# MIT-SPARK/Khronos

Hardware: AMD Instinct MI355X
Metric: active-window frames/sec (+ Mvoxel-updates/sec) at 1280x720 RGB-D+labels, 2 cm voxels (higher is better)
Workload: dtype f32

## Files before the change

### include/khronos_amd.h

```cpp
#ifndef KHRONOS_AMD_H_
#define KHRONOS_AMD_H_

#include <stddef.h>
#include <stdint.h>

#ifdef __cplusplus
extern "C" {
#endif

#define KHR_OK 0
#define KHR_EINVAL (-1)
#define KHR_ENOMEM (-2)
#define KHR_EDEVICE (-3)
#define KHR_ENOTFOUND (-4)
#define KHR_ESTATE (-5)

#define KHR_VOX_ACTIVE 1u
#define KHR_VOX_EVER_FREE 2u
#define KHR_VOX_TO_REMOVE 4u
#define KHR_VOX_SEM_VALID 8u
#define KHR_BLK_UPDATED 1u
#define KHR_BLK_MESH_UPDATED 2u
#define KHR_BLK_TRACKING_UPDATED 4u
#define KHR_BLK_HAS_ACTIVE_DATA 8u
// ... 8 lines not shown
  int32_t use_weight_dropoff;
  float weight_dropoff_epsilon;
  int32_t use_constant_weight;
  float max_weight;
  int32_t interpolation_method;
  float adaptive_max_range_difference;
  int32_t range_mode;
  int32_t semantic_mode;
  float label_confidence;
  float temporal_buffer;
  float tsdf_occupancy_threshold;
  int32_t neighbor_connectivity;
  float temporal_window;
  int32_t md_neighbor_connectivity;
  int32_t md_min_cluster_size;
  int32_t md_max_cluster_size;
  float md_min_separation_distance;
  float md_max_range;
  float md_min_z_coordinate;
  float mesh_min_weight;
  uint32_t max_blocks;
  uint32_t max_frame_pixels;
  uint32_t num_frame_slots;
  uint64_t max_mesh_vertices;
  uint32_t max_band_records;
  int32_t disable_culling;
  int32_t device;
  int32_t rank;
  int32_t world_size;
  int32_t relaxed_arithmetic;
  uint32_t max_snapshot_blocks;
  int32_t alloc_candidate;
  int32_t color_blend_weight;
  int32_t mesh_attr_source;
  float mesh_degenerate_eps;
  int32_t packed_likelihood_rows;
} khr_config;

typedef struct khr_sensor {
  int32_t width, height;
  float fx, fy, cx, cy;
  float min_range, max_range;
} khr_sensor;

typedef struct khr_frame {
  uint64_t timestamp_ns;
  double world_T_sensor[16];
  const float* depth;
  const uint8_t* color;
  const int32_t* label;
} khr_frame;

typedef struct khr_stats {
  uint64_t n_allocated_blocks;
  uint64_t n_visible_blocks;
  uint64_t n_new_blocks;
  uint64_t n_visited_voxels;
  uint64_t n_updated_voxels;
  uint64_t n_band_voxels;
  uint64_t n_tracking_updated_blocks;
  uint64_t n_seeds;
  uint64_t n_mesh_blocks;
  uint64_t n_mesh_vertices;
  uint64_t pool_exhausted;
  uint64_t cum_updated_voxels;
  uint64_t cum_band_voxels;
  uint64_t cum_visited_voxels;
  uint64_t cum_integrate_calls;
  uint64_t n_tsdf_blocks;
  uint64_t band_overflow;
  uint64_t n_tracking_processed_blocks;
  uint64_t n_fuse_items;
  uint64_t n_seed_waits;
  uint64_t n_seed_waits_late;
  uint64_t seed_wait_max_us;
  uint64_t seed_wait_hist[8];
  uint64_t seed_wait_late_us;
  uint64_t seed_wait_late_frame;
  uint64_t seed_wait_late_state;
  uint64_t n_md_device_merges;
  uint64_t n_md_host_walks;
  uint64_t n_md_prelaunched;
  uint64_t n_md_prelaunch_repeats;
} khr_stats;

typedef struct khr_cluster {
  int32_t id;
  uint64_t num_pixels_listed;
  uint32_t num_pixels_painted;
  float bbox_min[3], bbox_max[3];
  float centroid[3];
  int32_t semantic_id;
} khr_cluster;

typedef struct khr_object_detector_config {
  int32_t use_full_connectivity;
  int32_t min_cluster_size;
  int32_t max_cluster_size;
  int32_t use_3d;
  float grid_size;
  float max_range;
  const int32_t* object_labels;
  int32_t n_object_labels;
} khr_object_detector_config;

typedef struct khr_ctx khr_ctx;

int khr_create(const khr_config* cfg, khr_ctx** out);
void khr_destroy(khr_ctx* ctx);
const char* khr_last_error(void);

void khr_host_trace(const char* tag);
int khr_set_stream(khr_ctx* ctx, void* hip_stream);
int khr_sync(khr_ctx* ctx);
void khr_default_config(khr_config* cfg);
int khr_reset_map(khr_ctx* ctx, float voxel_size, float truncation_distance);
int khr_retain_slot(khr_ctx* ctx, int slot);
int khr_release_slot(khr_ctx* ctx, int slot);
int khr_depend_on(khr_ctx* ctx, khr_ctx* other);
int khr_get_config(khr_ctx* ctx, khr_config* out);

int khr_upload_frame(khr_ctx* ctx, const khr_sensor* sensor, const khr_frame* frame, int on_device);
int khr_set_frame_image(khr_ctx* ctx, int slot, int which, const int32_t* image, int on_device);
int khr_download_frame(khr_ctx* ctx, int slot, float* range, float* vertex_map, int32_t* dynamic_image);
int khr_download_frame_image(khr_ctx* ctx, int slot, int which, int32_t* image);
typedef struct khr_frame_copy khr_frame_copy;
int khr_frame_copy_create(khr_ctx* ctx, int slot, khr_frame_copy** out);
int khr_frame_copy_download(khr_frame_copy* fc, float* depth, float* range, uint8_t* color_rgb, int32_t* labels, float* vertex_map);
void khr_frame_copy_release(khr_frame_copy* fc);
int khr_copy_frame_image(khr_ctx* ctx, int slot, int which, void* device_dst);

int khr_integrate(khr_ctx* ctx, int slot, int allocate_blocks, int use_mask, int object_id);
int khr_integrate_shared(khr_ctx* ctx, khr_ctx* src, int src_slot, int allocate_blocks, int use_mask, int object_id);
int khr_integrate_shared_batch(khr_ctx* ctx, khr_ctx* src, const int* src_slots, const int* object_ids, int n_frames,
                               int allocate_blocks, int use_mask);
int khr_update_tracking(khr_ctx* ctx, uint64_t timestamp_ns);
int khr_update_tracking_phase(khr_ctx* ctx, uint64_t timestamp_ns, int phase);
#define KHR_HALO_RECORD_BYTES 528
int khr_export_halo(khr_ctx* ctx, void* records, int64_t cap_records, int on_device);
int khr_import_halo(khr_ctx* ctx, const void* records, int64_t n_records, int on_device);
int khr_detect_motion(khr_ctx* ctx, int slot);
int khr_motion_keys(khr_ctx* ctx, int slot, void* keys_out, int on_device, uint32_t* n_seed_pixels);
int khr_detect_motion_from_keys(khr_ctx* ctx, int slot, const void* keys, int on_device);
size_t khr_motion_bits_bytes(int64_t n_pixels);
int khr_motion_bits(khr_ctx* ctx, int slot, void* bits_device);
int khr_detect_motion_from_bits(khr_ctx* ctx, int slot, const void* bits_device);
int khr_dynamic_pack_bytes(khr_ctx* ctx, int slot, void* dst_device);
int khr_dynamic_unpack_bytes(khr_ctx* ctx, int slot, const void* src_device);
int khr_mirror_dynamic(khr_ctx* ctx, int src_slot, int dst_slot);
int khr_get_dynamic_clusters(khr_ctx* ctx, int slot, khr_cluster* out, int cap);
int khr_configure_object_detector(khr_ctx* ctx, const khr_object_detector_config* cfg);
int khr_detect_objects(khr_ctx* ctx, int slot);
int khr_detect_objects_launch(khr_ctx* ctx, int slot);
int khr_get_semantic_clusters(khr_ctx* ctx, int slot, khr_cluster* out, int cap);
int64_t khr_cluster_voxels(khr_ctx* ctx, int slot, int which, float voxel_size, int32_t* ids_out, int64_t* voxels_out,
                           int64_t cap);
int khr_cluster_voxels_launch(khr_ctx* ctx, int slot, int which, float voxel_size);
int64_t khr_cluster_voxels_fetch(khr_ctx* ctx, int which, int32_t* ids_out, int64_t* voxels_out, int64_t cap);
int khr_configure_object_voxel_sets(khr_ctx* ctx, float voxel_size);
typedef struct khr_pixel_ref {
  int32_t slot;
  int32_t which;
  int32_t id;
} khr_pixel_ref;
int khr_pixel_iou(khr_ctx* ctx, int slot, const khr_pixel_ref* refs, int n_refs, int max_id, uint32_t* n_points, uint32_t* inter);
int khr_forward_instances(khr_ctx* ctx, int slot, float max_range, const int32_t* background_ids, int n_background, int max_id,
// ... 228 lines not shown
```

### khronos_amd/capi.py

```python
import ctypes as C
import os

import numpy as np

_HERE = os.path.dirname(os.path.abspath(__file__))
LIB_PATH = os.path.join(_HERE, "lib", "libkhronos_amd.so")

KHR_OK, KHR_EINVAL, KHR_ENOMEM, KHR_EDEVICE, KHR_ENOTFOUND, KHR_ESTATE = 0, -1, -2, -3, -4, -5
VOX_ACTIVE, VOX_EVER_FREE, VOX_TO_REMOVE, VOX_SEM_VALID = 1, 2, 4, 8
BLK_UPDATED, BLK_MESH_UPDATED, BLK_TRACKING_UPDATED, BLK_HAS_ACTIVE_DATA = 1, 2, 4, 8


class KhrConfig(C.Structure):
    _fields_ = [
        ("voxel_size", C.c_float), ("voxels_per_side", C.c_int32), ("truncation_distance", C.c_float),
        ("with_semantics", C.c_int32), ("with_tracking", C.c_int32), ("num_labels", C.c_int32),
        ("use_weight_dropoff", C.c_int32), ("weight_dropoff_epsilon", C.c_float),
        ("use_constant_weight", C.c_int32), ("max_weight", C.c_float), ("interpolation_method", C.c_int32),
        ("adaptive_max_range_difference", C.c_float), ("range_mode", C.c_int32), ("semantic_mode", C.c_int32),
        ("label_confidence", C.c_float),
        ("temporal_buffer", C.c_float), ("tsdf_occupancy_threshold", C.c_float),
        ("neighbor_connectivity", C.c_int32), ("temporal_window", C.c_float),
        ("md_neighbor_connectivity", C.c_int32), ("md_min_cluster_size", C.c_int32),
        ("md_max_cluster_size", C.c_int32), ("md_min_separation_distance", C.c_float),
# ... 21 lines not shown


class KhrQueryStats(C.Structure):
    _fields_ = [(n, C.c_uint64) for n in ("n_value", "n_gradient", "n_voxel")]


KHR_QP_VALUE, KHR_QP_GRADIENT, KHR_QP_VOXEL = 1, 2, 4


class KhrDfRequest(C.Structure):
    _fields_ = [("origin", C.c_int32 * 3), ("dims", C.c_int32 * 3), ("ratio", C.c_int32), ("min_weight", C.c_float),
                ("max_distance", C.c_float), ("surface_distance", C.c_float), ("unknown_is_obstacle", C.c_int32),
                ("positive_only", C.c_int32)]


class KhrDfStats(C.Structure):
    _fields_ = [(n, C.c_uint64) for n in ("n_observed", "n_obstacle", "n_free", "n_in_range")]


KHR_DF_OBSERVED, KHR_DF_OBSTACLE, KHR_DF_IN_RANGE = 1, 2, 4
KHR_DF_MAX_DIM, KHR_DF_FAR = 512, 1 << 30


class KhrAlignRequest(C.Structure):
    _fields_ = [("n", C.c_int64), ("points", C.c_void_p), ("depth", C.c_void_p), ("sensor", KhrSensor), ("stride", C.c_int32),
                ("weights", C.c_void_p), ("world_T_source", C.c_double * 16), ("min_weight", C.c_float), ("gate", C.c_float),
                ("huber_delta", C.c_float)]


class KhrAlignOptions(C.Structure):
    _fields_ = [("max_iterations", C.c_int32), ("min_inliers", C.c_int32), ("lambda_", C.c_double), ("eps_rot", C.c_double),
                ("eps_trans", C.c_double)]


class KhrAlignResult(C.Structure):
    _fields_ = [("iterations", C.c_int32), ("converged", C.c_int32), ("n_inlier_first", C.c_uint64), ("n_inlier_last", C.c_uint64),
                ("rmse_first", C.c_double), ("rmse_last", C.c_double), ("H", C.c_double * 21), ("b", C.c_double * 6)]


KHR_ALIGN_WORDS, KHR_ALIGN_MAX_SOURCES = 32, 1 << 20


class KhrFrame(C.Structure):
    _fields_ = [("timestamp_ns", C.c_uint64), ("world_T_sensor", C.c_double * 16), ("depth", C.c_void_p),
                ("color", C.c_void_p), ("label", C.c_void_p)]


class KhrConvertedFrame(C.Structure):
    _fields_ = [("timestamp_ns", C.c_uint64), ("world_T_sensor", C.c_double * 16), ("range", C.c_void_p), ("depth", C.c_void_p),
                ("rgba", C.c_void_p), ("label", C.c_void_p), ("tile_max", C.c_void_p)]


class KhrCluster(C.Structure):
    _fields_ = [("id", C.c_int32), ("num_pixels_listed", C.c_uint64), ("num_pixels_painted", C.c_uint32),
                ("bbox_min", C.c_float * 3), ("bbox_max", C.c_float * 3), ("centroid", C.c_float * 3),
                ("semantic_id", C.c_int32)]


class KhrObjectDetectorConfig(C.Structure):
    _fields_ = [("use_full_connectivity", C.c_int32), ("min_cluster_size", C.c_int32), ("max_cluster_size", C.c_int32),
                ("use_3d", C.c_int32), ("grid_size", C.c_float), ("max_range", C.c_float),
                ("object_labels", C.POINTER(C.c_int32)), ("n_object_labels", C.c_int32)]


CKPT_SECTIONS = ("indices", "distance", "weight", "color", "last_observed", "last_occupied", "flags", "sem_label", "block_flags",
                 "likelihoods")


class KhrCheckpointHeader(C.Structure):
    _fields_ = [("magic", C.c_uint32), ("version", C.c_uint32), ("voxel_size", C.c_float), ("voxels_per_side", C.c_int32),
                ("truncation_distance", C.c_float), ("with_semantics", C.c_int32), ("with_tracking", C.c_int32),
                ("num_labels", C.c_int32), ("semantic_mode", C.c_int32), ("header_bytes", C.c_uint32),
                ("num_blocks", C.c_uint64), ("total_bytes", C.c_uint64), ("offset", C.c_uint64 * len(CKPT_SECTIONS))]


class KhrStats(C.Structure):
    _fields_ = [(n, C.c_uint64) for n in (
        "n_allocated_blocks", "n_visible_blocks", "n_new_blocks", "n_visited_voxels", "n_updated_voxels",
        "n_band_voxels", "n_tracking_updated_blocks", "n_seeds", "n_mesh_blocks", "n_mesh_vertices",
        "pool_exhausted", "cum_updated_voxels", "cum_band_voxels", "cum_visited_voxels", "cum_integrate_calls", "n_tsdf_blocks", "band_overflow",
        "n_tracking_processed_blocks", "n_fuse_items", "n_seed_waits", "n_seed_waits_late", "seed_wait_max_us")] + [
        ("seed_wait_hist", C.c_uint64 * 8)] + [(n, C.c_uint64) for n in (
        "seed_wait_late_us", "seed_wait_late_frame", "seed_wait_late_state", "n_md_device_merges", "n_md_host_walks",
        "n_md_prelaunched", "n_md_prelaunch_repeats")]


EXPORTS = [
    "khr_create", "khr_destroy", "khr_last_error", "khr_host_trace", "khr_set_stream", "khr_sync", "khr_default_config",
    "khr_upload_frame", "khr_set_frame_image", "khr_download_frame", "khr_frame_copy_create", "khr_frame_copy_download", "khr_frame_copy_release", "khr_integrate", "khr_update_tracking",
    "khr_detect_motion", "khr_generate_mesh", "khr_reset_inactive", "khr_mark_all_inactive", "khr_clear_updated",
    "khr_allocate_blocks", "khr_object_prune", "khr_get_stats", "khr_num_blocks", "khr_block_indices",
    "khr_download_block", "khr_mesh_num_vertices", "khr_download_mesh", "khr_fetch_mesh", "khr_fetch_mesh_into", "khr_timing_enable", "khr_timing_reset",
    "khr_timing_get", "khr_debug_read", "khr_tick_ingest", "khr_tick_integrate", "khr_tick_live_bound", "khr_tick_seed_counts", "khr_converted_bytes", "khr_export_converted",
    "khr_converted_views", "khr_tick_adopt", "khr_copy_frame_image", "khr_rv_detect_changes", "khr_last_removed", "khr_process_frame", "khr_ingest_ahead", "khr_ingest_ahead_host", "khr_ingest_cancel", "khr_integrate_shared", "khr_integrate_shared_batch", "khr_pixel_iou", "khr_forward_instances", "khr_update_tracking_phase",
    "khr_export_halo", "khr_import_halo", "khr_get_dynamic_clusters", "khr_motion_keys", "khr_motion_bits_bytes", "khr_motion_bits", "khr_detect_motion_from_bits",
    "khr_dynamic_pack_bytes", "khr_dynamic_unpack_bytes",
    "khr_detect_motion_from_keys", "khr_download_updated", "khr_mesh_halo_requests", "khr_mesh_halo_export",
    "khr_mesh_halo_requests_sorted", "khr_mesh_halo_plan", "khr_mesh_halo_answer", "khr_mesh_halo_adopt",
    "khr_mesh_halo_import", "khr_configure_object_detector", "khr_detect_objects", "khr_get_semantic_clusters",
    "khr_cluster_voxels", "khr_download_frame_image", "khr_detect_objects_launch", "khr_pool_exhausted", "khr_map_digest",
    "khr_rv_create", "khr_rv_destroy", "khr_rv_clear", "khr_rv_add_rays", "khr_rv_num_rays", "khr_rv_num_pairs", "khr_rv_check",
    "khr_snapshot_updated", "khr_take_snapshot", "khr_snapshot_num_blocks", "khr_snapshot_download", "khr_snapshot_download_extra", "khr_snapshot_download_begin", "khr_snapshot_download_end", "khr_snapshot_poll", "khr_fetch_mesh_launch", "khr_reserve_mesh_staging", "khr_reserve_snapshots", "khr_mirror_dynamic", "khr_snapshot_release",
    "khr_rv_check_stamps", "khr_get_config", "khr_cluster_voxels_launch", "khr_cluster_voxels_fetch", "khr_reset_map", "khr_depend_on", "khr_retain_slot", "khr_release_slot",
    "khr_map_slice", "khr_slice_voxel_z", "khr_render_view", "khr_query_points",
    "khr_align_linearize", "khr_align_frame", "khr_distance_field",
    "khr_checkpoint_size", "khr_checkpoint_save", "khr_checkpoint_load", "khr_checkpoint_inspect",
    "khr_debug_live_resources", "khr_configure_object_voxel_sets",
]

_lib = None


class KhronosAmdError(RuntimeError):
    pass


def load_library():
    global _lib
    if _lib is not None:
        return _lib
    if not os.path.exists(LIB_PATH):
        raise KhronosAmdError(
            "HIP extension %s is missing: run `python -c 'import __graft_entry__ as g; g.build()'`. "
            "The khronos_amd fusion path has no CPU fallback." % LIB_PATH)
    lib = C.CDLL(LIB_PATH)
    vp, i32, i64, u64 = C.c_void_p, C.c_int, C.c_int64, C.c_uint64
    lib.khr_create.argtypes = [C.POINTER(KhrConfig), C.POINTER(vp)]
    lib.khr_create.restype = i32
    lib.khr_destroy.argtypes = [vp]
    lib.khr_destroy.restype = None
    lib.khr_last_error.restype = C.c_char_p
    lib.khr_host_trace.argtypes = [C.c_char_p]
    lib.khr_host_trace.restype = None
    lib.khr_set_stream.argtypes = [vp, vp]
    lib.khr_sync.argtypes = [vp]
    lib.khr_default_config.argtypes = [C.POINTER(KhrConfig)]
    lib.khr_default_config.restype = None
    lib.khr_upload_frame.argtypes = [vp, C.POINTER(KhrSensor), C.POINTER(KhrFrame), i32]
    lib.khr_set_frame_image.argtypes = [vp, i32, i32, vp, i32]
    lib.khr_download_frame.argtypes = [vp, i32, vp, vp, vp]
    lib.khr_integrate.argtypes = [vp, i32, i32, i32, i32]
    lib.khr_integrate_shared.argtypes = [vp, vp, i32, i32, i32, i32]
    lib.khr_integrate_shared_batch.argtypes = [vp, vp, vp, vp, i32, i32, i32]
    lib.khr_update_tracking.argtypes = [vp, u64]
    lib.khr_update_tracking_phase.argtypes = [vp, u64, i32]
    lib.khr_export_halo.argtypes = [vp, vp, i64, i32]
    lib.khr_import_halo.argtypes = [vp, vp, i64, i32]
    lib.khr_detect_motion.argtypes = [vp, i32]
    lib.khr_motion_keys.argtypes = [vp, i32, vp, i32, C.POINTER(C.c_uint32)]
    lib.khr_detect_motion_from_keys.argtypes = [vp, i32, vp, i32]
    lib.khr_get_dynamic_clusters.argtypes = [vp, i32, C.POINTER(KhrCluster), i32]
    lib.khr_configure_object_detector.argtypes = [vp, C.POINTER(KhrObjectDetectorConfig)]
    lib.khr_detect_objects.argtypes = [vp, i32]
    lib.khr_pixel_iou.argtypes = [vp, i32, vp, i32, i32, vp, vp]
    lib.khr_forward_instances.argtypes = [vp, i32, C.c_float, vp, i32, i32, C.POINTER(KhrCluster)]
    lib.khr_download_frame_image.argtypes = [vp, i32, i32, vp]
    lib.khr_rv_create.argtypes = [C.c_float, C.c_float, C.c_float, i32, C.POINTER(vp)]
    lib.khr_rv_destroy.argtypes = [vp]
    lib.khr_rv_destroy.restype = None
    lib.khr_rv_clear.argtypes = [vp]
    lib.khr_rv_add_rays.argtypes = [vp, C.c_int64, vp, vp, vp]
    lib.khr_rv_num_rays.argtypes = [vp]
    lib.khr_rv_num_rays.restype = C.c_int64
    lib.khr_rv_num_pairs.argtypes = [vp]
    lib.khr_rv_num_pairs.restype = C.c_int64
    lib.khr_rv_check.argtypes = [vp, C.c_int64, vp, vp, vp, vp, vp, C.POINTER(C.c_uint64), C.POINTER(C.c_uint64)]
    lib.khr_rv_check_stamps.argtypes = [vp, vp, vp]
# ... 1045 lines not shown
```

### khronos_amd/csrc/khr_device.h

```cpp
#pragma once
#include <hip/hip_runtime.h>
#include <stdint.h>

namespace khr {

constexpr uint64_t kEmptyKey = ~0ull;
constexpr uint32_t kInvalidSlot = 0xffffffffu;

constexpr uint32_t BLK_UPDATED = 1u, BLK_MESH_UPDATED = 2u, BLK_TRACKING_UPDATED = 4u, BLK_HAS_ACTIVE = 8u,
                   BLK_LIVE = 16u,
                   BLK_TRACK_DIRTY = 32u,
                   BLK_ANY_KEEP = 64u,
                   BLK_HAS_NEG = 128u;
constexpr uint8_t VOX_ACTIVE = 1, VOX_EVER_FREE = 2, VOX_TO_REMOVE = 4, VOX_SEM_VALID = 8;
constexpr uint8_t VOX_OCC = 16;
constexpr uint8_t VOX_PUBLIC_MASK = 0x0f;

enum Counter : int {
  C_FREE_HEAD = 0,
  C_N_FREE,
  C_MAX_SLOT,
  C_N_VISIBLE,
  C_N_NEW,
  C_N_EF,
  C_N_LIVE,
  C_POOL_EXHAUSTED,
  C_N_UPD_LO,
  C_N_REMOVED,
  C_N_SEEDS,
  C_N_MESH,
  C_N_BAND,
  C_N_TSDF,
  C_BAND_OVERFLOW,
  C_TSDF_CURSOR,
  C_MESH_OVERFLOW,
  C_N_PROC,
  C_N_EF_A,
  C_N_PROC2,
  C_N_EF2,
  C_MP_DONE,
  C_N_ITEMS0,
  C_N_ITEMS1,
  C_N_ITEMS2,
  C_N_ITEMS3,
  C_COUNT = 32
};
enum Stat64 : int { S_UPD = 0 , S_BAND , S_MESH_VERTS, S_PRUNED, S_CUM_UPD, S_CUM_BAND, S_CUM_VISITED, S_CUM_CALLS, S_COUNT = 8 };

struct MeshDesc {
  uint32_t offset;
  uint32_t count;
};

struct DevMap {
  uint64_t* ht_keys;
  uint32_t* ht_vals;
  uint32_t ht_mask;
  uint32_t capacity;
  int4* blk_index;
  uint32_t* blk_flags;
  float* dist;
  float* weight;
  uint32_t* color;
  uint64_t* last_obs;
  ulonglong2* obs;
  uint64_t* last_occ;
  uint64_t* trk_lim;
  uint8_t* vflags;
  uint32_t* sem_label;
  float* lik;
  uint64_t* freebits;
  uint16_t* blk_band;
  uint32_t* free_slots;
  uint32_t* counters;
  unsigned long long* stats;
  MeshDesc* mesh_desc;
};

constexpr int kBandSlots = 32;
constexpr uint16_t kItemTouched = 0x8000u, kItemNeg = 0x4000u, kItemBandMask = 0x3fffu;
struct FuseList {
  uint4* a;
  uint4* b;
  uint32_t cap;
  uint32_t* counts;
};
__device__ inline uint32_t fuseClass(uint32_t band) { return band > 128u ? 0u : (band > 64u ? 1u : (band > 0u ? 2u : 3u)); }
__device__ inline uint4* fuseDescPtr(const FuseList& l, uint32_t cls, uint32_t pos) {
  uint4* const arr = cls < 2u ? l.a : l.b;
  return arr + ((cls & 1u) ? l.cap - 1u - pos : pos);
}

__host__ __device__ inline int likStride(int K) { return K <= 4 ? K : ((K + 31) & ~31); }

struct DevParams {
  float vs, vs_inv, bs, bs_inv, trunc;
  int vps, nvox, K;
  int KS;
  int with_semantics, with_tracking;
  int use_dropoff, const_weight, interp, range_mode, sem_mode;
  float dropoff_eps, max_weight, adaptive_diff, log_match, log_nomatch;
  float occ_thr;
  double temporal_buffer, temporal_window;
  int nn;
  float mesh_min_weight;
  float mesh_eps;
  int mesh_attr_source;
  int alloc_candidate;
  int rank, world;
  int dbg;
};

struct DevFrame {
  const float* depth;
  const float* range;
  const uint32_t* rgba;
  const int32_t* label;
  int32_t* dyn;
  const int32_t* obj;
  int W, H;
  float fx, fy, cx, cy, min_range, max_range;
  float R[9], t[3];
  float Rw[9], tw[3];
  uint64_t stamp;
  int has_color, has_label;
};

struct DevFrustum {
  float n[4][3];
  float infl;
  int3 bc;
  int n_steps;
  int max_steps;
  float tw[3];
};

__host__ __device__ inline uint32_t mix32(uint32_t h) {
  h ^= h >> 16;
  h *= 0x85ebca6bu;
  h ^= h >> 13;
  h *= 0xc2b2ae35u;
  h ^= h >> 16;
  return h;
}

__host__ __device__ inline int ownerOf(int x, int y, int z, int world) {
  if (world <= 1) return 0;
  const uint32_t h = mix32(static_cast<uint32_t>(x) * 73856093u ^
                           mix32(static_cast<uint32_t>(y) * 19349663u ^ mix32(static_cast<uint32_t>(z) * 83492791u)));
  return static_cast<int>((static_cast<uint64_t>(h) * static_cast<uint64_t>(world)) >> 32);
}

__host__ __device__ inline uint64_t packKey(int x, int y, int z) {
  return (static_cast<uint64_t>(static_cast<uint32_t>(x + (1 << 20)) & 0x1fffffu)) |
         (static_cast<uint64_t>(static_cast<uint32_t>(y + (1 << 20)) & 0x1fffffu) << 21) |
         (static_cast<uint64_t>(static_cast<uint32_t>(z + (1 << 20)) & 0x1fffffu) << 42);
}
__host__ __device__ inline void unpackKey(uint64_t k, int* x, int* y, int* z) {
  *x = static_cast<int>(k & 0x1fffffu) - (1 << 20);
  *y = static_cast<int>((k >> 21) & 0x1fffffu) - (1 << 20);
  *z = static_cast<int>((k >> 42) & 0x1fffffu) - (1 << 20);
}
__host__ __device__ inline uint32_t hashKey(uint64_t k) {
  return mix32(static_cast<uint32_t>(k) ^ mix32(static_cast<uint32_t>(k >> 32) + 0x9e3779b9u));
}

__device__ inline uint32_t htLookup(const DevMap& m, uint64_t key) {
  uint32_t h = hashKey(key) & m.ht_mask;
// ... 88 lines not shown
  if (!(vx >= 0 && vy >= 0 && vz >= 0 && vx < p.vps && vy < p.vps && vz < p.vps)) return ~0ull;
  *lin_out = vx + p.vps * (vy + p.vps * vz);
  return packKey(bx * p.vps + vx, by * p.vps + vy, bz * p.vps + vz);
}
__device__ inline uint64_t motionPixelKey(const DevMap& m, const DevParams& p, float r, float d, int u, int v, float fx,
                                          float fy, float cx, float cy, const float* Rw, const float* tw,
                                          float md_max_range, float min_z_world, int ignore_epoch = 0) {
  uint64_t bkey = 0ull;
  int lin = 0;
  uint64_t key = motionPixelVoxel(p, r, d, u, v, fx, fy, cx, cy, Rw, tw, md_max_range, min_z_world, &bkey, &lin);
  if (key == ~0ull) return key;
  uint32_t slot = htLookup(m, bkey);
  if (slot != kInvalidSlot && ignore_epoch != 0 && m.blk_index[slot].w == ignore_epoch) slot = kInvalidSlot;
  if (slot == kInvalidSlot) return ~0ull;
  if (m.vflags[static_cast<size_t>(slot) * p.nvox + lin] & VOX_EVER_FREE) key |= kSeedFlag;
  return key;
}

__device__ inline uint64_t lastObserved(const DevMap& m, size_t slot, uint32_t lin, int nvox) {
  const ulonglong2 w = m.obs[slot * static_cast<size_t>(nvox >> 6) + (lin >> 6)];
  return ((w.x >> (lin & 63u)) & 1ull) ? w.y : m.last_obs[slot * static_cast<size_t>(nvox) + lin];
}

__device__ inline double toSeconds(uint64_t ns) { return static_cast<double>(ns) / 1e9; }

__device__ inline uint32_t laneId() { return __lane_id(); }

__device__ inline uint32_t waveAggInc(uint32_t* counter, bool pred) {
  const unsigned long long mask = __ballot(pred);
  if (mask == 0) return 0;
  const uint32_t lane = laneId();
  const uint32_t rank = __popcll(mask & ((1ull << lane) - 1ull));
  const int leader = __ffsll(static_cast<long long>(mask)) - 1;
  uint32_t base = 0;
  if (lane == static_cast<uint32_t>(leader)) base = atomicAdd(counter, static_cast<uint32_t>(__popcll(mask)));
  base = __shfl(base, leader);
  return base + rank;
}

__device__ inline uint8_t toU8(float f) {
  float r = floorf(f + 0.5f);
  r = fminf(255.f, fmaxf(0.f, r));
  return static_cast<uint8_t>(r);
}

__device__ inline void publishSeedCount(const DevMap& m, volatile uint32_t* host_seed, uint32_t ticket) {
  host_seed[0] = atomicAdd(&m.counters[C_N_SEEDS], 0u);
  __threadfence_system();
  host_seed[1] = ticket;
  __threadfence_system();
}

constexpr int kUpdateStatSlots = 2048;

__device__ inline void beginIntegrate(DevMap m, int nvox, uint32_t* wg_stats) {
  unsigned long long u = 0, b = 0;
  uint2* __restrict__ st = reinterpret_cast<uint2*>(wg_stats);
#pragma unroll 4
  for (int i = threadIdx.x; i < kUpdateStatSlots; i += blockDim.x) {
    const uint2 v = st[i];
    u += v.x;
    b += v.y;
    if (v.x | v.y) st[i] = make_uint2(0u, 0u);
  }
#pragma unroll
  for (int o = 32; o > 0; o >>= 1) {
    u += __shfl_down(u, o);
    b += __shfl_down(b, o);
  }
  if ((threadIdx.x & 63) == 0 && (u | b)) {
    atomicAdd(&m.stats[S_CUM_UPD], u);
    atomicAdd(&m.stats[S_CUM_BAND], b);
  }
  if (threadIdx.x == 0) {
    m.stats[S_CUM_VISITED] += static_cast<unsigned long long>(m.counters[C_N_VISIBLE]) * nvox;
    m.stats[S_CUM_CALLS] += 1ull;
    m.counters[C_N_VISIBLE] = 0u;
    m.counters[C_N_NEW] = 0u;
    m.counters[C_N_TSDF] = 0u;
    m.counters[C_N_ITEMS0] = 0u;
    m.counters[C_N_ITEMS1] = 0u;
    m.counters[C_N_ITEMS2] = 0u;
    m.counters[C_N_ITEMS3] = 0u;
  }
}

__device__ inline uint32_t ufLoad(const uint32_t* parent, uint32_t x) { return __atomic_load_n(parent + x, __ATOMIC_RELAXED); }
__device__ inline uint32_t ufFind(uint32_t* parent, uint32_t x) {
  uint32_t p = ufLoad(parent, x);
  while (p != x) {
    const uint32_t gp = ufLoad(parent, p);
    if (gp != p) atomicMin(parent + x, gp);
    x = p;
    p = gp;
  }
  return x;
}
__device__ inline uint32_t ufFind(const uint32_t* parent, uint32_t x) {
  while (true) {
    const uint32_t p = ufLoad(parent, x);
    if (p == x) return x;
    x = p;
  }
}
__device__ inline void ufUnion(uint32_t* parent, uint32_t a, uint32_t b) {
  a = ufFind(parent, a);
  b = ufFind(parent, b);
  while (a != b) {
    if (a < b) { const uint32_t t = a; a = b; b = t; }
    const uint32_t old = atomicCAS(parent + a, a, b);
    if (old == a) return;
    a = ufFind(parent, old);
  }
}

}
```

### khronos_amd/csrc/khr_kernels_fuse.h

```cpp
#pragma once
#include "khr_device.h"
#include "khr_fuse_math.h"

namespace khr {

typedef float f2u __attribute__((ext_vector_type(2), aligned(4)));

struct FuseFrame {
  const float* range;
  const int32_t* dyn;
  const uint32_t* rgba;
  const int32_t* label;
  const int32_t* obj;
  int W, H;
  float fx, fy, cx, cy, min_range, max_range;
  float R[9], t[3];
  uint64_t stamp;
  int use_mask, do_sem, has_color, object_id;
  const float* tile_max;
  int tw, th;
};

struct FuseArgs : FuseFrame {
  const int4* blk_index;
  uint32_t* blk_flags;
  float* dist;
  float* weight;
  uint64_t* last_obs;
  ulonglong2* obs;
  uint32_t* color;
  uint8_t* vflags;
  uint32_t* sem_label;
  float* lik;
  uint32_t* wg_stats;
  uint16_t* blk_band;
  float vs, bs, trunc, dropoff_eps, max_weight, adaptive_diff, log_match, log_nomatch;
  int interp, range_mode, use_dropoff, const_weight, with_tracking;
  int K, sem_mode;
  int KS;
  int band_mode;
  int blend_pre;
  const uint32_t* gate;
  void* sink;
  const FuseFrame* frames;
  int n_frames;
  uint8_t* item_mask;
  const uint32_t* frame_bits;
  int frame_words;
  int frame_bit0;
};

constexpr int kRecCap = 256;

typedef uint32_t u4v __attribute__((ext_vector_type(4)));
typedef const u4v __attribute__((address_space(4))) * DescK;

__device__ __forceinline__ uint32_t firstListPos() { return (blockIdx.x & 7u) * (gridDim.x >> 3) + (blockIdx.x >> 3); }
__device__ __forceinline__ uint32_t pullListPos(uint32_t* s_q, int lane, uint32_t first) {
  uint32_t j = 0u;
  if (lane == 0) j = atomicAdd(s_q, 1u);
  j = static_cast<uint32_t>(__builtin_amdgcn_readfirstlane(static_cast<int>(j)));
  return first + gridDim.x * j;
}
__device__ __forceinline__ uint4 descOf(const FuseList& list, uint32_t nc0, uint32_t nc1, uint32_t nc2, uint32_t i) {
  const DescK la = (DescK)list.a, lb = (DescK)list.b;
  u4v d;
  if (i < nc0) d = la[i];
  else if (i < nc1) d = la[list.cap - 1u - (i - nc0)];
  else if (i < nc2) d = lb[i - nc1];
  else d = lb[list.cap - 1u - (i - nc2)];
  return make_uint4(d.x, d.y, d.z, d.w);
}
__device__ __forceinline__ FuseFrame loadFuseFrame(const FuseFrame* p) {
  FuseFrame F;
  const uint32_t __attribute__((address_space(4)))* const w = (const uint32_t __attribute__((address_space(4)))*)p;
  uint32_t* const d = reinterpret_cast<uint32_t*>(&F);
#pragma unroll
  for (int i = 0; i < static_cast<int>(sizeof(FuseFrame) / 4); ++i) d[i] = w[i];
  return F;
}
__device__ __forceinline__ bool frameMayTouch(const FuseArgs& a, size_t item, int fi, uint32_t& fbits) {
  if (a.frame_bits == nullptr) return true;
  const int gf = fi + a.frame_bit0;
  if ((gf & 31) == 0 || fi == 0)
    fbits = *(const uint32_t __attribute__((address_space(4)))*)(a.frame_bits + item * static_cast<size_t>(a.frame_words) + static_cast<size_t>(gf >> 5));
  return ((fbits >> (gf & 31)) & 1u) != 0u;
}
__device__ __forceinline__ void multiItemEpilogue(const FuseArgs& a, size_t slot, int sbi, int lane, bool touched, bool wrote_neg, uint32_t cnt) {
  if (lane == 0) {
    if (touched) atomicOr(&a.blk_flags[slot], BLK_UPDATED | BLK_MESH_UPDATED | BLK_TRACKING_UPDATED | (wrote_neg ? BLK_HAS_NEG : 0u));
    a.blk_band[slot * kBandSlots + (sbi & (kBandSlots - 1))] = static_cast<uint16_t>(min(cnt, 65535u));
  }
}
template <int WPW>
__device__ __forceinline__ void statsEpilogue(uint32_t (&s_stat)[WPW][2], int wave, int lane, uint32_t n_upd, uint32_t n_band, uint32_t* wg_stats) {
  if (lane == 0) {
    s_stat[wave][0] = n_upd;
    s_stat[wave][1] = n_band;
  }
  __syncthreads();
  if (threadIdx.x == 0) {
    uint32_t su = 0u, sb = 0u;
#pragma unroll
    for (int w = 0; w < WPW; ++w) {
      su += s_stat[w][0];
      sb += s_stat[w][1];
    }
    if (su | sb) {
      wg_stats[2 * blockIdx.x] += su;
      wg_stats[2 * blockIdx.x + 1] += sb;
    }
  }
}


typedef const FuseArgs __attribute__((address_space(4))) * FuseArgsK;
typedef const FuseFrame __attribute__((address_space(4))) * FuseFrameK;
constexpr int kLikVec = 5;
template <int VPS>
__device__ inline void fuseBandRecord(FuseArgsK ka, FuseFrameK kf, size_t slot, uint32_t lin_mode, float w, float w_new, float u, float v) {
  constexpr int NV = VPS * VPS * VPS;
  const FuseArgs __attribute__((address_space(4)))& a = *ka;
  const FuseFrame __attribute__((address_space(4)))& f = *kf;
  const uint32_t lin = lin_mode & 0xffffu;
  const bool use_nearest = (lin_mode & 0x10000u) != 0;
  const int K = a.K;
  const bool has_color = f.has_color != 0, do_sem = f.do_sem != 0, vec = (K & 3) == 0;
  char* const color_b = reinterpret_cast<char*>(a.color + slot * NV);
  char* const vfl_b = reinterpret_cast<char*>(a.vflags + slot * NV);
  char* const lab_b = reinterpret_cast<char*>(a.sem_label + slot * NV);
  char* const lik_b = reinterpret_cast<char*>(a.lik + slot * NV * static_cast<size_t>(a.KS));
  const uint32_t lik_o = lin * static_cast<uint32_t>(a.KS) * 4u;
  int px4[4];
  float du, dv, w4[4];
  interpPixels(u, v, f.W, f.H, px4, &du, &dv);
  const int best = interpWeights(du, dv, use_nearest, w4);
  const uint32_t best_o = static_cast<uint32_t>(px4[best]) * 4u;
  uint32_t c4[4] = {0u, 0u, 0u, 0u}, co = 0u;
  if (has_color) {
    const char* const rgba_b = reinterpret_cast<const char*>(f.rgba);
#pragma unroll
    for (int k = 0; k < 4; ++k) c4[k] = *reinterpret_cast<const uint32_t*>(rgba_b + static_cast<uint32_t>(px4[k]) * 4u);
    co = *reinterpret_cast<const uint32_t*>(color_b + lin * 4u);
  }
  int label = -1;
// ... 129 lines not shown
      if (p0 > 0) {
#pragma unroll
        for (int p = 0; p < kRowPasses; ++p) {
          const uint32_t rl = min((p0 + static_cast<uint32_t>(p)) * rpp + rl0, n_here - 1u);
          l4[p] = *reinterpret_cast<const float4*>(lik_b + ((rec[base + rl] & 0xffffu) * row_bytes + j16));
        }
      }
#pragma unroll
      for (int p = 0; p < kRowPasses; ++p) {
        const uint32_t rl_own = (p0 + static_cast<uint32_t>(p)) * rpp + rl0;
        const uint32_t rl = min(rl_own, n_here - 1u);
        const uint32_t pk = rec[CAP + base + rl];
        const uint32_t off = (rec[base + rl] & 0xffffu) * row_bytes + j16;
        const bool on = (pk & 0x80000000u) != 0u;
        const int lab = static_cast<int>(pk & 0xffffu);
        const bool emp = (pk & 0x40000000u) != 0u;
        float l[4] = {l4[p].x, l4[p].y, l4[p].z, l4[p].w};
        float bv = -__builtin_inff();
        uint32_t bk = 0xffffu;
#pragma unroll
        for (int q = 0; q < 4; ++q) {
          const int k = 4 * static_cast<int>(j) + q;
          if (k < K) {
            if (emp) l[q] = 0.f;
            l[q] += (k == lab) ? add_hit : add_miss;
            if (k == 0 || l[q] > bv) {
              bv = l[q];
              bk = static_cast<uint32_t>(k);
            }
          } else {
            l[q] = 0.f;
          }
        }
        *reinterpret_cast<float4*>(lik_b + off) = on ? make_float4(l[0], l[1], l[2], l[3]) : l4[p];
        auto take = [&](float ov, uint32_t ok, uint32_t sh) {
          if (j + sh < lpr && ov > bv) {
            bv = ov;
            bk = ok;
          }
        };
        take(__uint_as_float(rowDown<1>(__float_as_uint(bv))), rowDown<1>(bk), 1u);
        take(__uint_as_float(rowDown<2>(__float_as_uint(bv))), rowDown<2>(bk), 2u);
        take(__uint_as_float(rowDown<4>(__float_as_uint(bv))), rowDown<4>(bk), 4u);
        if (lpr > 8u) take(__uint_as_float(rowDown<8>(__float_as_uint(bv))), rowDown<8>(bk), 8u);
        for (uint32_t sh = 16u; sh < lpr; sh <<= 1) {
          const float ov = __shfl_down(bv, sh);
          const uint32_t ok = static_cast<uint32_t>(__shfl_down(static_cast<int>(bk), sh));
          take(ov, ok, sh);
        }
        if (on && j == 0u && rl_own < n_here) rec[2 * CAP + base + rl] = bk;
      }
    }
    __builtin_amdgcn_fence(__ATOMIC_RELEASE, "wavefront");
    __builtin_amdgcn_wave_barrier();
    __builtin_amdgcn_fence(__ATOMIC_ACQUIRE, "wavefront");
    if (valid && upd) {
      *reinterpret_cast<uint32_t*>(lab_b + lin * 4u) = rec[2 * CAP + r];
      if (empty) *reinterpret_cast<uint8_t*>(vfl_b + lin) = fl | VOX_SEM_VALID;
    }
  }
}

template <int VPS, int ZR>
struct FuseItem {
  size_t slot;
  int z0, sbi;
  float oz, pxy2;
  int lin_xy;
  float u[ZR], v[ZR], z[ZR], yz[ZR], d[ZR], w[ZR];
  f2u ra[ZR], rb[ZR];
};

template <int VPS, int ZSPLIT, bool DEFCFG, bool EXACT, int WPW>
__global__ __launch_bounds__(64 * WPW) void k_fuse(FuseArgs a, FuseList list) {
  constexpr int NV = VPS * VPS * VPS;
  constexpr int SL = VPS * VPS;
  constexpr int PATCHES = SL / 64;
  constexpr int ZR = VPS / ZSPLIT;
  static_assert(SL % 64 == 0 && VPS % ZSPLIT == 0 && (ZR == 2 || ZR == 4), "bad block shape");
  static_assert(64 * ZR <= kRecCap, "record list must hold one item");
  __shared__ uint32_t s_rec[WPW][5][kRecCap];
  __shared__ uint32_t s_stat[WPW][2];
  __shared__ uint32_t s_q;
  const int wave = __builtin_amdgcn_readfirstlane(static_cast<int>(threadIdx.x >> 6));
  const int lane = static_cast<int>(threadIdx.x & 63);
  const int range_mode = DEFCFG ? 0 : a.range_mode;
  const int interp = DEFCFG ? 2 : a.interp;
  const bool use_dropoff = DEFCFG ? true : (a.use_dropoff != 0);
  const bool const_weight = DEFCFG ? false : (a.const_weight != 0);
  const float Wm1 = static_cast<float>(a.W - 1), Hm1 = static_cast<float>(a.H - 1);
  const float fxfy = a.fx * a.fy;
  const float den = a.trunc - a.dropoff_eps;
  const float yden = rcpRefined(den);
  const char* const range_b = reinterpret_cast<const char*>(a.range);
  const uint32_t W4 = static_cast<uint32_t>(a.W) * 4u;
  const uint32_t n_items = list.counts[0] + list.counts[1] + list.counts[2] + list.counts[3];
  uint32_t n_upd = 0, n_band = 0;
  if (a.gate != nullptr && *a.gate != 0u) return;
  if (threadIdx.x == 0) s_q = 0u;
  __syncthreads();
  char* const sink_b = reinterpret_cast<char*>(a.sink) + (static_cast<size_t>(blockIdx.x) * WPW + static_cast<size_t>(wave)) * 256u;
  const bool trk = a.with_tracking != 0;
  const uint32_t first = firstListPos();
  auto pull = [&]() -> uint32_t { return pullListPos(&s_q, lane, first); };
  auto descOf = [&](uint32_t i) -> uint4 {
    typedef const FuseList __attribute__((address_space(4))) * FuseListK;
    const char __attribute__((address_space(4)))* kb = (const char __attribute__((address_space(4)))*)__builtin_amdgcn_kernarg_segment_ptr();
    asm volatile("" : "+s"(kb));
    const FuseListK kl = (FuseListK)(kb + ((sizeof(FuseArgs) + 7u) & ~static_cast<size_t>(7)));
    const uint32_t __attribute__((address_space(4)))* const kc = (const uint32_t __attribute__((address_space(4)))*)kl->counts;
    const uint32_t c0 = kc[0], c1 = c0 + kc[1], c2 = c1 + kc[2];
    const DescK la = (DescK)kl->a, lb = (DescK)kl->b;
    const uint32_t cap = kl->cap;
    u4v d;
    if (i < c0) d = la[i];
    else if (i < c1) d = la[cap - 1u - (i - c0)];
    else if (i < c2) d = lb[i - c1];
    else d = lb[cap - 1u - (i - c2)];
    return make_uint4(d.x, d.y, d.z, d.w);
  };

  auto phase1 = [&](FuseItem<VPS, ZR>& it, const uint4 desc) {
    const uint32_t dx = static_cast<uint32_t>(__builtin_amdgcn_readfirstlane(static_cast<int>(desc.x)));
    it.slot = dx & 0xffffffu;
    it.sbi = static_cast<int>(dx >> 24);
    const int bx = __builtin_amdgcn_readfirstlane(static_cast<int>(desc.y));
    const int by = __builtin_amdgcn_readfirstlane(static_cast<int>(desc.z));
    const int bz = __builtin_amdgcn_readfirstlane(static_cast<int>(desc.w));
    const int patch = it.sbi % PATCHES;
    it.z0 = (it.sbi / PATCHES) * ZR;
    const float ox = static_cast<float>(bx) * a.bs, oy = static_cast<float>(by) * a.bs;
    it.oz = static_cast<float>(bz) * a.bs;
    it.lin_xy = patch * 64 + lane;
    const int ix = it.lin_xy % VPS, iy = it.lin_xy / VPS;
    const float px = ox + (static_cast<float>(ix) + 0.5f) * a.vs;
    const float py = oy + (static_cast<float>(iy) + 0.5f) * a.vs;
    float pxy[3];
#pragma unroll
    for (int c = 0; c < 3; ++c) pxy[c] = a.R[3 * c] * px + a.R[3 * c + 1] * py;
    it.pxy2 = pxy[2];
    const char* const dist_b = reinterpret_cast<const char*>(a.dist + it.slot * NV);
    const char* const wgt_b = reinterpret_cast<const char*>(a.weight + it.slot * NV);
#pragma unroll
    for (int k = 0; k < ZR; ++k) {
      const int iz = it.z0 + k;
      const uint32_t lin = static_cast<uint32_t>(it.lin_xy + iz * SL);
      const float pz = it.oz + (static_cast<float>(iz) + 0.5f) * a.vs;
      const VoxelProj p = projectVoxel(a, pxy, pz, Wm1, Hm1, range_mode);
      const PairOffsets o = pairOffsets<true>(p.uc, p.vc, a.H, W4);
      it.ra[k] = *reinterpret_cast<const f2u*>(range_b + o.o0);
      it.rb[k] = *reinterpret_cast<const f2u*>(range_b + o.o1);
      it.d[k] = *reinterpret_cast<const float*>(dist_b + lin * 4u);
      it.w[k] = *reinterpret_cast<const float*>(wgt_b + lin * 4u);
      it.u[k] = p.uc;
      it.v[k] = p.vc;
      it.z[k] = p.ok ? p.range : -1.f;
      it.yz[k] = p.yz;
    }
  };

  auto phase2 = [&](FuseItem<VPS, ZR>& cur) {
    const size_t slot = cur.slot;
    char* const dist_b = reinterpret_cast<char*>(a.dist + slot * NV);
    char* const wgt_b = reinterpret_cast<char*>(a.weight + slot * NV);
    char* const lobs_b = reinterpret_cast<char*>(a.last_obs + slot * NV);
    uint32_t cnt = 0;
    bool touched = false;
    bool wrote_neg = false;
    const size_t w0 = slot * static_cast<size_t>(NV / 64) + static_cast<size_t>(cur.z0 * PATCHES + cur.sbi % PATCHES);
    u4v ow_next = trk ? ((DescK)(a.obs + w0))[0] : u4v{0u, 0u, 0u, 0u};
#pragma unroll
    for (int k = 0; k < ZR; ++k) {
      const u4v ow_k = ow_next;
      if (k + 1 < ZR && trk) ow_next = ((DescK)(a.obs + w0))[(k + 1) * PATCHES];
      bool ok = cur.z[k] >= 0.f;
      const int iz = cur.z0 + k;
      const uint32_t lin = static_cast<uint32_t>(cur.lin_xy + iz * SL);
      const float d_old = cur.d[k], w_old = cur.w[k];
      float d_out = d_old, w_out = w_old;
      if (__builtin_amdgcn_ballot_w64(ok) != 0ull) {
      const float uc = cur.u[k], vc = cur.v[k], voxel_range = cur.z[k], yz = cur.yz[k];
      float depth = voxel_range;
      if (range_mode != 0) {
        const float pz = cur.oz + (static_cast<float>(iz) + 0.5f) * a.vs;
        depth = (cur.pxy2 + a.R[8] * pz) + a.t[2];
      }
      const SurfaceSample s = sampleSurface(ok, cur.ra[k].x, cur.ra[k].y, cur.rb[k].x, cur.rb[k].y, uc, vc, a.W, interp, a.adaptive_diff, voxel_range,
                                            a.min_range, a.max_range, a.trunc);
      const float sdf = s.sdf;
      const bool use_nearest = s.use_nearest;
      ok = s.ok;
      bool in_band = s.in_band;
      if (__builtin_expect(a.use_mask && __builtin_amdgcn_ballot_w64(in_band) != 0ull, 0)) {
        const PairOffsets o = pairOffsets<false>(uc, vc, a.H, W4);
        if (in_band && *reinterpret_cast<const int32_t*>(reinterpret_cast<const char*>(a.dyn) + maskPixelOffset(s, o.o0, o.o1)) != 0) {
          ok = false;
          in_band = false;
        }
      }
      if (__builtin_amdgcn_ballot_w64(ok) != 0ull) {
      const float w = measurementWeight<EXACT>(a.vs, fxfy, depth, yz, sdf, a.trunc, a.dropoff_eps, den, yden, use_dropoff, const_weight);
      ok = ok && (w > 0.f);
      in_band = in_band && ok;
      const VoxelAverage avg = runningAverage<EXACT>(d_old, w_old, sdf, w, a.trunc, a.max_weight);
      const float d_new = avg.d_new, w_new = avg.w_new;
      if (ok) {
        d_out = d_new;
        w_out = w_new;
      }
      const unsigned long long m_band = __builtin_amdgcn_ballot_w64(in_band);
      wrote_neg = wrote_neg || (__builtin_amdgcn_ballot_w64(ok && d_new < 0.f) != 0ull);
      if (m_band) {
        n_band += static_cast<uint32_t>(__popcll(m_band));
        if (in_band) {
          const uint32_t pos = cnt + __builtin_amdgcn_mbcnt_hi(static_cast<uint32_t>(m_band >> 32),
                                                              __builtin_amdgcn_mbcnt_lo(static_cast<uint32_t>(m_band), 0u));
          uint32_t* const rec = &s_rec[wave][0][pos];
          rec[0] = lin | (use_nearest ? 0x10000u : 0u);
          rec[kRecCap] = __float_as_uint(w);
          rec[2 * kRecCap] = __float_as_uint(a.blend_pre ? w_old : w_new);
          rec[3 * kRecCap] = __float_as_uint(uc);
          rec[4 * kRecCap] = __float_as_uint(vc);
        }
        cnt += static_cast<uint32_t>(__popcll(m_band));
      }
      } else {
        ok = false;
      }
      }
      const unsigned long long m_ok = __builtin_amdgcn_ballot_w64(ok);
      n_upd += static_cast<uint32_t>(__popcll(m_ok));
      touched = touched || (m_ok != 0ull);
      {
        char* const d_b = m_ok != 0ull ? dist_b : sink_b;
        char* const w_b = m_ok != 0ull ? wgt_b : sink_b;
        const uint32_t vo = (m_ok != 0ull ? lin : static_cast<uint32_t>(lane)) * 4u;
        *reinterpret_cast<float*>(d_b + vo) = d_out;
        *reinterpret_cast<float*>(w_b + vo) = w_out;
      }
      {
        const uint64_t bits0 = static_cast<uint64_t>(ow_k.x) | (static_cast<uint64_t>(ow_k.y) << 32);
        const uint64_t stamp0 = static_cast<uint64_t>(ow_k.z) | (static_cast<uint64_t>(ow_k.w) << 32);
        const bool same = stamp0 == a.stamp;
        const uint64_t mat = (m_ok != 0ull && !same) ? (bits0 & ~m_ok) : 0ull;
        const uint64_t nb = m_ok == 0ull ? bits0 : (same ? (bits0 | m_ok) : m_ok);
        const uint64_t ns = m_ok == 0ull ? stamp0 : a.stamp;
        const bool real = trk && mat != 0ull;
        char* const st_b = real ? lobs_b : sink_b;
        const uint32_t first_lin = lin - static_cast<uint32_t>(lane) + static_cast<uint32_t>(__builtin_ctzll(mat | (1ull << 63)));
        const bool mine = ((mat >> static_cast<uint32_t>(lane)) & 1ull) != 0ull;
        const uint32_t so = real ? (mine ? lin : first_lin) * 8u : 0u;
        *reinterpret_cast<uint64_t*>(st_b + so) = stamp0;
        ulonglong2* const wp = trk ? (a.obs + w0 + k * PATCHES) : reinterpret_cast<ulonglong2*>(sink_b + 16);
        *wp = make_ulonglong2(nb, ns);
      }
    }
    const uint32_t item_band = cnt;
    if (__builtin_expect(cnt > 0u, 0)) {
      __builtin_amdgcn_fence(__ATOMIC_RELEASE, "wavefront");
      __builtin_amdgcn_wave_barrier();
      FuseArgsK ka = (FuseArgsK)__builtin_amdgcn_kernarg_segment_ptr();
      asm volatile("" : "+s"(ka));
      const FuseFrameK kf = (FuseFrameK)ka;
      if (ka->band_mode != 0 && fuseBandRowsOk(ka->KS, ka->sem_mode, ka->do_sem, ka->has_color)) {
        fuseBandRows<VPS>(ka, kf, slot, &s_rec[wave][0][0], cnt, lane);
      } else {
        for (uint32_t r = static_cast<uint32_t>(lane); r < cnt; r += 64u) {
          const uint32_t* const rec = &s_rec[wave][0][r];
          fuseBandRecord<VPS>(ka, kf, slot, rec[0], __uint_as_float(rec[kRecCap]), __uint_as_float(rec[2 * kRecCap]),
                              __uint_as_float(rec[3 * kRecCap]), __uint_as_float(rec[4 * kRecCap]));
        }
      }
      __builtin_amdgcn_fence(__ATOMIC_ACQUIRE, "wavefront");
      __builtin_amdgcn_wave_barrier();
      __builtin_amdgcn_s_waitcnt(0x0f70);
    }
    {
      const uint32_t recw = min(item_band, static_cast<uint32_t>(kItemBandMask)) | (touched ? kItemTouched : 0u) | (wrote_neg ? kItemNeg : 0u);
      a.blk_band[slot * kBandSlots + (cur.sbi & (kBandSlots - 1))] = static_cast<uint16_t>(recw);
    }
  };

  uint32_t item = pull();
  if (item < n_items) {
    FuseItem<VPS, ZR> sa, sb;
    uint4 d_cur = descOf(item);
    phase1(sa, d_cur);
    uint32_t item_next = pull();
    uint4 d_next = item_next < n_items ? descOf(item_next) : d_cur;
    while (true) {
      {
        phase1(sb, d_next);
        const uint32_t item_nn = item_next < n_items ? pull() : 0xffffffffu;
        const uint4 d_nn = item_nn < n_items ? descOf(item_nn) : d_next;
        phase2(sa);
        if (item_next >= n_items) break;
        item_next = item_nn;
        d_next = d_nn;
      }
      {
        phase1(sa, d_next);
        const uint32_t item_nn = item_next < n_items ? pull() : 0xffffffffu;
        const uint4 d_nn = item_nn < n_items ? descOf(item_nn) : d_next;
        phase2(sb);
        if (item_next >= n_items) break;
        item_next = item_nn;
        d_next = d_nn;
      }
    }
  }
  statsEpilogue<WPW>(s_stat, wave, lane, n_upd, n_band, a.wg_stats);
}

__global__ __launch_bounds__(256) void k_fuse_fold(uint32_t* __restrict__ blk_flags, uint16_t* __restrict__ blk_band,
                                                  const uint32_t* __restrict__ max_slot, const uint32_t* gate) {
  if (gate != nullptr && *gate != 0u) return;
  const uint32_t s = blockIdx.x * blockDim.x + threadIdx.x;
  if (s >= *max_slot) return;
  foldItemRecords(blk_flags, blk_band, s);
}

template <int VPS, int ZSPLIT, bool EXACT, int WPW, int MINW>
__global__ __launch_bounds__(64 * WPW, MINW) void k_fuse2(FuseArgs a, FuseList list) {
  constexpr int NV = VPS * VPS * VPS;
  constexpr int SL = VPS * VPS;
  constexpr int PATCHES = SL / 64;
  constexpr int ZR = VPS / ZSPLIT;
  constexpr int CAP = 64 * ZR;
  static_assert(SL % 64 == 0 && VPS % ZSPLIT == 0 && (ZR == 2 || ZR == 4), "bad block shape");
  __shared__ uint32_t s_rec[WPW][5][CAP];
  __shared__ uint32_t s_stat[WPW][2];
  __shared__ uint32_t s_q;
  const int wave = __builtin_amdgcn_readfirstlane(static_cast<int>(threadIdx.x >> 6));
  const int lane = static_cast<int>(threadIdx.x & 63);
  const float den = a.trunc - a.dropoff_eps;
  const float yden = rcpRefined(den);
  const uint32_t nc0 = list.counts[0], nc1 = nc0 + list.counts[1], nc2 = nc1 + list.counts[2], n_items = nc2 + list.counts[3];
  uint32_t n_upd = 0, n_band = 0;
  if (a.gate != nullptr && *a.gate != 0u) return;
  if (threadIdx.x == 0) s_q = 0u;
  __syncthreads();
  const uint32_t first = firstListPos();
  uint32_t item = pullListPos(&s_q, lane, first);
  uint4 desc = make_uint4(0u, 0u, 0u, 0u);
  if (item < n_items) desc = descOf(list, nc0, nc1, nc2, item);
  while (item < n_items) {
    const uint32_t item_next = pullListPos(&s_q, lane, first);
    uint4 d_next = make_uint4(0u, 0u, 0u, 0u);
    if (item_next < n_items) d_next = descOf(list, nc0, nc1, nc2, item_next);
    const size_t slot = desc.x & 0xffffffu;
    const int sbi = static_cast<int>(desc.x >> 24);
    const int bx = static_cast<int>(desc.y), by = static_cast<int>(desc.z), bz = static_cast<int>(desc.w);
    const int patch = sbi % PATCHES;
    const int z0 = (sbi / PATCHES) * ZR;
    const float ox = static_cast<float>(bx) * a.bs, oy = static_cast<float>(by) * a.bs, oz = static_cast<float>(bz) * a.bs;
    const int lin_xy = patch * 64 + lane;
    const int ix = lin_xy % VPS, iy = lin_xy / VPS;
    const float px = ox + (static_cast<float>(ix) + 0.5f) * a.vs;
    const float py = oy + (static_cast<float>(iy) + 0.5f) * a.vs;
    char* const dist_b = reinterpret_cast<char*>(a.dist + slot * NV);
    char* const wgt_b = reinterpret_cast<char*>(a.weight + slot * NV);
    char* const lobs_b = reinterpret_cast<char*>(a.last_obs + slot * NV);
    const size_t mi = slot * static_cast<size_t>(PATCHES * ZSPLIT) + static_cast<size_t>(sbi);
    bool touched = false, wrote_neg = false;
    uint32_t cnt = 0;
    const int n_frames = a.n_frames;
    float dreg[ZR], wreg[ZR];
    int lidx[ZR];
#pragma unroll
    for (int k = 0; k < ZR; ++k) {
      const uint32_t lin = static_cast<uint32_t>(lin_xy + (z0 + k) * SL);
      dreg[k] = *reinterpret_cast<const float*>(dist_b + lin * 4u);
      wreg[k] = *reinterpret_cast<const float*>(wgt_b + lin * 4u);
      lidx[k] = -1;
    }
    uint32_t frame_mask = ~0u;
    if (a.item_mask != nullptr) {
      const uint32_t word = *(const uint32_t __attribute__((address_space(4)))*)(a.item_mask + (mi & ~static_cast<size_t>(3)));
      frame_mask = (word >> (8u * static_cast<uint32_t>(mi & 3))) & 0xffu;
      asm volatile("" : "+s"(frame_mask) : : "memory");
      if (lane == 0) a.item_mask[mi] = 0;
    }
    uint32_t fbits = ~0u;
    for (int fi = 0; fi < n_frames; ++fi) {
    if (((frame_mask >> fi) & 1u) == 0u) continue;
    if (!frameMayTouch(a, mi, fi, fbits)) {
      cnt = 0;
      continue;
    }
    const FuseFrame F = loadFuseFrame(a.frames + fi);
// ... 409 lines not shown
```

### khronos_amd/csrc/khr_kernels_fusion.h

```cpp
#pragma once
#include "khr_device.h"

namespace khr {


constexpr int kTile = 16;
constexpr int kMaxTick = 8;

__device__ inline void ingestTile(const float* __restrict__ depth_in, const uint8_t* __restrict__ rgb_in,
                                  const int32_t* __restrict__ label_in, float* __restrict__ depth, float* __restrict__ range,
                                  uint32_t* __restrict__ rgba, int32_t* __restrict__ label, int32_t* __restrict__ dyn,
                                  float* __restrict__ tile_max, int tile, int tw, int W, int H, float fx, float fy, float cx,
                                  float cy, int range_mode, float* d_out, float* r_out) {
  const int tx = tile % tw, ty = tile / tw;
  const int u = tx * kTile + (threadIdx.x & 15), v = ty * kTile + (threadIdx.x >> 4);
  float r = 0.f, d = 0.f;
  if (u < W && v < H) {
    const int i = v * W + u;
    d = depth_in[i];
    if (d > 0.f && isfinite(d)) {
      if (range_mode == 0) {
        r = d;
      } else {
        const float x = (static_cast<float>(u) - cx) / fx, y = (static_cast<float>(v) - cy) / fy;
        r = d * sqrtf((x * x + y * y) + 1.f);
      }
    }
    depth[i] = d;
    range[i] = r;
    dyn[i] = 0;
    if (rgb_in)
      rgba[i] = static_cast<uint32_t>(rgb_in[3 * i]) | (static_cast<uint32_t>(rgb_in[3 * i + 1]) << 8) |
                (static_cast<uint32_t>(rgb_in[3 * i + 2]) << 16) | 0xff000000u;
    if (label_in) label[i] = label_in[i];
  }
  *d_out = d;
  *r_out = r;
  float rm = r;
#pragma unroll
  for (int o = 32; o > 0; o >>= 1) rm = fmaxf(rm, __shfl_down(rm, o));
  __shared__ float s[4];
  if ((threadIdx.x & 63) == 0) s[threadIdx.x >> 6] = rm;
  __syncthreads();
  if (threadIdx.x == 0) tile_max[tile] = fmaxf(fmaxf(s[0], s[1]), fmaxf(s[2], s[3]));
}

__global__ __launch_bounds__(256) void k_frame_ingest(const float* __restrict__ depth_in,
                                                     const uint8_t* __restrict__ rgb_in,
                                                     const int32_t* __restrict__ label_in, float* __restrict__ depth,
                                                     float* __restrict__ range, uint32_t* __restrict__ rgba,
                                                     int32_t* __restrict__ label, int32_t* __restrict__ dyn,
                                                     float* __restrict__ tile_max, int tw, int W, int H, float fx,
                                                     float fy, float cx, float cy, int range_mode, DevMap m, int nvox,
                                                     uint32_t* __restrict__ wg_stats, int do_begin) {
  if (blockIdx.x == 0 && threadIdx.x == 0) m.counters[C_N_SEEDS] = 0u;
  if (do_begin && blockIdx.x == 0) beginIntegrate(m, nvox, wg_stats);
  float d, r;
  ingestTile(depth_in, rgb_in, label_in, depth, range, rgba, label, dyn, tile_max, blockIdx.x, tw, W, H, fx, fy, cx, cy,
             range_mode, &d, &r);
}

struct TickIngest {
  const float* depth_in[kMaxTick];
  const uint8_t* rgb_in[kMaxTick];
  const int32_t* label_in[kMaxTick];
  float* depth[kMaxTick];
  float* range[kMaxTick];
  uint32_t* rgba[kMaxTick];
  int32_t* label[kMaxTick];
  int32_t* dyn[kMaxTick];
  float* tile_max[kMaxTick];
  float Rw[kMaxTick][9], tw[kMaxTick][3], min_z_world[kMaxTick];
};
__global__ __launch_bounds__(256) void k_tick_ingest(TickIngest t, int tw, int W, int H, float fx, float fy, float cx, float cy,
                                                    int range_mode, DevMap m, DevParams p, float md_max_range, int count_seeds,
                                                    uint32_t* __restrict__ seed_counts) {
  const int cam = blockIdx.y;
  if (blockIdx.x == 0 && cam == 0 && threadIdx.x == 0) m.counters[C_N_SEEDS] = 0u;
  float d, r;
  ingestTile(t.depth_in[cam], t.rgb_in[cam], t.label_in[cam], t.depth[cam], t.range[cam], t.rgba[cam], t.label[cam], t.dyn[cam],
             t.tile_max[cam], blockIdx.x, tw, W, H, fx, fy, cx, cy, range_mode, &d, &r);
  if (!count_seeds) return;
  const int u = (blockIdx.x % tw) * kTile + (threadIdx.x & 15), v = (blockIdx.x / tw) * kTile + (threadIdx.x >> 4);
  bool seed = false;
  if (u < W && v < H) {
    const uint64_t key = motionPixelKey(m, p, r, d, u, v, fx, fy, cx, cy, t.Rw[cam], t.tw[cam], md_max_range, t.min_z_world[cam]);
    seed = key != ~0ull && (key & kSeedFlag);
  }
  const unsigned long long b = __ballot(seed);
  if (b && laneId() == static_cast<uint32_t>(__ffsll(static_cast<long long>(b)) - 1))
    atomicAdd(&seed_counts[cam], static_cast<uint32_t>(__popcll(b)));
}

struct TickAdopt {
  const float* range[kMaxTick];
  const float* depth[kMaxTick];
  int32_t* dyn[kMaxTick];
  float Rw[kMaxTick][9], tw[kMaxTick][3], min_z_world[kMaxTick];
};
__global__ __launch_bounds__(256) void k_tick_adopt(TickAdopt t, int W, int H, float fx, float fy, float cx, float cy, DevMap m,
                                                   DevParams p, float md_max_range, int count_seeds,
                                                   uint32_t* __restrict__ seed_counts) {
  const int cam = blockIdx.y;
  if (blockIdx.x == 0 && cam == 0 && threadIdx.x == 0) m.counters[C_N_SEEDS] = 0u;
  const int i = blockIdx.x * blockDim.x + threadIdx.x;
  bool seed = false;
  if (i < W * H) {
    t.dyn[cam][i] = 0;
    if (count_seeds) {
      const float r = t.range[cam][i];
      const float d = t.depth[cam] ? t.depth[cam][i] : r;
      const uint64_t key = motionPixelKey(m, p, r, d, i % W, i / W, fx, fy, cx, cy, t.Rw[cam], t.tw[cam], md_max_range, t.min_z_world[cam]);
      seed = key != ~0ull && (key & kSeedFlag);
    }
  }
  const unsigned long long b = __ballot(seed);
  if (b && laneId() == static_cast<uint32_t>(__ffsll(static_cast<long long>(b)) - 1))
    atomicAdd(&seed_counts[cam], static_cast<uint32_t>(__popcll(b)));
}

__global__ __launch_bounds__(256) void k_pack_converted(const float* __restrict__ range, const uint32_t* __restrict__ rgba,
                                                       const int32_t* __restrict__ label, const float* __restrict__ tile_max,
                                                       const float* __restrict__ depth, uint32_t n, uint32_t n_tiles,
                                                       uint32_t tiles_padded, uint32_t* __restrict__ out) {
  const uint32_t stride = gridDim.x * blockDim.x;
  for (uint32_t i = blockIdx.x * blockDim.x + threadIdx.x; i < n; i += stride) {
    out[i] = __float_as_uint(range[i]);
    out[n + i] = rgba ? rgba[i] : 0u;
    out[2 * n + i] = label ? static_cast<uint32_t>(label[i]) : 0u;
    if (depth) out[3 * n + tiles_padded + i] = __float_as_uint(depth[i]);
  }
  for (uint32_t i = blockIdx.x * blockDim.x + threadIdx.x; i < tiles_padded; i += stride)
    out[3 * n + i] = i < n_tiles ? __float_as_uint(tile_max[i]) : 0u;
}

__global__ void k_tick_publish(uint32_t* __restrict__ counts, int n, volatile uint32_t* __restrict__ host_counts,
                               volatile uint32_t* __restrict__ host_ticket, uint32_t ticket, long long* __restrict__ dev_counts) {
  if (threadIdx.x < static_cast<uint32_t>(n)) {
    const uint32_t v = atomicAdd(&counts[threadIdx.x], 0u);
    host_counts[threadIdx.x] = v;
    if (dev_counts) dev_counts[threadIdx.x] = static_cast<long long>(v);
    counts[threadIdx.x] = 0u;
// ... 90 lines not shown
struct TickFrusta {
  float R[kMaxTick][9], t[kMaxTick][3], max_range[kMaxTick];
  DevFrustum fr[kMaxTick];
};
constexpr int kTickAllocThreads = 1024;
__global__ __launch_bounds__(kTickAllocThreads) void k_tick_alloc(DevMap m, DevParams p, TickFrusta tf, int ncam, int3 lo, int3 dim,
                                                   uint32_t* __restrict__ work, uint32_t list_stride,
                                                   uint32_t* __restrict__ new_list, uint32_t* __restrict__ tick_counts, int epoch) {
  const int total = dim.x * dim.y * dim.z;
  const int i = blockIdx.x * blockDim.x + threadIdx.x;
  uint32_t seen = 0u;
  int bx = 0, by = 0, bz = 0;
  if (i < total) {
    bx = lo.x + i % dim.x;
    by = lo.y + (i / dim.x) % dim.y;
    bz = lo.z + i / (dim.x * dim.y);
    if (ownerOf(bx, by, bz, p.world) == p.rank) {
      for (int k = 0; k < ncam; ++k) {
        const DevFrustum& fr = tf.fr[k];
        if (abs(bx - fr.bc.x) > fr.n_steps || abs(by - fr.bc.y) > fr.n_steps || abs(bz - fr.bc.z) > fr.n_steps) continue;
        const bool in = blockIsCandidate(p, fr, tf.R[k], tf.t[k], tf.max_range[k], bx, by, bz);
        if (in) seen |= 1u << k;
      }
    }
  }
  const bool visible = seen != 0u;
  uint32_t slot = kInvalidSlot;
  const uint64_t key = packKey(bx, by, bz);
  if (visible) slot = htLookup(m, key);
  const bool need = visible && slot == kInvalidSlot;
  const uint32_t fidx = waveAggInc(&m.counters[C_FREE_HEAD], need);
  bool got = false;
  if (need) {
    if (fidx < m.counters[C_N_FREE]) {
      slot = m.free_slots[fidx];
      got = true;
      m.blk_index[slot] = make_int4(bx, by, bz, epoch);
      m.blk_flags[slot] = BLK_LIVE | BLK_TRACK_DIRTY | BLK_ANY_KEEP;
      m.mesh_desc[slot] = MeshDesc{0u, 0u};
      htInsertUnique(m, key, slot);
      atomicMax(&m.counters[C_MAX_SLOT], slot + 1);
    } else {
      atomicAdd(&m.counters[C_POOL_EXHAUSTED], 1u);
      slot = kInvalidSlot;
    }
  }
  const uint32_t nidx = waveAggInc(&m.counters[C_N_NEW], got);
  if (got) new_list[nidx] = slot;
  if (slot == kInvalidSlot) seen = 0u;
  __shared__ uint32_t s_cnt[kMaxTick], s_base[kMaxTick];
  if (threadIdx.x < kMaxTick) s_cnt[threadIdx.x] = 0u;
  __syncthreads();
  uint32_t loff[kMaxTick];
#pragma unroll
  for (int k = 0; k < kMaxTick; ++k) {
    loff[k] = 0u;
    if (k < ncam) loff[k] = waveAggInc(&s_cnt[k], ((seen >> k) & 1u) != 0u);
  }
  __syncthreads();
  if (threadIdx.x < static_cast<uint32_t>(ncam)) {
    const uint32_t n = s_cnt[threadIdx.x];
    s_base[threadIdx.x] = n ? atomicAdd(&tick_counts[2 * threadIdx.x], n) : 0u;
  }
  if (threadIdx.x == 64) {
    uint32_t tot = 0u;
    for (int k = 0; k < ncam; ++k) tot += s_cnt[k];
    if (tot) atomicAdd(&m.counters[C_N_VISIBLE], tot);
  }
  __syncthreads();
#pragma unroll
  for (int k = 0; k < kMaxTick; ++k)
    if (k < ncam && ((seen >> k) & 1u)) work[static_cast<size_t>(k) * list_stride + s_base[k] + loff[k]] = slot;
}

__global__ void k_begin_integrate(DevMap m, int nvox, uint32_t* wg_stats) {
  if (blockIdx.x == 0) beginIntegrate(m, nvox, wg_stats);
}
__global__ void k_tick_begin(DevMap m, int nvox, uint32_t* wg_stats, uint32_t* tick_counts, uint32_t extra_calls) {
  beginIntegrate(m, nvox, wg_stats);
  if (threadIdx.x < 6 * kMaxTick) tick_counts[threadIdx.x] = 0u;
  if (threadIdx.x == 0) m.stats[S_CUM_CALLS] += extra_calls;
}

__device__ inline void cullBlocks(const DevMap& m, const DevParams& p, const DevFrame& f, const uint32_t* __restrict__ work,
                                  const uint32_t* __restrict__ n_work, FuseList out, uint32_t wpb,
                                  uint32_t* __restrict__ n_tsdf, const float* __restrict__ tile_max, int tw, int th,
                                  uint32_t bid, uint32_t nblk, uint32_t* __restrict__ item_mask = nullptr, uint32_t cam = 0u) {
  constexpr int kPerWg = 8;
  __shared__ uint4 s_blk[kPerWg];
  __shared__ uint16_t s_item[4][kPerWg * kBandSlots];
  __shared__ uint32_t s_nkeep, s_ccnt[4], s_off[4];
  const uint32_t n = *n_work;
  const uint32_t lane = threadIdx.x & 63;
  for (uint32_t base = bid * kPerWg; base < n; base += nblk * kPerWg) {
  if (threadIdx.x == 0) s_nkeep = 0;
  if (threadIdx.x < 4) s_ccnt[threadIdx.x] = 0;
  __syncthreads();
  for (uint32_t wi = base + (threadIdx.x >> 6); wi < min(n, base + kPerWg); wi += 4) {
    const uint32_t slot = work[wi];
    const int4 bi = m.blk_index[slot];
    bool keep = true;
    if (tile_max) {
      const float margin = 1e-3f;
      const float lo[3] = {static_cast<float>(bi.x) * p.bs + 0.5f * p.vs, static_cast<float>(bi.y) * p.bs + 0.5f * p.vs,
                           static_cast<float>(bi.z) * p.bs + 0.5f * p.vs};
      const float ext = p.bs - p.vs;
      float zmin = 1e30f, zmax = -1e30f, umin = 1e30f, umax = -1e30f, vmin = 1e30f, vmax = -1e30f;
      float pcs[8][3];
#pragma unroll
      for (int k = 0; k < 8; ++k) {
        xform(f.R, f.t, lo[0] + ((k & 1) ? ext : 0.f), lo[1] + ((k & 2) ? ext : 0.f), lo[2] + ((k & 4) ? ext : 0.f), pcs[k]);
        zmin = fminf(zmin, pcs[k][2]);
        zmax = fmaxf(zmax, pcs[k][2]);
      }
      if (zmax <= -margin) keep = false;
      if (zmin > f.max_range + margin) keep = false;
      if (p.range_mode == 0 && zmax < f.min_range - margin) keep = false;
      if (keep && zmin > 0.05f) {
#pragma unroll
        for (int k = 0; k < 8; ++k) {
          const float u = (pcs[k][0] * f.fx) / pcs[k][2] + f.cx, v = (pcs[k][1] * f.fy) / pcs[k][2] + f.cy;
          umin = fminf(umin, u); umax = fmaxf(umax, u);
          vmin = fminf(vmin, v); vmax = fmaxf(vmax, v);
        }
        if (umax < -1.f || vmax < -1.f || umin > static_cast<float>(f.W) || vmin > static_cast<float>(f.H)) {
          keep = false;
        } else {
          const int tx0 = max(0, (static_cast<int>(floorf(umin)) - 1) / kTile);
          const int ty0 = max(0, (static_cast<int>(floorf(vmin)) - 1) / kTile);
          const int tx1 = min(tw - 1, (static_cast<int>(ceilf(umax)) + 2) / kTile);
          const int ty1 = min(th - 1, (static_cast<int>(ceilf(vmax)) + 2) / kTile);
          if (tx1 >= tx0 && ty1 >= ty0) {
            const int nx = tx1 - tx0 + 1, nt = nx * (ty1 - ty0 + 1);
            float mr = 0.f;
            for (int t = lane; t < nt; t += 64) mr = fmaxf(mr, tile_max[(ty0 + t / nx) * tw + tx0 + t % nx]);
#pragma unroll
            for (int o = 32; o > 0; o >>= 1) mr = fmaxf(mr, __shfl_xor(mr, o));
            if (mr < zmin - p.trunc - margin) keep = false;
          }
        }
      }
    }
    if (keep) {
      uint32_t kslot = 0;
      if (lane == 0) {
        kslot = atomicAdd(&s_nkeep, 1u);
        s_blk[kslot] = make_uint4(slot, static_cast<uint32_t>(bi.x), static_cast<uint32_t>(bi.y), static_cast<uint32_t>(bi.z));
      }
      kslot = __shfl(kslot, 0);
      const uint32_t lpi = 64u / wpb, item = lane / lpi, sub = lane % lpi;
      bool ikeep = true;
      if (tile_max && (p.dbg & 256) == 0) {
        const float margin = 1e-3f;
        const int patches = (p.vps * p.vps) >> 6, rows = 64 / p.vps, zr = p.vps / (static_cast<int>(wpb) / patches);
        const int y0 = (static_cast<int>(item) % patches) * rows, z0 = (static_cast<int>(item) / patches) * zr;
        const float lo[3] = {static_cast<float>(bi.x) * p.bs + 0.5f * p.vs, static_cast<float>(bi.y) * p.bs + (static_cast<float>(y0) + 0.5f) * p.vs,
                             static_cast<float>(bi.z) * p.bs + (static_cast<float>(z0) + 0.5f) * p.vs};
        const float ex[3] = {p.bs - p.vs, static_cast<float>(rows - 1) * p.vs, static_cast<float>(zr - 1) * p.vs};
        float zmin = 1e30f, zmax = -1e30f, umin = 1e30f, umax = -1e30f, vmin = 1e30f, vmax = -1e30f;
        float pcs[8][3];
#pragma unroll
        for (int k = 0; k < 8; ++k) {
          xform(f.R, f.t, lo[0] + ((k & 1) ? ex[0] : 0.f), lo[1] + ((k & 2) ? ex[1] : 0.f), lo[2] + ((k & 4) ? ex[2] : 0.f), pcs[k]);
          zmin = fminf(zmin, pcs[k][2]);
          zmax = fmaxf(zmax, pcs[k][2]);
        }
        if (zmax <= -margin) ikeep = false;
        if (zmin > f.max_range + margin) ikeep = false;
        if (p.range_mode == 0 && zmax < f.min_range - margin) ikeep = false;
        if (ikeep && zmin > 0.05f) {
#pragma unroll
          for (int k = 0; k < 8; ++k) {
            const float iz = __builtin_amdgcn_rcpf(pcs[k][2]);
            const float u = (pcs[k][0] * f.fx) * iz + f.cx, v = (pcs[k][1] * f.fy) * iz + f.cy;
            umin = fminf(umin, u); umax = fmaxf(umax, u);
            vmin = fminf(vmin, v); vmax = fmaxf(vmax, v);
          }
          if (umax < -2.f || vmax < -2.f || umin > static_cast<float>(f.W) + 1.f || vmin > static_cast<float>(f.H) + 1.f) {
            ikeep = false;
          } else {
            const int tx0 = max(0, (static_cast<int>(floorf(umin)) - 2) / kTile);
            const int ty0 = max(0, (static_cast<int>(floorf(vmin)) - 2) / kTile);
            const int tx1 = min(tw - 1, (static_cast<int>(ceilf(umax)) + 3) / kTile);
            const int ty1 = min(th - 1, (static_cast<int>(ceilf(vmax)) + 3) / kTile);
            const int nx = tx1 - tx0 + 1, nt = nx * (ty1 - ty0 + 1);
            if (tx1 >= tx0 && ty1 >= ty0 && nt <= 16 * static_cast<int>(lpi)) {
              float m0 = 0.f, m1 = 0.f;
              int t = static_cast<int>(sub);
              for (; t + static_cast<int>(lpi) < nt; t += 2 * static_cast<int>(lpi)) {
                const int t2 = t + static_cast<int>(lpi);
                const float a = tile_max[(ty0 + t / nx) * tw + tx0 + t % nx];
                const float b = tile_max[(ty0 + t2 / nx) * tw + tx0 + t2 % nx];
                m0 = fmaxf(m0, a);
                m1 = fmaxf(m1, b);
              }
              if (t < nt) m0 = fmaxf(m0, tile_max[(ty0 + t / nx) * tw + tx0 + t % nx]);
              float mr = fmaxf(m0, m1);
              for (uint32_t o = 1; o < lpi; o <<= 1) mr = fmaxf(mr, __shfl_xor(mr, static_cast<int>(o)));
              if (mr < zmin - p.trunc - margin) ikeep = false;
            }
          }
        }
      }
      if (ikeep && sub == 0 && item_mask) {
        const size_t mi = static_cast<size_t>(slot) * wpb + item;
        const uint32_t sh = 8u * static_cast<uint32_t>(mi & 3);
        const uint32_t old = atomicOr(&item_mask[mi >> 2], (1u << cam) << sh);
        if ((old >> sh) & 0xffu) ikeep = false;
      }
      if (ikeep && sub == 0) {
        const uint32_t cls = fuseClass(m.blk_band[static_cast<size_t>(slot) * kBandSlots + item] & kItemBandMask);
        s_item[cls][atomicAdd(&s_ccnt[cls], 1u)] = static_cast<uint16_t>((kslot << 8) | item);
      }
    }
  }
  __syncthreads();
  if (threadIdx.x < 4) s_off[threadIdx.x] = s_ccnt[threadIdx.x] ? atomicAdd(&out.counts[threadIdx.x], s_ccnt[threadIdx.x]) : 0u;
  if (threadIdx.x == 0 && s_nkeep) atomicAdd(n_tsdf, s_nkeep);
  __syncthreads();
#pragma unroll
  for (uint32_t cls = 0; cls < 4; ++cls) {
    for (uint32_t i = threadIdx.x; i < s_ccnt[cls]; i += blockDim.x) {
      const uint32_t it = s_item[cls][i];
      uint4 d = s_blk[it >> 8];
      d.x |= (it & 0xffu) << 24;
      *fuseDescPtr(out, cls, s_off[cls] + i) = d;
    }
  }
  __syncthreads();
  }
}

__global__ __launch_bounds__(256) void k_cull_blocks(DevMap m, DevParams p, DevFrame f,
                                                    const uint32_t* __restrict__ work, FuseList out, uint32_t wpb,
                                                    const float* __restrict__ tile_max, int tw, int th) {
  cullBlocks(m, p, f, work, &m.counters[C_N_VISIBLE], out, wpb, &m.counters[C_N_TSDF], tile_max, tw, th, blockIdx.x, gridDim.x);
}

struct TickFrames {
  DevFrame f[kMaxTick];
  const float* tile_max[kMaxTick];
};
__global__ __launch_bounds__(256) void k_tick_cull(DevMap m, DevParams p, TickFrames t, const uint32_t* __restrict__ work,
                                                  uint32_t list_stride, uint4* __restrict__ desc, uint32_t desc_stride, uint32_t wpb,
                                                  uint32_t* __restrict__ tick_counts, int use_tiles, int tw, int th,
                                                  uint32_t* __restrict__ item_mask) {
  const int cam = blockIdx.y;
  const int lc = item_mask ? 0 : cam;
  FuseList out{desc + static_cast<size_t>(2 * lc) * desc_stride, desc + static_cast<size_t>(2 * lc + 1) * desc_stride, desc_stride,
               &tick_counts[2 * kMaxTick + 4 * lc]};
  cullBlocks(m, p, t.f[cam], work + static_cast<size_t>(cam) * list_stride, &tick_counts[2 * cam], out, wpb, &tick_counts[2 * cam + 1],
             use_tiles ? t.tile_max[cam] : nullptr, tw, th, blockIdx.x, gridDim.x, item_mask, static_cast<uint32_t>(cam));
}

__global__ __launch_bounds__(256) void k_alloc_list(DevMap m, const int* __restrict__ idx, int n,
                                                   uint32_t* __restrict__ new_list) {
  const int i = blockIdx.x * blockDim.x + threadIdx.x;
  bool need = false;
  int bx = 0, by = 0, bz = 0;
  if (i < n) {
    bx = idx[3 * i];
    by = idx[3 * i + 1];
    bz = idx[3 * i + 2];
    need = htLookup(m, packKey(bx, by, bz)) == kInvalidSlot;
  }
  const uint32_t fidx = waveAggInc(&m.counters[C_FREE_HEAD], need);
  bool got = false;
  uint32_t slot = kInvalidSlot;
  if (need) {
    if (fidx < m.counters[C_N_FREE]) {
      slot = m.free_slots[fidx];
      got = true;
      m.blk_index[slot] = make_int4(bx, by, bz, 0);
      m.blk_flags[slot] = BLK_LIVE | BLK_TRACK_DIRTY | BLK_ANY_KEEP;
      m.mesh_desc[slot] = MeshDesc{0u, 0u};
      htInsertUnique(m, packKey(bx, by, bz), slot);
      atomicMax(&m.counters[C_MAX_SLOT], slot + 1);
    } else {
      atomicAdd(&m.counters[C_POOL_EXHAUSTED], 1u);
    }
  }
  const uint32_t nidx = waveAggInc(&m.counters[C_N_NEW], got);
  if (got) new_list[nidx] = slot;
}

__global__ __launch_bounds__(256) void k_list_live(DevMap m, uint32_t* __restrict__ work, uint32_t* counter,
                                                  uint32_t require_flags, FuseList out = FuseList{nullptr, nullptr, 0u, nullptr},
                                                  uint32_t wpb = 0u) {
  const uint32_t s = blockIdx.x * blockDim.x + threadIdx.x;
  bool live = false;
  if (s < m.counters[C_MAX_SLOT]) {
    const uint32_t fl = m.blk_flags[s];
    live = (fl & BLK_LIVE) && ((fl & require_flags) == require_flags);
  }
  const uint32_t idx = waveAggInc(counter, live);
  if (live) work[idx] = s;
  if (out.a) {
    const unsigned long long mask = __ballot(live);
    if (mask) {
      const uint32_t lane = laneId();
      const int leader = __ffsll(static_cast<long long>(mask)) - 1;
      uint32_t base = 0;
      if (lane == static_cast<uint32_t>(leader)) base = atomicAdd(&out.counts[3], static_cast<uint32_t>(__popcll(mask)) * wpb);
      base = __shfl(base, leader) + static_cast<uint32_t>(__popcll(mask & ((1ull << lane) - 1ull))) * wpb;
      if (live) {
        const int4 bi = m.blk_index[s];
        for (uint32_t it = 0; it < wpb; ++it)
          *fuseDescPtr(out, 3u, base + it) =
              make_uint4(s | (it << 24), static_cast<uint32_t>(bi.x), static_cast<uint32_t>(bi.y), static_cast<uint32_t>(bi.z));
      }
    }
  }
}

__device__ inline void initBlocks(const DevMap& m, const DevParams& p, const uint32_t* __restrict__ new_list, uint32_t bid,
                                  uint32_t nblk) {
  const uint32_t n = m.counters[C_N_NEW];
  const int nv = p.nvox;
  for (uint32_t b = bid; b < n; b += nblk) {
    const size_t slot = new_list[b];
    const uint4 z = make_uint4(0, 0, 0, 0);
    uint4* d4 = reinterpret_cast<uint4*>(m.dist + slot * nv);
    uint4* w4 = reinterpret_cast<uint4*>(m.weight + slot * nv);
    uint4* c4 = reinterpret_cast<uint4*>(m.color + slot * nv);
    uint4* l4 = reinterpret_cast<uint4*>(m.sem_label + slot * nv);
    for (int i = threadIdx.x; i < nv / 4; i += blockDim.x) {
      d4[i] = z;
      w4[i] = z;
      c4[i] = z;
      if (p.with_semantics) l4[i] = z;
    }
    uint4* f4 = reinterpret_cast<uint4*>(m.vflags + slot * nv);
    for (int i = threadIdx.x; i < nv / 16; i += blockDim.x) f4[i] = z;
    if (threadIdx.x < kBandSlots) m.blk_band[slot * kBandSlots + threadIdx.x] = 0;
    if (p.with_tracking) {
      uint4* o4 = reinterpret_cast<uint4*>(m.last_obs + slot * nv);
      uint4* q4 = reinterpret_cast<uint4*>(m.last_occ + slot * nv);
      for (int i = threadIdx.x; i < nv / 2; i += blockDim.x) {
        o4[i] = z;
        q4[i] = z;
      }
      uint64_t* fb = m.freebits + slot * (nv / 64);
      for (int i = threadIdx.x; i < nv / 64; i += blockDim.x) {
        fb[i] = 0ull;
        m.obs[slot * (nv / 64) + i] = make_ulonglong2(0ull, 0ull);
      }
    }
  }
}

__global__ __launch_bounds__(256) void k_init_blocks(DevMap m, DevParams p, const uint32_t* __restrict__ new_list) {
  initBlocks(m, p, new_list, blockIdx.x, gridDim.x);
}

__global__ __launch_bounds__(256) void k_init_cull(DevMap m, DevParams p, DevFrame f, const uint32_t* __restrict__ new_list,
                                                  const uint32_t* __restrict__ work, FuseList out, uint32_t wpb,
                                                  const float* __restrict__ tile_max, int tw, int th, uint32_t n_cull) {
  if (blockIdx.x < n_cull)
    cullBlocks(m, p, f, work, &m.counters[C_N_VISIBLE], out, wpb, &m.counters[C_N_TSDF], tile_max, tw, th, blockIdx.x, n_cull);
  else
    initBlocks(m, p, new_list, blockIdx.x - n_cull, gridDim.x - n_cull);
}

__device__ inline uint32_t foldItemRecords(uint32_t* __restrict__ blk_flags, uint16_t* __restrict__ blk_band, uint32_t s) {
  static_assert(kBandSlots == 32, "record row = 4 x 16 bytes");
  uint4* const row = reinterpret_cast<uint4*>(blk_band + static_cast<size_t>(s) * kBandSlots);
  uint32_t any = 0u;
  uint4 r[4];
#pragma unroll
  for (int i = 0; i < 4; ++i) {
    r[i] = row[i];
    any |= r[i].x | r[i].y | r[i].z | r[i].w;
  }
  const uint32_t tm = static_cast<uint32_t>(kItemTouched) * 0x00010001u, nm = static_cast<uint32_t>(kItemNeg) * 0x00010001u;
  uint32_t fl = blk_flags[s];
  if ((any & tm) == 0u) return fl;
  fl |= BLK_UPDATED | BLK_MESH_UPDATED | BLK_TRACKING_UPDATED | ((any & nm) ? BLK_HAS_NEG : 0u);
  blk_flags[s] = fl;
  const uint32_t keep = static_cast<uint32_t>(kItemBandMask) * 0x00010001u;
#pragma unroll
  for (int i = 0; i < 4; ++i) row[i] = make_uint4(r[i].x & keep, r[i].y & keep, r[i].z & keep, r[i].w & keep);
  return fl;
}
__global__ __launch_bounds__(256) void k_tracking_select(DevMap m, uint64_t lim_active, uint64_t lim_free, int force_full,
                                                        uint32_t* __restrict__ proc, uint32_t* __restrict__ ef_list,
                                                        uint32_t* __restrict__ cnt ,
                                                        uint32_t* __restrict__ cnt_next, uint16_t* __restrict__ fold_band) {
  const uint32_t s = blockIdx.x * blockDim.x + threadIdx.x;
  if (s == 0) { cnt_next[0] = 0u; cnt_next[1] = 0u; }
  bool need = false, touched = false, reload = false;
  if (s < m.counters[C_MAX_SLOT]) {
    const uint32_t fl = fold_band ? foldItemRecords(m.blk_flags, fold_band, s) : m.blk_flags[s];
    if (fl & BLK_LIVE) {
      touched = fl & BLK_TRACKING_UPDATED;
      need = force_full || (fl & (BLK_TRACKING_UPDATED | BLK_TRACK_DIRTY));
      reload = need;
      if (!need) {
        const ulonglong2 lim = reinterpret_cast<const ulonglong2*>(m.trk_lim)[s];
        need = !(lim_active <= lim.x && lim_free <= lim.y);
      }
    }
  }
  const uint32_t ip = waveAggInc(&cnt[0], need);
  if (need) {
    proc[ip] = s | (reload ? 0x80000000u : 0u);
    reinterpret_cast<ulonglong2*>(m.trk_lim)[s] = make_ulonglong2(~0ull, ~0ull);
    m.blk_flags[s] = m.blk_flags[s] & ~(BLK_TRACKING_UPDATED | BLK_HAS_ACTIVE | BLK_TRACK_DIRTY | BLK_ANY_KEEP);
  }
  const uint32_t ie = waveAggInc(&cnt[1], touched);
  if (touched) ef_list[ie] = s;
}

template <int VPS, int CH>
__global__ __launch_bounds__(256) void k_tracking_update(DevMap m, DevParams p, uint64_t stamp, uint64_t prev_stamp,
                                                        uint64_t lim_active, uint64_t lim_free,
                                                        const uint32_t* __restrict__ proc, const uint32_t* __restrict__ n_proc) {
  constexpr int NV = VPS * VPS * VPS;
  __shared__ uint64_t s_min[2][4];
  __shared__ uint32_t s_bits;
  const uint32_t n = *n_proc * CH;
  for (uint32_t wi = blockIdx.x; wi < n; wi += gridDim.x) {
    const uint32_t pe = proc[wi / CH];
    const uint32_t s = pe & 0x7fffffffu;
    const bool reload = (pe >> 31) != 0u;
    const int g0 = static_cast<int>(wi % CH) * (NV / 4 / CH);
    const size_t slot = s;
    const float4* __restrict__ dist4 = reinterpret_cast<const float4*>(m.dist + slot * NV);
    const ulonglong2* __restrict__ lobs2 = reinterpret_cast<const ulonglong2*>(m.last_obs + slot * NV);
    uint64_t* __restrict__ locc = m.last_occ + slot * NV;
    uint32_t* __restrict__ vfl4 = reinterpret_cast<uint32_t*>(m.vflags + slot * NV);
    uint64_t* __restrict__ fb = m.freebits + slot * (NV / 64);
    bool any_active = false, any_keep = false;
    uint64_t a_min = ~0ull, f_min = ~0ull;
    if (threadIdx.x == 0) s_bits = 0u;
    constexpr int G = NV / 4 / CH / 256 > 0 ? NV / 4 / CH / 256 : 1;
    constexpr int GEND = NV / 4 / CH;
    float4 d_[G];
    ulonglong2 oa_[G], ob_[G], ca_[G], cb_[G], ow_[G];
    uint32_t v4_[G];
    uint32_t need_[G];
#pragma unroll
    for (int q = 0; q < G; ++q) {
// ... 270 lines not shown
```

### khronos_amd/csrc/khronos_amd.hip

```cpp
#include <hip/hip_runtime.h>
#include <hip/hip_ext.h>
#include <hipcub/hipcub.hpp>

#include <algorithm>
#include <array>
#include <atomic>
#include <chrono>
#include <memory>
#include <mutex>
#include <cmath>
#include <cstdarg>
#include <cstdio>
#include <climits>
#include <cstring>
#include <cstdlib>
#include <functional>
#include <map>
#include <string>
#include <thread>
#include <tuple>
#include <unordered_map>
#include <vector>

#include "../../include/khronos_amd.h"
#include "khr_device.h"
#include "khr_owned.h"
#include "khr_kernels_aux.h"
#include "khr_kernels_fusion.h"
#include "khr_kernels_fuse.h"
#include "khr_kernels_objects.h"
#include "khr_kernels_slice.h"
#include "khr_kernels_render.h"
#include "khr_kernels_query.h"
#include "khr_kernels_distance.h"
#include "khr_kernels_align.h"
#include "khr_kernels_checkpoint.h"

using namespace khr;

namespace {

thread_local std::string g_last_error;

int fail(int code, const char* fmt, ...) {
  char buf[512];
  va_list ap;
  va_start(ap, fmt);
  vsnprintf(buf, sizeof(buf), fmt, ap);
  va_end(ap);
  g_last_error = buf;
  return code;
}

#define HIP_TRY(expr)                                                                              \
  do {                                                                                             \
    hipError_t _e = (expr);                                                                        \
    if (_e != hipSuccess)                                                                          \
      return fail(KHR_EDEVICE, "%s failed: %s (%s:%d)", #expr, hipGetErrorString(_e), __FILE__, __LINE__); \
  } while (0)
#define KHR_TRY(expr)                  \
  do {                                 \
    if (int _rc = (expr)) return _rc;  \
  } while (0)

#define KHR_CHAIN(...)                       \
  do {                                       \
    if (rc == KHR_OK) rc = (__VA_ARGS__);    \
  } while (0)

struct FrameSlot {
  float* depth = nullptr;
  float* range = nullptr;
  uint32_t* rgba = nullptr;
  int32_t* label = nullptr;
  int32_t* dyn = nullptr;
  uint8_t* dynw = nullptr;
  int32_t* obj = nullptr;
  uint8_t* rgb_staging = nullptr;
  float* tile_max = nullptr;
  const float* x_depth = nullptr;
  const float* x_range = nullptr;
  const uint32_t* x_rgba = nullptr;
  const int32_t* x_label = nullptr;
  const float* x_tile_max = nullptr;
  const float* vDepth() const { return x_depth ? x_depth : depth; }
  const float* vRange() const { return x_range ? x_range : range; }
  const uint32_t* vRgba() const { return x_rgba ? x_rgba : rgba; }
  const int32_t* vLabel() const { return x_label ? x_label : label; }
  const float* vTileMax() const { return x_tile_max ? x_tile_max : tile_max; }
  int tw = 0, th = 0;
  khr_sensor sensor{};
  khr_frame meta{};
  bool valid = false, has_color = false, has_label = false, has_obj = false, objects_done = false;
  bool dyn_clean = false;
  bool dynw_valid = false;
  uint64_t aux_seq = 0;
  std::vector<khr_cluster> sem_clusters;
  std::vector<khr_cluster> clusters;
};

struct TimingRec {
  int which;
  Event a, b;
};

constexpr int kNumTimers = 13;
constexpr uint32_t kObjHead = 512;
constexpr uint32_t kCvHead = 8192;
constexpr int kGvReleaseGrid = 64;
constexpr uint32_t kCompCap = 1024, kCompHead = 64;

}

struct khr_ctx {
  khr_config cfg{};
  DevParams p{};
  DevMap m{};
  int device = 0;
  Stream stream;
  Stream aux_stream;
  Stream copy_stream;
  Stream snap_stream;
  Stream mc_stream;
  Stream h2d_stream;
  Event ev_aux, ev_aux_done;
  uint64_t aux_seq_issued = 0, aux_seq_done = 0, obj_seq = 0, cv_seq[3] = {0, 0, 0};
  std::vector<DevBuf<uint8_t>> allocs;
  std::vector<FrameSlot> slots;
  int next_slot = 0;
  std::unique_ptr<std::atomic<int>[]> slot_leases;
  uint32_t* d_work = nullptr;
  uint32_t* d_new = nullptr;
  uint32_t* d_ef = nullptr;
  uint32_t* d_trk_proc = nullptr;
  uint32_t* d_tick_work = nullptr;
  uint32_t* d_tick_counts = nullptr;
  uint32_t* d_tick_seeds = nullptr;
  PinnedBuf<uint32_t> h_tick;
  uint32_t tick_ticket = 0;
  std::vector<uint32_t> tick_seed_host;
  int tick_seed_n = 0, tick_seed_collected = 0;
  int tick_epoch = 0, motion_ignore_epoch = 0;
  unsigned long long* d_dbg = nullptr;
  unsigned long long* d_digest = nullptr;
  uint32_t* d_wg_stats = nullptr;
  bool fold_pending = false;
  int stream_priority = 0;
  unsigned char* d_fuse_sink = nullptr;
  DevBuf<uint32_t> d_pix_scratch;
  DevBuf<uint8_t> d_inst;
  uint4* d_work4 = nullptr;
  uint4* d_tick_work4 = nullptr;
  FuseFrame* d_tick_frames = nullptr;
  uint32_t* d_tick_mask = nullptr;
  bool tick_mask_dirty = false;
  uint32_t item_cap = 0;
  struct SnapArena {
    DevBuf<uint8_t> buf;
    PinnedBuf<uint32_t> count;
    volatile uint32_t* h_count() const { return count.get(); }
    int alloc(size_t bytes) {
      if (buf.alloc(bytes)) return fail(KHR_ENOMEM, "snapshot arena of %zu bytes", bytes);
      if (count.alloc(16)) {
        buf.reset();
        return fail(KHR_ENOMEM, "snapshot pinned words");
      }
      count[0] = count[1] = 0;
      return KHR_OK;
    }
  };
  struct SnapPool {
    std::mutex mu;
    std::vector<SnapArena> free;
    bool dead = false;
  };
  std::shared_ptr<SnapPool> snap_pool = std::make_shared<SnapPool>();
// ... 491 lines not shown
static std::vector<khr_ctx*> g_live_ctx;
static int createStream(khr_ctx* c, Stream& out) {
  int lo = 0, hi = 0;
  if (hipDeviceGetStreamPriorityRange(&lo, &hi) != hipSuccess || lo == hi || c->stream_priority == 0)
    return out.create(hipStreamNonBlocking);
  const int prio = c->stream_priority > 0 ? hi : lo;
  return out.create(hipStreamNonBlocking, &prio);
}

static bool ctxIsLive(khr_ctx* c) {
  std::lock_guard<std::mutex> lock(g_live_mu);
  return std::find(g_live_ctx.begin(), g_live_ctx.end(), c) != g_live_ctx.end();
}

int khr_release_slot(khr_ctx* c, int slot) {
  if (!c) return fail(KHR_EINVAL, "bad slot");
  std::lock_guard<std::mutex> live_lock(g_live_mu);
  if (std::find(g_live_ctx.begin(), g_live_ctx.end(), c) == g_live_ctx.end())
    return KHR_OK;
  if (slot < 0 || slot >= static_cast<int>(c->slots.size())) return fail(KHR_EINVAL, "bad slot");
  int cur = c->slot_leases[slot].load(std::memory_order_acquire);
  while (cur > 0)
    if (c->slot_leases[slot].compare_exchange_weak(cur, cur - 1, std::memory_order_acq_rel, std::memory_order_acquire)) return KHR_OK;
  return fail(KHR_ESTATE, "slot %d was not retained", slot);
}

int khr_depend_on(khr_ctx* c, khr_ctx* other) {
  if (!c || !other) return fail(KHR_EINVAL, "null ctx");
  if (c->device != other->device) return fail(KHR_EINVAL, "contexts live on different devices");
  HIP_TRY(hipSetDevice(c->device));
  KHR_TRY(c->ev_dep_aux.ensure());
  if (c->stream == other->stream) {
    HIP_TRY(hipEventRecord(c->ev_dep_aux, other->aux_stream));
    HIP_TRY(hipStreamWaitEvent(c->stream, c->ev_dep_aux, 0));
    c->dep_src = other;
    return KHR_OK;
  }
  KHR_TRY(c->ev_dep.ensure());
  HIP_TRY(hipEventRecord(c->ev_dep, other->stream));
  HIP_TRY(hipStreamWaitEvent(c->stream, c->ev_dep, 0));
  HIP_TRY(hipEventRecord(c->ev_dep_aux, other->aux_stream));
  HIP_TRY(hipStreamWaitEvent(c->stream, c->ev_dep_aux, 0));
  c->dep_src = other;
  return KHR_OK;
}

int khr_reset_map(khr_ctx* c, float voxel_size, float truncation_distance) {
  if (!c) return fail(KHR_EINVAL, "null ctx");
  if (!(voxel_size > 0.f) || !(truncation_distance > 0.f)) return fail(KHR_EINVAL, "voxel_size / truncation_distance must be > 0");
  HIP_TRY(hipSetDevice(c->device));
  c->cfg.voxel_size = voxel_size;
  c->cfg.truncation_distance = truncation_distance;
  deriveMetricParams(c->cfg, c->p);
  const size_t n = std::max<size_t>(static_cast<size_t>(c->m.ht_mask) + 1, c->m.capacity);
  hipLaunchKernelGGL(k_reset_map, dim3(gridFor(n)), dim3(256), 0, c->stream, c->m);
  HIP_TRY(hipGetLastError());
  c->mesh_cur = 0;
  c->mesh_total = 0;
  c->mesh_stale = false;
  c->host_index_valid = false, ++c->map_gen;
  c->explicit_blocks = 0;
  c->last_removed = 0;
  c->removed_pending = false;
  c->last_track_stamp = 0;
  c->dep_src = nullptr;
  c->halo_n = 0;
  c->mh_n = 0;
  c->stats = khr_stats{};
  for (auto& s : c->slots) {
    s.valid = false;
    s.clusters.clear();
    s.sem_clusters.clear();
  }
  for (size_t i = 0; i < c->slots.size(); ++i) c->slot_leases[i].store(0);
  return KHR_OK;
}

int khr_get_config(khr_ctx* c, khr_config* out) {
  if (!c || !out) return fail(KHR_EINVAL, "null argument");
  *out = c->cfg;
  return KHR_OK;
}

int khr_create(const khr_config* cfg, khr_ctx** out) {
  if (!cfg || !out) return fail(KHR_EINVAL, "null argument");
  *out = nullptr;
  if (!(cfg->voxel_size > 0.f) || !(cfg->truncation_distance > 0.f)) return fail(KHR_EINVAL, "voxel_size / truncation_distance must be > 0");
  if (cfg->voxels_per_side != 16 && cfg->voxels_per_side != 8) return fail(KHR_EINVAL, "voxels_per_side must be 8 or 16");
  auto conn_ok = [](int c) { return c == 6 || c == 18 || c == 26; };
  if (!conn_ok(cfg->neighbor_connectivity) || !conn_ok(cfg->md_neighbor_connectivity)) return fail(KHR_EINVAL, "neighbor_connectivity must be one of {6, 18, 26}");
  if (!(cfg->temporal_buffer > 0.f) || !(cfg->temporal_window > 0.f)) return fail(KHR_EINVAL, "temporal_buffer / temporal_window must be > 0");
  if (cfg->tsdf_occupancy_threshold == 0.f) return fail(KHR_EINVAL, "tsdf_occupancy_threshold must be != 0");
  if (cfg->md_max_cluster_size < cfg->md_min_cluster_size) return fail(KHR_EINVAL, "param 'max_cluster_size' must be >= 'min_cluster_size'");
  if (!(cfg->md_max_range > 0.f)) return fail(KHR_EINVAL, "md_max_range must be > 0");
  if (cfg->with_semantics && cfg->num_labels < 1) return fail(KHR_EINVAL, "num_labels must be >= 1 with semantics");
  if (cfg->semantic_mode == 1 && cfg->with_semantics && cfg->num_labels != 2) return fail(KHR_EINVAL, "binary semantic integrator needs num_labels == 2");
  if (cfg->max_blocks < 1 || cfg->max_frame_pixels < 1 || cfg->num_frame_slots < 1) return fail(KHR_EINVAL, "capacities must be >= 1");
  if (cfg->world_size < 1 || cfg->rank < 0 || cfg->rank >= cfg->world_size) return fail(KHR_EINVAL, "bad rank / world_size");

  int ndev = 0;
  if (hipGetDeviceCount(&ndev) != hipSuccess || ndev == 0)
    return fail(KHR_EDEVICE, "no HIP device available: the khronos_amd fusion path has no CPU fallback");
  if (cfg->device < 0 || cfg->device >= ndev) return fail(KHR_EINVAL, "device %d out of range (%d devices)", cfg->device, ndev);
  HIP_TRY(hipSetDevice(cfg->device));

  std::unique_ptr<khr_ctx, void (*)(khr_ctx*)> owner(new khr_ctx(), khr_destroy);
  khr_ctx* c = owner.get();
  c->cfg = *cfg;
  c->device = cfg->device;
  {
    static const bool prio_off = std::getenv("KHR_STREAM_PRIORITY") && std::atoi(std::getenv("KHR_STREAM_PRIORITY")) == 0;
    static const int prio_window = std::getenv("KHR_WINDOW_PRIORITY") ? std::atoi(std::getenv("KHR_WINDOW_PRIORITY")) : 0;
    c->stream_priority = prio_off ? 0 : (cfg->voxels_per_side == 8 ? -1 : prio_window);
  }
  if (createStream(c, c->stream)) return fail(KHR_EDEVICE, "hipStreamCreate failed");
  if (createStream(c, c->aux_stream) || c->ev_aux.ensure() || c->ev_aux_done.ensure())
    return fail(KHR_EDEVICE, "auxiliary stream / event creation failed");
  if (c->h_pinned.alloc(16) || c->ev_seed.ensure()) return fail(KHR_EDEVICE, "pinned scratch / event creation failed");
  std::memset(c->h_pinned, 0, 64);
  if (ensureStage(c, 1u << 20) != KHR_OK ||
      c->h_up.alloc(std::max<size_t>(1u << 16, cfg->voxels_per_side == 8 ? sizeof(int32_t) * 3 * static_cast<size_t>(cfg->max_blocks) : 0)))
    return fail(KHR_ENOMEM, "pinned staging buffers");

  DevParams& p = c->p;
  deriveMetricParams(*cfg, p);
  p.vps = cfg->voxels_per_side;
  p.nvox = p.vps * p.vps * p.vps;
  p.K = cfg->with_semantics ? cfg->num_labels : 1;
  p.KS = cfg->packed_likelihood_rows ? p.K : likStride(p.K);
  p.with_semantics = cfg->with_semantics;
  p.with_tracking = cfg->with_tracking;
  p.use_dropoff = cfg->use_weight_dropoff;
  p.const_weight = cfg->use_constant_weight;
  p.interp = cfg->interpolation_method;
  p.range_mode = cfg->range_mode;
  p.sem_mode = cfg->semantic_mode;
  p.max_weight = cfg->max_weight;
  p.adaptive_diff = cfg->adaptive_max_range_difference;
  p.log_match = std::log(cfg->label_confidence);
  p.log_nomatch = cfg->num_labels > 1 ? std::log((1.f - cfg->label_confidence) / static_cast<float>(cfg->num_labels - 1)) : 0.f;
  p.temporal_buffer = static_cast<double>(cfg->temporal_buffer);
  p.temporal_window = static_cast<double>(cfg->temporal_window);
  p.nn = cfg->neighbor_connectivity;
  p.mesh_min_weight = cfg->mesh_min_weight;
  p.mesh_eps = cfg->mesh_degenerate_eps > 0.f ? cfg->mesh_degenerate_eps : 1e-6f;
  p.mesh_attr_source = cfg->mesh_attr_source;
  p.alloc_candidate = cfg->alloc_candidate;
  p.rank = cfg->rank;
  p.world = cfg->world_size;
  p.dbg = std::getenv("KHR_DEBUG") ? std::atoi(std::getenv("KHR_DEBUG")) : 0;

  DevMap& m = c->m;
  const size_t cap = cfg->max_blocks, nv = p.nvox;
  uint32_t ht = 1;
  while (ht < cap * 4) ht <<= 1;
  m.ht_mask = ht - 1;
  m.capacity = static_cast<uint32_t>(cap);
  int rc = KHR_OK;
  KHR_CHAIN(devAlloc(c, &m.ht_keys, ht, false));
  KHR_CHAIN(devAlloc(c, &m.ht_vals, ht));
  KHR_CHAIN(devAlloc(c, &m.blk_index, cap));
  KHR_CHAIN(devAlloc(c, &m.blk_flags, cap));
  KHR_CHAIN(devAlloc(c, &m.dist, cap * nv, false));
  KHR_CHAIN(devAlloc(c, &m.weight, cap * nv, false));
  KHR_CHAIN(devAlloc(c, &m.color, cap * nv, false));
  KHR_CHAIN(devAlloc(c, &m.vflags, cap * nv, false));
  KHR_CHAIN(devAlloc(c, &m.sem_label, cfg->with_semantics ? cap * nv : 1, false));
  if (rc == KHR_OK && devAlloc(c, &m.lik, cfg->with_semantics ? cap * nv * p.KS : 1, false) != KHR_OK) {
    fail(KHR_ENOMEM, "the label-likelihood layer of %zu blocks needs %.2f GB (%d floats per voxel%s); khr_config.packed_likelihood_rows = 1 "
                     "stores %d per voxel, a smaller max_blocks less of everything", static_cast<size_t>(cap),
         1e-9 * static_cast<double>(cap) * nv * p.KS * 4, p.KS, p.KS != p.K ? ": rows padded to 128-byte lines" : "", p.K);
    KHR_CHAIN(KHR_ENOMEM);
  }
  KHR_CHAIN(devAlloc(c, &m.last_obs, cfg->with_tracking ? cap * nv : 1, false));
  KHR_CHAIN(devAlloc(c, &m.last_occ, cfg->with_tracking ? cap * nv : 1, false));
  KHR_CHAIN(devAlloc(c, &m.trk_lim, cfg->with_tracking ? cap * 2 : 2));
  KHR_CHAIN(devAlloc(c, &m.freebits, cfg->with_tracking ? cap * (nv / 64) : 1, false));
  KHR_CHAIN(devAlloc(c, &m.obs, cfg->with_tracking ? cap * (nv / 64) : 1, false));
  KHR_CHAIN(devAlloc(c, &m.free_slots, cap, false));
  KHR_CHAIN(devAlloc(c, &m.counters, C_COUNT));
  KHR_CHAIN(devAlloc(c, &m.stats, S_COUNT));
  KHR_CHAIN(devAlloc(c, &m.mesh_desc, cap));
  KHR_CHAIN(devAlloc(c, &c->d_work, cap));
  KHR_CHAIN(devAlloc(c, &c->d_new, cap));
  KHR_CHAIN(devAlloc(c, &c->d_ef, cap));
  KHR_CHAIN(devAlloc(c, &c->d_trk_proc, cap));
  KHR_CHAIN(devAlloc(c, &c->d_dbg, 4096 * 4 * 12));
  KHR_CHAIN(devAlloc(c, &c->d_digest, kDigestWords));
  KHR_CHAIN(devAlloc(c, &c->d_wg_stats, 2 * kUpdateStatSlots));
  KHR_CHAIN(devAlloc(c, &c->d_fuse_sink, static_cast<size_t>(kUpdateStatSlots) * 16 * 256, false));
  KHR_CHAIN(devAlloc(c, &c->d_fetch_done, 4));
  {
    const int zs = (cfg->voxels_per_side != 8 && (cfg->world_size >= 4 || cfg->max_frame_pixels <= 640u * 480u)) ? 8 : 4;
    c->fuse_zsplit = zs;
    c->wpb = static_cast<uint32_t>((cfg->voxels_per_side * cfg->voxels_per_side / 64) * zs);
    c->item_cap = static_cast<uint32_t>(cap) * c->wpb;
  }
  KHR_CHAIN(devAlloc(c, &c->d_work4, 2 * static_cast<size_t>(c->item_cap), false));
  if (cfg->voxels_per_side == 8 && rc == KHR_OK) {
    const size_t bits_words = static_cast<size_t>(c->item_cap) * 4;
    if (c->h_frames.alloc(kMaxMultiFrames) || c->d_frames.alloc(kMaxMultiFrames) || c->ev_frames.ensure() ||
        hipEventRecord(c->ev_frames, c->stream) != hipSuccess || c->d_frame_bits.alloc(bits_words) ||
        c->d_multi_list.alloc(2 * static_cast<size_t>(c->item_cap) + 1))
      rc = fail(KHR_ENOMEM, "buffers of the multi-frame update");
    if (rc == KHR_OK && (c->h_totals.alloc(C_COUNT + 2) || c->ev_up.ensure() || hipEventRecord(c->ev_up, c->stream) != hipSuccess ||
                         c->ev_dep.ensure() || c->ev_dep_aux.ensure()))
      rc = fail(KHR_ENOMEM, "page-locked words / events of an object mini-map");
  }
  KHR_CHAIN(devAlloc(c, &m.blk_band, cap * kBandSlots));
  KHR_CHAIN(devAlloc(c, &c->d_removed, cap));
  KHR_CHAIN(devAlloc(c, &c->d_mesh_count, cap + 1));
  KHR_CHAIN(devAlloc(c, &c->d_mesh_offset, cap + 1));
  KHR_CHAIN(devAlloc(c, &c->d_regen, cap));
  KHR_CHAIN(devAlloc(c, &c->d_mesh_old_off, cap + 1));
  KHR_CHAIN(devAlloc(c, &c->d_mh_flag, cap));
  KHR_CHAIN(devAlloc(c, &c->d_mesh_nwork, 8));
  const size_t npx = cfg->max_frame_pixels;
  KHR_CHAIN(devAlloc(c, &c->d_keys, npx, false));
  KHR_CHAIN(devAlloc(c, &c->d_pix, npx, false));
  {
    uint32_t ts = 1;
    while (ts < 2 * npx) ts <<= 1;
    c->md_mask = ts - 1;
    c->md_list_cap = static_cast<uint32_t>(std::min<size_t>(npx, 1u << 20));
    KHR_CHAIN(devAlloc(c, &c->d_md_keys, 3 * static_cast<size_t>(ts), false));
    KHR_CHAIN(devAlloc(c, &c->d_md_counts, 3 * static_cast<size_t>(ts), false));
    KHR_CHAIN(devAlloc(c, &c->d_md_ids, 3 * static_cast<size_t>(ts), false));
    {
      uint8_t* head = nullptr;
      KHR_CHAIN(devAlloc(c, &head, 16 + sizeof(CompAcc) * kCompCap));
      c->d_md_n = reinterpret_cast<uint32_t*>(head);
    }
    KHR_CHAIN(devAlloc(c, &c->d_md_parent, c->md_list_cap, false));
    KHR_CHAIN(devAlloc(c, &c->d_md_rootidx, c->md_list_cap, false));
    KHR_CHAIN(devAlloc(c, &c->d_md_edges, c->md_list_cap, false));
    KHR_CHAIN(devAlloc(c, &c->d_md_comp_acc, c->md_list_cap, false));
    KHR_CHAIN(devAlloc(c, &c->d_md_comp_final, kCompCap));
    KHR_CHAIN(c->h_md_head.alloc(16 + sizeof(CompAcc) * kCompCap));
    KHR_CHAIN(devAlloc(c, &c->d_md_scratch4, 16));
    c->md_host_walk = std::getenv("KHR_MD_HOST_WALK") != nullptr;
    if (const char* e = std::getenv("KHR_MD_LDS_MAX")) c->md_lds_max = std::min<uint32_t>(kCompLds, static_cast<uint32_t>(std::atoi(e)));
    KHR_CHAIN(devAlloc(c, &c->d_md_seed_keys, c->md_list_cap, false));
    KHR_CHAIN(devAlloc(c, &c->d_md_bnd_keys, c->md_list_cap, false));
    KHR_CHAIN(devAlloc(c, &c->d_md_seed_counts, c->md_list_cap, false));
    KHR_CHAIN(devAlloc(c, &c->d_md_bnd_counts, c->md_list_cap, false));
    KHR_CHAIN(devAlloc(c, &c->d_md_seed_final, c->md_list_cap, false));
    KHR_CHAIN(devAlloc(c, &c->d_md_bnd_final, c->md_list_cap, false));
    KHR_CHAIN(devAlloc(c, &c->d_md_bnd_deg, c->md_list_cap, false));
    KHR_CHAIN(devAlloc(c, &c->d_md_bnd_mask, c->md_list_cap, false));
    KHR_CHAIN(devAlloc(c, &c->d_md_adj, static_cast<size_t>(c->md_list_cap) * 26, false));
    KHR_CHAIN(c->h_md_walk.alloc(std::min<size_t>(c->md_list_cap, 16384) * (3 + 26 + 3 + 3) + 16));
    KHR_CHAIN(devAlloc(c, &c->d_md_acc, 256, false));
    KHR_CHAIN(c->h_md_acc_pinned.alloc(256));
    {
      std::vector<ClusterAcc> init(256);
      for (auto& a : init) clusterAccReset(a);
      KHR_CHAIN(hipMemcpy(c->d_md_acc, init.data(), sizeof(ClusterAcc) * 256, hipMemcpyHostToDevice) != hipSuccess ? KHR_EDEVICE : KHR_OK);
    }
  }
  if (rc == KHR_OK) {
    size_t t3 = 0;
    hipcub::DeviceScan::ExclusiveSum(nullptr, t3, c->d_mesh_count, c->d_mesh_offset, static_cast<int>(cap + 1), c->stream);
    c->cub_temp_bytes = t3 + 256;
    uint8_t* tmp = nullptr;
    KHR_CHAIN(devAlloc(c, &tmp, c->cub_temp_bytes, false));
    c->d_cub_temp = tmp;
  }
  for (int b = 0; b < 2 && rc == KHR_OK; ++b) {
    KHR_CHAIN(devAlloc(c, &c->mesh[b].points, cfg->max_mesh_vertices * 3, false));
    KHR_CHAIN(devAlloc(c, &c->mesh[b].colors, cfg->max_mesh_vertices, false));
    KHR_CHAIN(devAlloc(c, &c->mesh[b].labels, cfg->max_mesh_vertices, false));
    KHR_CHAIN(devAlloc(c, &c->mesh[b].stamps, cfg->max_mesh_vertices, false));
  }
  c->slots.resize(cfg->num_frame_slots);
  c->slot_leases.reset(new std::atomic<int>[cfg->num_frame_slots]);
  for (uint32_t i = 0; i < cfg->num_frame_slots; ++i) c->slot_leases[i].store(0);
  for (auto& s : c->slots) {
    if (rc != KHR_OK) break;
    KHR_CHAIN(devAlloc(c, &s.depth, npx, false));
    KHR_CHAIN(devAlloc(c, &s.range, npx + 4, false));
    KHR_CHAIN(devAlloc(c, &s.rgba, npx + 4, false));
    KHR_CHAIN(devAlloc(c, &s.label, npx, false));
    KHR_CHAIN(devAlloc(c, &s.dyn, npx));
    KHR_CHAIN(devAlloc(c, &s.dynw, npx, false));
    KHR_CHAIN(devAlloc(c, &s.obj, npx));
    KHR_CHAIN(devAlloc(c, &s.rgb_staging, npx * 3, false));
    KHR_CHAIN(devAlloc(c, &s.tile_max, npx / 16 + 64, false));
  }
  if (rc != KHR_OK) return rc;
  hipError_t e = hipMemsetAsync(m.ht_keys, 0xff, sizeof(uint64_t) * ht, c->stream);
  if (e == hipSuccess) {
    std::vector<uint32_t> ident(cap);
    for (size_t i = 0; i < cap; ++i) ident[i] = static_cast<uint32_t>(i);
    e = hipMemcpyAsync(m.free_slots, ident.data(), sizeof(uint32_t) * cap, hipMemcpyHostToDevice, c->stream);
    uint32_t ctr[C_COUNT] = {0};
    ctr[C_N_FREE] = static_cast<uint32_t>(cap);
    if (e == hipSuccess) e = hipMemcpyAsync(m.counters, ctr, sizeof(ctr), hipMemcpyHostToDevice, c->stream);
    if (e == hipSuccess) e = hipMemcpyToSymbol(HIP_SYMBOL(g_mc_tri), kMcTriTable, sizeof(kMcTriTable));
    if (e == hipSuccess) e = hipMemcpyToSymbol(HIP_SYMBOL(g_mc_ntri), kMcNumTris, sizeof(kMcNumTris));
    if (e == hipSuccess) e = hipStreamSynchronize(c->stream);
  }
  if (e != hipSuccess) return fail(KHR_EDEVICE, "context initialisation failed: %s", hipGetErrorString(e));
  {
    std::lock_guard<std::mutex> lock(g_live_mu);
    g_live_ctx.push_back(c);
  }
  *out = owner.release();
  return KHR_OK;
}

void khr_destroy(khr_ctx* c) {
  if (!c) return;
  {
    std::lock_guard<std::mutex> lock(g_live_mu);
    g_live_ctx.erase(std::remove(g_live_ctx.begin(), g_live_ctx.end(), c), g_live_ctx.end());
  }
  hipSetDevice(c->device);
  for (Stream* st : {&c->stream, &c->aux_stream, &c->h2d_stream, &c->snap_stream, &c->mc_stream, &c->copy_stream})
    if (*st) hipStreamSynchronize(*st);
  resolveTimers(c);
  if (c->pending_snapshot) khr_snapshot_release(c->pending_snapshot);
  {
    std::lock_guard<std::mutex> lock(c->snap_pool->mu);
    c->snap_pool->dead = true;
    c->snap_pool->free.clear();
  }
  {
    std::lock_guard<std::mutex> lock(c->frame_pool->mu);
    c->frame_pool->dead = true;
    c->frame_pool->free.clear();
  }
  delete c;
}

int khr_set_stream(khr_ctx* c, void* hip_stream) {
  if (!c) return fail(KHR_EINVAL, "null ctx");
  HIP_TRY(hipStreamSynchronize(c->stream));
  HIP_TRY(hipStreamSynchronize(c->aux_stream));
  if (hip_stream) {
    c->stream.refer(static_cast<hipStream_t>(hip_stream));
    return KHR_OK;
  }
  return createStream(c, c->stream);
}

int khr_sync(khr_ctx* c) {
  if (!c) return fail(KHR_EINVAL, "null ctx");
  HIP_TRY(hipStreamSynchronize(c->stream));
  HIP_TRY(hipStreamSynchronize(c->aux_stream));
  return KHR_OK;
}

static int auxAfterMain(khr_ctx* c) {
  HIP_TRY(hipEventRecord(c->ev_aux, c->stream));
  HIP_TRY(hipStreamWaitEvent(c->aux_stream, c->ev_aux, 0));
  return KHR_OK;
}

static int peekSlot(const khr_ctx* c) {
  const int n_slots = static_cast<int>(c->slots.size());
  for (int k = 0; k < n_slots; ++k) {
    const int cand = (c->next_slot + k) % n_slots;
    if (c->slot_leases[cand].load(std::memory_order_acquire) == 0) return cand;
  }
  return -1;
}

static int acquireSlot(khr_ctx* c) {
  const int n_slots = static_cast<int>(c->slots.size());
  int slot = -1;
  for (int k = 0; k < n_slots && slot < 0; ++k) {
    const int cand = (c->next_slot + k) % n_slots;
    if (c->slot_leases[cand].load(std::memory_order_acquire) == 0) slot = cand;
  }
  if (slot < 0) return fail(KHR_ENOMEM, "all %d frame slots are retained (raise num_frame_slots)", n_slots);
  c->next_slot = (slot + 1) % n_slots;
  if (c->slots[slot].aux_seq > c->aux_seq_done) {
    const uint64_t upto = c->aux_seq_issued;
    if (hipStreamQuery(c->aux_stream) != hipSuccess) HIP_TRY(hipStreamSynchronize(c->aux_stream));
    c->aux_seq_done = upto;
  }
  c->slots[slot].aux_seq = 0;
  FrameSlot& fs = c->slots[slot];
  fs.x_depth = fs.x_range = nullptr, fs.x_rgba = nullptr, fs.x_label = nullptr, fs.x_tile_max = nullptr;
  return slot;
}

static bool validSlot(const khr_ctx* c, int slot) {
  return slot >= 0 && slot < static_cast<int>(c->slots.size()) && c->slots[slot].valid;
}

static int checkSensor(const khr_ctx* c, const khr_sensor* sensor) {
  const size_t n = static_cast<size_t>(sensor->width) * sensor->height;
  if (sensor->width < 2 || sensor->height < 2 || n > c->cfg.max_frame_pixels)
    return fail(KHR_EINVAL, "frame %dx%d exceeds max_frame_pixels=%u", sensor->width, sensor->height, c->cfg.max_frame_pixels);
  if (!(sensor->fx > 0.f) || !(sensor->fy > 0.f) || !(sensor->max_range > sensor->min_range))
    return fail(KHR_EINVAL, "bad intrinsics / range");
  return KHR_OK;
}

static FrameSlot& newFrameSlot(khr_ctx* c, int slot, const khr_sensor& sensor, const khr_frame& meta, bool has_color, bool has_label,
                               bool valid) {
  FrameSlot& s = c->slots[slot];
  s.valid = valid;
  s.sensor = sensor;
  s.meta = meta;
  s.meta.depth = nullptr;
  s.meta.color = nullptr;
  s.meta.label = nullptr;
  s.has_color = has_color;
  s.has_label = has_label;
  s.has_obj = false;
  if (c->obj_cv_slot == slot) c->obj_cv_slot = -1;
  s.objects_done = false;
  s.clusters.clear();
  s.sem_clusters.clear();
  s.tw = (sensor.width + kTile - 1) / kTile;
  s.th = (sensor.height + kTile - 1) / kTile;
  s.dyn_clean = true, s.dynw_valid = false;
  return s;
}

struct IngestOpts {
  hipStream_t stream = nullptr;
  bool pinned = false;
  Event* h2d_event = nullptr;
  bool begin = false;
};

static int uploadFrame(khr_ctx* c, const khr_sensor* sensor, const khr_frame* frame, int on_device, const IngestOpts& opts) {
  if (!c || !sensor || !frame || !frame->depth) return fail(KHR_EINVAL, "null argument");
  KHR_TRY(checkSensor(c, sensor));
  const size_t n = static_cast<size_t>(sensor->width) * sensor->height;
  HIP_TRY(hipSetDevice(c->device));
  const int slot = acquireSlot(c);
  if (slot < 0) return slot;
  const hipMemcpyKind kind = on_device ? hipMemcpyDeviceToDevice : hipMemcpyHostToDevice;
  FrameSlot& s = newFrameSlot(c, slot, *sensor, *frame, frame->color != nullptr, frame->label != nullptr, false);
  const bool pinned = !on_device && opts.pinned;
  hipStream_t ist = ((on_device || pinned) && opts.stream) ? opts.stream : static_cast<hipStream_t>(c->stream);
  Event& evh = opts.h2d_event ? *opts.h2d_event : c->ev_h2d;
  ScopedTimer tm(c, ist == c->stream ? 6 : -1);
  const float* depth_src = frame->depth;
  const uint8_t* rgb_src = frame->color;
  const int32_t* label_src = frame->label;
  if (!on_device) {
    hipStream_t cs = c->stream;
    if (pinned) {
      if (!c->h2d_stream) KHR_TRY(createStream(c, c->h2d_stream));
      KHR_TRY(evh.ensure());
      cs = c->h2d_stream;
      if (ist == c->stream) {
        KHR_TRY(c->ev_ingest.ensure());
        HIP_TRY(hipEventRecord(c->ev_ingest, c->stream));
        HIP_TRY(hipStreamWaitEvent(cs, c->ev_ingest, 0));
      }
    }
    HIP_TRY(hipMemcpyAsync(s.depth, frame->depth, n * sizeof(float), kind, cs));
    depth_src = s.depth;
    if (frame->color) {
      HIP_TRY(hipMemcpyAsync(s.rgb_staging, frame->color, n * 3, kind, cs));
      rgb_src = s.rgb_staging;
    }
    if (frame->label) {
      HIP_TRY(hipMemcpyAsync(s.label, frame->label, n * sizeof(int32_t), kind, cs));
      label_src = s.label;
    }
    if (pinned) {
      HIP_TRY(hipEventRecord(evh, cs));
      HIP_TRY(hipStreamWaitEvent(ist, evh, 0));
      if (!opts.h2d_event) c->h2d_pending = true;
      c->h2d_bytes += n * (4u + (frame->color ? 3u : 0u) + (frame->label ? 4u : 0u));
    }
  }
  hipLaunchKernelGGL(k_frame_ingest, dim3(s.tw * s.th), dim3(256), 0, ist, depth_src, rgb_src, label_src, s.depth,
                     s.range, s.rgba, s.label, s.dyn, s.tile_max, s.tw, sensor->width, sensor->height, sensor->fx, sensor->fy,
                     sensor->cx, sensor->cy, c->p.range_mode, c->m, c->p.nvox, c->d_wg_stats, opts.begin ? 1 : 0);
  HIP_TRY(hipGetLastError());
  c->begun = opts.begin;
  if (!on_device && !pinned) HIP_TRY(hipStreamSynchronize(c->stream));
  s.valid = true;
  return slot;
}

int khr_upload_frame(khr_ctx* c, const khr_sensor* sensor, const khr_frame* frame, int on_device) {
  return uploadFrame(c, sensor, frame, on_device, IngestOpts{});
}

int khr_set_frame_image(khr_ctx* c, int slot, int which, const int32_t* image, int on_device) {
  if (!c || !validSlot(c, slot)) return fail(KHR_EINVAL, "bad slot");
  FrameSlot& s = c->slots[slot];
  const size_t n = static_cast<size_t>(s.sensor.width) * s.sensor.height;
  int32_t* dst = which == 0 ? s.dyn : s.obj;
  if (image) {
    HIP_TRY(hipMemcpyAsync(dst, image, n * sizeof(int32_t), on_device ? hipMemcpyDeviceToDevice : hipMemcpyHostToDevice, c->stream));
    if (!on_device) HIP_TRY(hipStreamSynchronize(c->stream));
  } else {
    HIP_TRY(hipMemsetAsync(dst, 0, n * sizeof(int32_t), c->stream));
  }
  if (which == 1) s.has_obj = image != nullptr;
  if (which == 1 && c->obj_cv_slot == slot) c->obj_cv_slot = -1;
  if (which == 0) s.dyn_clean = image == nullptr;
  if (which == 0) s.dynw_valid = false;
  if (which == 1) {
    const int rca = auxAfterMain(c);
    if (rca) return rca;
  }
  return KHR_OK;
}

int khr_download_frame(khr_ctx* c, int slot, float* range, float* vertex_map, int32_t* dynamic_image) {
  if (!c || !validSlot(c, slot)) return fail(KHR_EINVAL, "bad slot");
  FrameSlot& s = c->slots[slot];
  const size_t n = static_cast<size_t>(s.sensor.width) * s.sensor.height;
  if (range) HIP_TRY(hipMemcpyAsync(range, s.vRange(), n * sizeof(float), hipMemcpyDeviceToHost, c->stream));
  if (dynamic_image) HIP_TRY(hipMemcpyAsync(dynamic_image, s.dyn, n * sizeof(int32_t), hipMemcpyDeviceToHost, c->stream));
  if (vertex_map) {
    DevTemp tmpv;
    KHR_TRY(tmpv.alloc(n * 3 * sizeof(float)));
    float* d_v = tmpv.as<float>();
    hipLaunchKernelGGL(k_vertex_map, dim3(gridFor(n)), dim3(256), 0, c->stream, makeDevFrame(c, s), d_v);
    HIP_TRY(hipMemcpyAsync(vertex_map, d_v, n * 3 * sizeof(float), hipMemcpyDeviceToHost, c->stream));
    HIP_TRY(hipStreamSynchronize(c->stream));
  }
  HIP_TRY(hipStreamSynchronize(c->stream));
  return KHR_OK;
}

struct khr_frame_copy {
  std::shared_ptr<khr_ctx::FramePool> pool;
  DevBuf<uint8_t> block;
  int device = 0;
  Event ready;
  DevFrame f{};
  size_t n = 0, n_pad = 0;
};

int khr_frame_copy_create(khr_ctx* c, int slot, khr_frame_copy** out) {
  if (!c || !out || !validSlot(c, slot)) return fail(KHR_EINVAL, "bad argument");
  HIP_TRY(hipSetDevice(c->device));
  FrameSlot& s = c->slots[slot];
  const size_t n = static_cast<size_t>(s.sensor.width) * s.sensor.height, n_pad = (n + 3) / 4 * 4;
  if (n_pad > c->cfg.max_frame_pixels) return fail(KHR_EINVAL, "frame larger than max_frame_pixels");
  auto fc = std::make_unique<khr_frame_copy>();
  fc->pool = c->frame_pool;
  fc->device = c->device;
  const size_t bytes = 16 * n_pad;
  {
    std::lock_guard<std::mutex> lock(c->frame_pool->mu);
    auto& fr = c->frame_pool->free;
    for (size_t i = 0; i < fr.size(); ++i)
      if (fr[i].count() >= bytes) {
        fc->block = std::move(fr[i]);
        fr.erase(fr.begin() + static_cast<long>(i));
        break;
      }
  }
  if (!fc->block && fc->block.alloc(bytes)) return fail(KHR_ENOMEM, "frame copy (%zu bytes)", bytes);
  if (fc->ready.ensure()) return fail(KHR_EDEVICE, "event");
  if (s.aux_seq) HIP_TRY(hipStreamWaitEvent(c->stream, c->ev_aux_done, 0));
  hipLaunchKernelGGL(k_frame_copy, dim3(512), dim3(256), 0, c->stream, reinterpret_cast<const uint4*>(s.vDepth()),
                     reinterpret_cast<const uint4*>(s.vRange()), s.has_color ? reinterpret_cast<const uint4*>(s.vRgba()) : nullptr,
                     s.has_label ? reinterpret_cast<const uint4*>(s.vLabel()) : nullptr, reinterpret_cast<uint4*>(fc->block.get()),
                     static_cast<uint32_t>(n_pad / 4));
  HIP_TRY(hipGetLastError());
  HIP_TRY(hipEventRecord(fc->ready, c->stream));
  fc->f = makeDevFrame(c, s);
  fc->f.depth = reinterpret_cast<const float*>(fc->block.get());
  fc->f.range = reinterpret_cast<const float*>(fc->block + 4 * n_pad);
  fc->f.rgba = reinterpret_cast<const uint32_t*>(fc->block + 8 * n_pad);
  fc->f.label = reinterpret_cast<const int32_t*>(fc->block + 12 * n_pad);
  fc->f.dyn = nullptr;
  fc->f.obj = nullptr;
  fc->n = n;
  fc->n_pad = n_pad;
  *out = fc.release();
  return KHR_OK;
}

int khr_frame_copy_download(khr_frame_copy* fc, float* depth, float* range, uint8_t* color_rgb, int32_t* labels, float* vertex_map) {
  if (!fc) return fail(KHR_EINVAL, "null frame copy");
  HIP_TRY(hipSetDevice(fc->device));
  HIP_TRY(hipEventSynchronize(fc->ready));
  const size_t n = fc->n;
  if (depth) HIP_TRY(hipMemcpy(depth, fc->f.depth, n * 4, hipMemcpyDeviceToHost));
  if (range) HIP_TRY(hipMemcpy(range, fc->f.range, n * 4, hipMemcpyDeviceToHost));
  if (labels) HIP_TRY(hipMemcpy(labels, fc->f.label, n * 4, hipMemcpyDeviceToHost));
  if (color_rgb || vertex_map) {
    DevTemp tmp;
    KHR_TRY(tmp.alloc(n * 12));
    if (color_rgb) {
      hipLaunchKernelGGL(k_rgba_to_rgb, dim3(static_cast<unsigned>((n + 255) / 256)), dim3(256), 0, nullptr, fc->f.rgba, tmp.as<uint8_t>(), static_cast<uint32_t>(n));
      HIP_TRY(hipMemcpy(color_rgb, tmp.get(), n * 3, hipMemcpyDeviceToHost));
    }
    if (vertex_map) {
      hipLaunchKernelGGL(k_vertex_map, dim3(static_cast<unsigned>((n + 255) / 256)), dim3(256), 0, nullptr, fc->f, tmp.as<float>());
      HIP_TRY(hipMemcpy(vertex_map, tmp.get(), n * 12, hipMemcpyDeviceToHost));
    }
  }
  return KHR_OK;
}

void khr_frame_copy_release(khr_frame_copy* fc) {
  if (!fc) return;
  hipSetDevice(fc->device);
  if (fc->ready) hipEventSynchronize(fc->ready);
  {
    std::lock_guard<std::mutex> lock(fc->pool->mu);
    if (!fc->pool->dead && fc->pool->free.size() < 8) fc->pool->free.push_back(std::move(fc->block));
  }
  delete fc;
}

int khr_copy_frame_image(khr_ctx* c, int slot, int which, void* device_dst) {
  if (!c || !device_dst || !validSlot(c, slot)) return fail(KHR_EINVAL, "bad argument");
  if (which != 0 && which != 1) return fail(KHR_EINVAL, "which must be 0 (dynamic) or 1 (object)");
  HIP_TRY(hipSetDevice(c->device));
  FrameSlot& s = c->slots[slot];
  const size_t n = static_cast<size_t>(s.sensor.width) * s.sensor.height;
  if (which == 1 && !s.has_obj) {
    HIP_TRY(hipMemsetAsync(device_dst, 0, n * sizeof(int32_t), c->stream));
    return KHR_OK;
  }
  if (which == 1) {
    HIP_TRY(hipEventRecord(c->ev_aux_done, c->aux_stream));
    HIP_TRY(hipStreamWaitEvent(c->stream, c->ev_aux_done, 0));
  }
  HIP_TRY(hipMemcpyAsync(device_dst, which == 0 ? s.dyn : s.obj, n * sizeof(int32_t), hipMemcpyDeviceToDevice, c->stream));
  return KHR_OK;
}

int khr_download_frame_image(khr_ctx* c, int slot, int which, int32_t* image) {
  if (!c || !image || !validSlot(c, slot)) return fail(KHR_EINVAL, "bad argument");
  if (which != 0 && which != 1) return fail(KHR_EINVAL, "which must be 0 (dynamic) or 1 (object)");
  FrameSlot& s = c->slots[slot];
  const size_t n = static_cast<size_t>(s.sensor.width) * s.sensor.height;
  if (which == 1 && !s.has_obj) {
    std::memset(image, 0, n * sizeof(int32_t));
    return KHR_OK;
  }
  if (which == 1) HIP_TRY(hipStreamSynchronize(c->aux_stream));
  HIP_TRY(hipMemcpyAsync(image, which == 0 ? s.dyn : s.obj, n * sizeof(int32_t), hipMemcpyDeviceToHost, c->stream));
  HIP_TRY(hipStreamSynchronize(c->stream));
  return KHR_OK;
}

static int integrateAlloc(khr_ctx* c, FrameSlot& s, const DevFrame& f, int allocate_blocks) {
  DevMap& m = c->m;
  if (!c->begun) hipLaunchKernelGGL(k_begin_integrate, dim3(1), dim3(256), 0, c->stream, m, c->p.nvox, c->d_wg_stats);
  c->begun = false;
  if (allocate_blocks) {
    ScopedTimer tm(c, 3);
    const DevFrustum fr = makeFrustum(c, f);
    const int S = 2 * fr.n_steps + 1;
    const size_t total = static_cast<size_t>(S) * S * S;
    hipLaunchKernelGGL(k_alloc_visible, dim3(gridFor(total)), dim3(256), 0, c->stream, m, c->p, f, fr, c->d_work, c->d_new,
                       c->h_pinned.dev() + 2, c->seed_publish_pending ? c->seed_ticket : 0u, &m.counters[C_N_VISIBLE], 0);
    c->seed_publish_pending = false;
    hipLaunchKernelGGL(k_init_cull, dim3(1024 + 1024), dim3(256), 0, c->stream, m, c->p, f, c->d_new, c->d_work,
                       FuseList{c->d_work4, c->d_work4 + c->item_cap, c->item_cap, &m.counters[C_N_ITEMS0]}, c->wpb,
                       c->cfg.disable_culling ? nullptr : s.vTileMax(), s.tw, s.th, 1024u);
    c->host_index_valid = false, ++c->map_gen;
  } else {
    hipLaunchKernelGGL(k_list_live, dim3(gridFor(m.capacity)), dim3(256), 0, c->stream, m, c->d_work,
                       &m.counters[C_N_VISIBLE], 0u, FuseList{c->d_work4, c->d_work4 + c->item_cap, c->item_cap, &m.counters[C_N_ITEMS0]},
                       c->wpb);
  }
  HIP_TRY(hipGetLastError());
  return KHR_OK;
}

struct UpdateLists {
  FuseList list{nullptr, nullptr, 0u, nullptr};
};

static int fuseGrid(khr_ctx* c, const void* kernel, int group, int block) {
  static std::map<std::pair<int, const void*>, int> cache;
  static std::mutex cache_mu;
  std::lock_guard<std::mutex> lock(cache_mu);
  const std::pair<int, const void*> key{c->device, kernel};
  auto it = cache.find(key);
  if (it != cache.end()) return it->second;
  int per_cu = 0, cus = 256;
  if (hipOccupancyMaxActiveBlocksPerMultiprocessor(&per_cu, kernel, block, 0) != hipSuccess || per_cu < 1) per_cu = 1;
  per_cu = std::min(per_cu, std::max(1, kUpdateWavesPerCu / (block / 64)));
  hipDeviceProp_t prop;
  if (hipGetDeviceProperties(&prop, c->device) == hipSuccess && prop.multiProcessorCount > 0) cus = prop.multiProcessorCount;
  per_cu = std::min(per_cu, 8);
  int grid = std::min(kUpdateStatSlots, per_cu * cus);
  grid = std::max(8 * group, grid / (8 * group) * (8 * group));
  cache[key] = grid;
  return grid;
}

static int fuse2Grid(khr_ctx* c, const void* kern, int wpw) {
  static std::map<std::pair<int, const void*>, int> cache;
  static std::mutex mu;
  std::lock_guard<std::mutex> lock(mu);
  const std::pair<int, const void*> key{c->device, kern};
  auto it = cache.find(key);
  if (it != cache.end()) return it->second;
  int per_cu = 0;
  if (hipOccupancyMaxActiveBlocksPerMultiprocessor(&per_cu, kern, 64 * wpw, 0) != hipSuccess || per_cu < 1) per_cu = 1;
  hipDeviceProp_t prop;
  int cus = 256;
  if (hipGetDeviceProperties(&prop, c->device) == hipSuccess && prop.multiProcessorCount > 0) cus = prop.multiProcessorCount;
  const int grid = std::min(kUpdateStatSlots, per_cu * cus) / 8 * 8;
  cache[key] = grid;
  return grid;
}

static void fillFuseFrame(const khr_ctx* c, const FrameSlot& s, const DevFrame& f, int use_mask, int object_id, FuseFrame* a) {
  a->range = f.range; a->dyn = f.dyn; a->rgba = f.rgba; a->label = f.label; a->obj = f.obj;
  a->W = f.W; a->H = f.H; a->fx = f.fx; a->fy = f.fy; a->cx = f.cx; a->cy = f.cy; a->min_range = f.min_range; a->max_range = f.max_range;
  std::memcpy(a->R, f.R, sizeof(a->R));
  std::memcpy(a->t, f.t, sizeof(a->t));
  a->stamp = f.stamp;
  a->use_mask = (use_mask && !s.dyn_clean) ? 1 : 0;
  a->has_color = f.has_color;
  a->object_id = object_id;
  a->do_sem = (c->p.with_semantics && ((c->p.sem_mode == 1) ? (object_id >= 0 && f.obj != nullptr) : (f.has_label != 0))) ? 1 : 0;
  a->tile_max = s.vTileMax();
  a->tw = s.tw;
  a->th = s.th;
}
static void fillFuseMap(khr_ctx* c, FuseArgs* a) {
  DevMap& m = c->m;
  a->blk_index = m.blk_index; a->blk_flags = m.blk_flags; a->dist = m.dist; a->weight = m.weight; a->last_obs = m.last_obs; a->obs = m.obs;
  a->color = m.color; a->vflags = m.vflags; a->sem_label = m.sem_label; a->lik = m.lik; a->wg_stats = c->d_wg_stats;
  a->blk_band = m.blk_band;
  a->vs = c->p.vs; a->bs = c->p.bs; a->trunc = c->p.trunc; a->dropoff_eps = c->p.dropoff_eps; a->max_weight = c->p.max_weight;
  a->adaptive_diff = c->p.adaptive_diff; a->log_match = c->p.log_match; a->log_nomatch = c->p.log_nomatch;
  a->interp = c->p.interp; a->range_mode = c->p.range_mode; a->use_dropoff = c->p.use_dropoff; a->const_weight = c->p.const_weight;
  a->with_tracking = c->p.with_tracking;
  a->K = c->p.K; a->KS = c->p.KS; a->sem_mode = c->p.sem_mode;
  a->band_mode = c->cfg.max_frame_pixels <= 640u * 480u ? 0 : 1;
  a->sink = c->d_fuse_sink;
  a->blend_pre = c->cfg.color_blend_weight != 0;
}

static int integrateUpdateMulti(khr_ctx* c, khr_ctx* src, const int* src_slots, const int* object_ids, int n_frames, int use_mask) {
  if (c->cfg.voxels_per_side != 8 || n_frames < 2 || n_frames > kMaxMultiFrames) return 1;
  FuseArgs a{};
  fillFuseMap(c, &a);
  const bool defcfg = a.range_mode == 0 && a.interp == 2 && a.use_dropoff && !a.const_weight;
  if (!defcfg) return 1;
  if (!c->h_frames) {
    if (c->h_frames.alloc(kMaxMultiFrames) || c->d_frames.alloc(kMaxMultiFrames)) return fail(KHR_ENOMEM, "frame argument staging");
    KHR_TRY(c->ev_frames.ensure());
  } else {
    HIP_TRY(hipEventSynchronize(c->ev_frames));
  }
  for (int i = 0; i < n_frames; ++i) {
    FrameSlot& s = src->slots[src_slots[i]];
    const DevFrame f = makeDevFrame(src, s);
    fillFuseFrame(c, s, f, use_mask, object_ids ? object_ids[i] : -1, &c->h_frames[i]);
  }
  {
    const uint32_t n_words = static_cast<uint32_t>(sizeof(FuseFrame) / 4) * static_cast<uint32_t>(n_frames);
    hipLaunchKernelGGL(k_copy_words, dim3((n_words + 255) / 256), dim3(256), 0, c->stream, reinterpret_cast<const uint32_t*>(c->h_frames.dev()),
                       reinterpret_cast<uint32_t*>(c->d_frames.get()), n_words);
  }
  HIP_TRY(hipEventRecord(c->ev_frames, c->stream));
  static_cast<FuseFrame&>(a) = c->h_frames[0];
  a.frames = c->d_frames;
  a.n_frames = n_frames;
  if (c->item_cap > 0) {
    const int n_words = (n_frames + 31) / 32;
    const size_t need = static_cast<size_t>(c->item_cap) * static_cast<size_t>(n_words);
    if (need > c->d_frame_bits.count()) {
      const size_t want = static_cast<size_t>(c->item_cap) * static_cast<size_t>((n_words + 3) / 4 * 4);
      HIP_TRY(hipStreamSynchronize(c->stream));
      if (c->d_frame_bits.reserve(want)) return fail(KHR_ENOMEM, "frame bits of the multi-frame update (%zu bytes)", want * sizeof(uint32_t));
    }
    const uint64_t tests = static_cast<uint64_t>(c->explicit_blocks > 0 ? std::min<uint64_t>(c->explicit_blocks, c->m.capacity) : c->m.capacity) *
                           c->wpb * static_cast<uint64_t>(n_words) * 32u;
    const unsigned grid = static_cast<unsigned>(std::min<uint64_t>((tests + 255) / 256, 8192));
    hipLaunchKernelGGL((k_multi_cull<8>), dim3(std::max(1u, grid)), dim3(256), 0, c->stream, c->m.blk_flags, c->m.blk_index, &c->m.counters[C_MAX_SLOT],
                       c->p.vs, c->p.bs, c->p.trunc, static_cast<const FuseFrame*>(c->d_frames.get()), n_frames, n_words, c->wpb, BLK_LIVE, c->d_frame_bits);
    HIP_TRY(hipGetLastError());
    a.frame_bits = c->d_frame_bits;
    a.frame_words = n_words;
  }
  FuseList list{c->d_work4, c->d_work4 + c->item_cap, c->item_cap, &c->m.counters[C_N_ITEMS0]};
  if (a.frame_bits != nullptr) {
    if (!c->d_multi_list) {
      HIP_TRY(hipStreamSynchronize(c->stream));
      if (c->d_multi_list.alloc(2 * static_cast<size_t>(c->item_cap) + 1)) return fail(KHR_ENOMEM, "item list of the multi-frame update");
    }
    uint32_t* const counts = reinterpret_cast<uint32_t*>(c->d_multi_list + 2 * static_cast<size_t>(c->item_cap));
    HIP_TRY(hipMemsetAsync(counts, 0, 16, c->stream));
    list = FuseList{c->d_multi_list, c->d_multi_list + c->item_cap, c->item_cap, counts};
    const uint64_t n_it = static_cast<uint64_t>(c->explicit_blocks > 0 ? std::min<uint64_t>(c->explicit_blocks, c->m.capacity) : c->m.capacity) * c->wpb;
    hipLaunchKernelGGL(k_multi_order, dim3(static_cast<unsigned>((n_it + 1023) / 1024)), dim3(1024), 0, c->stream, c->m.blk_flags, c->m.blk_index,
                       &c->m.counters[C_MAX_SLOT], static_cast<const uint32_t*>(c->d_frame_bits.get()), a.frame_words, n_frames, c->wpb, BLK_LIVE, list);
    HIP_TRY(hipGetLastError());
  }
  constexpr int WPW = 8;
  auto go = [&](auto kern) {
    int grid = fuse2Grid(c, reinterpret_cast<const void*>(kern), WPW);
    if (c->explicit_blocks > 0) {
      const uint64_t items = c->explicit_blocks * c->wpb;
      grid = std::max(8, static_cast<int>(std::min<uint64_t>(static_cast<uint64_t>(grid), (items + WPW - 1) / WPW) + 7) / 8 * 8);
    }
    for (int k0 = 0; k0 < n_frames; k0 += kMultiChunk) {
      a.frames = c->d_frames + k0;
      a.n_frames = std::min(kMultiChunk, n_frames - k0);
      a.frame_bit0 = k0;
      KHR_LAUNCH_TIMED(0, kern, dim3(grid), dim3(64 * WPW), a, list);
    }
  };
  const bool object_map = c->p.with_semantics && a.sem_mode == 1 && a.K == 2 && a.KS == 2 && !a.with_tracking;
  if (object_map) {
    if (exactArithmetic(c)) go(&k_fuse_obj<true, WPW, 4>);
    else go(&k_fuse_obj<false, WPW, 4>);
  } else {
    if (exactArithmetic(c)) go(&k_fuse2<8, 4, true, WPW, 4>);
    else go(&k_fuse2<8, 4, false, WPW, 4>);
  }
  HIP_TRY(hipGetLastError());
  return KHR_OK;
}

static int integrateUpdate(khr_ctx* c, FrameSlot& s, const DevFrame& f, int allocate_blocks, int use_mask,
                           int object_id, bool defer_fold, const UpdateLists* lists = nullptr, const uint32_t* gate = nullptr) {
  DevMap& m = c->m;
  FuseList list{c->d_work4, c->d_work4 + c->item_cap, c->item_cap, &m.counters[C_N_ITEMS0]};
  if (lists) list = lists->list;
  FuseArgs a{};
  fillFuseMap(c, &a);
  fillFuseFrame(c, s, f, use_mask, object_id, &a);
  const bool defcfg = a.range_mode == 0 && a.interp == 2 && a.use_dropoff && !a.const_weight;
  const bool exact = exactArithmetic(c);
  int rc = dispatchVps(c, [&](auto vps) {
    constexpr int V = decltype(vps)::value;
    auto launch = [&](auto zsplit) {
      constexpr int ZS = decltype(zsplit)::value;
      constexpr int G = 1;
      auto go = [&](auto kern, int wpw) {
        int grid = fuseGrid(c, reinterpret_cast<const void*>(kern), G, 64 * wpw);
        if (!allocate_blocks && c->explicit_blocks > 0) {
          const uint64_t items = c->explicit_blocks * c->wpb;
          const int want = static_cast<int>(std::min<uint64_t>(static_cast<uint64_t>(grid), (items + wpw - 1) / wpw));
          grid = std::max(8, (want + 7) / 8 * 8);
        }
        static bool said = false;
        if (!said && std::getenv("KHR_VERBOSE")) { said = true; std::fprintf(stderr, "[khr] k_fuse<%d,%d> %d waves / workgroup, grid %d\n", V, ZS, wpw, grid); }
        KHR_LAUNCH_TIMED(0, kern, dim3(grid), dim3(64 * wpw), a, list);
        if (defer_fold) c->fold_pending = true;
        else hipLaunchKernelGGL(k_fuse_fold, dim3((c->m.capacity + 255) / 256), dim3(256), 0, c->stream, m.blk_flags, m.blk_band,
                                &m.counters[C_MAX_SLOT], gate);
      };
      a.gate = gate;
      constexpr int WD = kUpdateWpw;
      if (defcfg && !exact) {
        go(&k_fuse<V, ZS, true, false, WD>, WD);
      } else if (defcfg) {
        go(&k_fuse<V, ZS, true, true, WD>, WD);
      } else {
        go(&k_fuse<V, ZS, false, true, WD>, WD);
      }
    };
    const int zs = c->fuse_zsplit;
    if (V == 8) {
      launch(std::integral_constant<int, 4>());
    } else {
      if (zs == 8) launch(std::integral_constant<int, (V == 16 ? 8 : 4)>());
      else launch(std::integral_constant<int, 4>());
    }
    return KHR_OK;
  });
  if (rc) return rc;
  HIP_TRY(hipGetLastError());
  return KHR_OK;
}

int khr_integrate(khr_ctx* c, int slot, int allocate_blocks, int use_mask, int object_id) {
  if (!c || !validSlot(c, slot)) return fail(KHR_EINVAL, "bad slot");
  HIP_TRY(hipSetDevice(c->device));
  FrameSlot& s = c->slots[slot];
  const DevFrame f = makeDevFrame(c, s);
  if (object_id >= 0 && s.has_obj) {
    HIP_TRY(hipEventRecord(c->ev_aux_done, c->aux_stream));
    HIP_TRY(hipStreamWaitEvent(c->stream, c->ev_aux_done, 0));
  }
  int rc = integrateAlloc(c, s, f, allocate_blocks);
  if (rc) return rc;
  return integrateUpdate(c, s, f, allocate_blocks, use_mask, object_id, false);
}

int khr_integrate_shared(khr_ctx* c, khr_ctx* src, int src_slot, int allocate_blocks, int use_mask, int object_id) {
  if (!c || !src || !validSlot(src, src_slot)) return fail(KHR_EINVAL, "bad source slot");
  if (c->device != src->device) return fail(KHR_EINVAL, "contexts live on different devices");
  HIP_TRY(hipSetDevice(c->device));
  if (c->dep_src != src) {
    if (c->stream != src->stream) HIP_TRY(hipStreamSynchronize(src->stream));
    HIP_TRY(hipStreamSynchronize(src->aux_stream));
  }
  FrameSlot& s = src->slots[src_slot];
  const DevFrame f = makeDevFrame(src, s);
  int rc = integrateAlloc(c, s, f, allocate_blocks);
  if (rc) return rc;
  return integrateUpdate(c, s, f, allocate_blocks, use_mask, object_id, false);
}

int khr_integrate_shared_batch(khr_ctx* c, khr_ctx* src, const int* src_slots, const int* object_ids, int n_frames,
                               int allocate_blocks, int use_mask) {
  if (!c || !src || !src_slots || n_frames < 0) return fail(KHR_EINVAL, "bad argument");
  for (int i = 0; i < n_frames; ++i)
    if (!validSlot(src, src_slots[i])) return fail(KHR_EINVAL, "bad source slot");
// ... 2113 lines not shown
  HIP_TRY(hipSetDevice(c->device));
  std::vector<std::array<int32_t, 3>> v(n);
  for (int64_t i = 0; i < n; ++i) v[i] = {indices[3 * i], indices[3 * i + 1], indices[3 * i + 2]};
  std::sort(v.begin(), v.end());
  v.erase(std::unique(v.begin(), v.end()), v.end());
  const size_t bytes = sizeof(int32_t) * 3 * v.size();
  HT("ab_enter");
  if (c->ev_up) HIP_TRY(hipEventSynchronize(c->ev_up));
  KHR_TRY(c->ev_up.ensure());
  HT("ab_prev_upload_consumed");
  if (bytes > c->h_up.count()) {
    HIP_TRY(hipStreamSynchronize(c->stream));
    const size_t want = std::max<size_t>(2 * bytes, 1u << 16);
    if (c->h_up.reserve(want)) return fail(KHR_ENOMEM, "block index staging of %zu bytes", want);
  }
  std::memcpy(c->h_up, v.data(), bytes);
  HIP_TRY(hipMemsetAsync(&c->m.counters[C_N_NEW], 0, sizeof(uint32_t), c->stream));
  c->explicit_blocks += v.size();
  hipLaunchKernelGGL(k_alloc_list, dim3(gridFor(v.size())), dim3(256), 0, c->stream, c->m, static_cast<const int*>(c->h_up.dev()),
                     static_cast<int>(v.size()), c->d_new);
  HIP_TRY(hipEventRecord(c->ev_up, c->stream));
  hipLaunchKernelGGL(k_init_blocks, dim3(2048), dim3(256), 0, c->stream, c->m, c->p, c->d_new);
  HIP_TRY(hipGetLastError());
  c->host_index_valid = false, ++c->map_gen;
  return KHR_OK;
}

int khr_object_prune(khr_ctx* c, float min_confidence, float min_observations, int64_t* n_pruned) {
  if (!c) return fail(KHR_EINVAL, "null ctx");
  if (!c->cfg.with_semantics || c->p.K < 2) return fail(KHR_ESTATE, "object pruning needs a binary semantic layer");
  HIP_TRY(hipMemsetAsync(&c->m.stats[S_PRUNED], 0, sizeof(unsigned long long), c->stream));
  int rc = dispatchVps(c, [&](auto vps) {
    hipLaunchKernelGGL((k_object_prune<decltype(vps)::value>), dim3(kStreamGrid), dim3(256), 0, c->stream, c->m, c->p,
                       min_confidence, min_observations);
    return KHR_OK;
  });
  if (rc) return rc;
  if (n_pruned) {
    unsigned long long np = 0;
    HIP_TRY(hipMemcpyAsync(&np, &c->m.stats[S_PRUNED], sizeof(np), hipMemcpyDeviceToHost, c->stream));
    HIP_TRY(hipStreamSynchronize(c->stream));
    *n_pruned = static_cast<int64_t>(np);
  }
  return KHR_OK;
}

static int refreshMeshTotals(khr_ctx* c);

int64_t khr_pool_exhausted(khr_ctx* c) {
  if (!c) return fail(KHR_EINVAL, "null ctx");
  const int rc = readCounters(c);
  if (rc) return rc;
  return static_cast<int64_t>(c->h_counters[C_POOL_EXHAUSTED]);
}

int khr_get_stats(khr_ctx* c, khr_stats* out) {
  if (!c || !out) return fail(KHR_EINVAL, "null argument");
  int rc = readCounters(c);
  if (rc) return rc;
  unsigned long long st[S_COUNT];
  HIP_TRY(hipMemcpy(st, c->m.stats, sizeof(st), hipMemcpyDeviceToHost));
  rc = ensureHostIndex(c);
  if (rc) return rc;
  rc = refreshMeshTotals(c);
  if (rc) return rc;
  khr_stats s = c->stats;
  s.n_allocated_blocks = c->host_index.size();
  s.n_visible_blocks = c->h_counters[C_N_VISIBLE];
  s.n_new_blocks = c->h_counters[C_N_NEW];
  s.n_visited_voxels = static_cast<uint64_t>(c->h_counters[C_N_VISIBLE]) * c->p.nvox;
  std::vector<uint32_t> wgs(2 * kUpdateStatSlots);
  HIP_TRY(hipMemcpy(wgs.data(), c->d_wg_stats, sizeof(uint32_t) * wgs.size(), hipMemcpyDeviceToHost));
  uint64_t cur_upd = 0, cur_band = 0;
  for (int i = 0; i < kUpdateStatSlots; ++i) {
    cur_upd += wgs[2 * i];
    cur_band += wgs[2 * i + 1];
  }
  s.n_updated_voxels = cur_upd;
  s.n_band_voxels = cur_band;
  s.n_tracking_updated_blocks = c->h_counters[c->ef_cur ? C_N_EF2 : C_N_EF_A];
  s.pool_exhausted = c->h_counters[C_POOL_EXHAUSTED];
  s.n_tsdf_blocks = c->h_counters[C_N_TSDF];
  s.n_fuse_items = static_cast<uint64_t>(c->h_counters[C_N_ITEMS0]) + c->h_counters[C_N_ITEMS1] + c->h_counters[C_N_ITEMS2] +
                   c->h_counters[C_N_ITEMS3];
  s.n_seed_waits = c->n_seed_waits;
  s.n_seed_waits_late = c->n_seed_waits_late;
  s.seed_wait_max_us = c->seed_wait_max_us;
  for (int i = 0; i < 8; ++i) s.seed_wait_hist[i] = c->seed_wait_hist[i];
  s.seed_wait_late_us = c->seed_wait_late_us;
  s.seed_wait_late_frame = c->seed_wait_late_frame;
  s.seed_wait_late_state = c->seed_wait_late_state;
  s.n_md_device_merges = c->n_md_device_merges;
  s.n_md_host_walks = c->n_md_host_walks;
  s.n_md_prelaunched = c->n_md_prelaunched;
  s.n_md_prelaunch_repeats = c->n_md_prelaunch_repeats;
  s.band_overflow = 0;
  s.n_tracking_processed_blocks = c->h_counters[c->ef_cur ? C_N_PROC2 : C_N_PROC];
  s.cum_updated_voxels = st[S_CUM_UPD] + cur_upd;
  s.cum_band_voxels = st[S_CUM_BAND] + cur_band;
  s.cum_visited_voxels = st[S_CUM_VISITED] + s.n_visited_voxels;
  s.cum_integrate_calls = st[S_CUM_CALLS];
  *out = s;
  return KHR_OK;
}

int64_t khr_num_blocks(khr_ctx* c) {
  if (!c) return fail(KHR_EINVAL, "null ctx");
  int rc = ensureHostIndex(c);
  if (rc) return rc;
  return static_cast<int64_t>(c->host_index.size());
}

int64_t khr_block_indices(khr_ctx* c, int32_t* out, int64_t cap, int only_updated) {
  if (!c) return fail(KHR_EINVAL, "null ctx");
  int rc = ensureHostIndex(c);
  if (rc) return rc;
  int64_t n = 0;
  for (auto& kv : c->host_index) {
    if (only_updated && !(c->host_flags[kv.second] & BLK_UPDATED)) continue;
    if (out && n < cap) {
      out[3 * n] = kv.first[0];
      out[3 * n + 1] = kv.first[1];
      out[3 * n + 2] = kv.first[2];
    }
    ++n;
  }
  return n;
}

int khr_download_block(khr_ctx* c, int32_t bx, int32_t by, int32_t bz, float* distance, float* weight,
                       uint8_t* color_rgba, uint64_t* last_observed, uint64_t* last_occupied, uint8_t* voxel_flags,
                       uint32_t* sem_label, float* likelihoods, uint8_t* block_flags) {
  if (!c) return fail(KHR_EINVAL, "null ctx");
  int rc = ensureHostIndex(c);
  if (rc) return rc;
  auto it = c->host_index.find({bx, by, bz});
  if (it == c->host_index.end()) return fail(KHR_ENOTFOUND, "block (%d,%d,%d) not allocated", bx, by, bz);
  const size_t slot = it->second, nv = c->p.nvox;
  const DevMap& m = c->m;
  auto D = [&](void* dst, const void* src, size_t bytes) { return hipMemcpyAsync(dst, src, bytes, hipMemcpyDeviceToHost, c->stream); };
  if (distance) HIP_TRY(D(distance, m.dist + slot * nv, nv * 4));
  if (weight) HIP_TRY(D(weight, m.weight + slot * nv, nv * 4));
  if (color_rgba) HIP_TRY(D(color_rgba, m.color + slot * nv, nv * 4));
  std::vector<uint8_t> raw_flags;
  if (voxel_flags || (last_occupied && c->cfg.with_tracking)) {
    raw_flags.resize(nv);
    HIP_TRY(D(raw_flags.data(), m.vflags + slot * nv, nv));
  }
  std::vector<uint64_t> obs_words;
  if (last_observed) {
    if (c->cfg.with_tracking) {
      HIP_TRY(D(last_observed, m.last_obs + slot * nv, nv * 8));
      obs_words.resize(2 * (nv / 64));
      HIP_TRY(D(obs_words.data(), m.obs + slot * (nv / 64), (nv / 64) * 16));
    } else std::memset(last_observed, 0, nv * 8);
  }
  if (last_occupied) {
    if (c->cfg.with_tracking) HIP_TRY(D(last_occupied, m.last_occ + slot * nv, nv * 8));
    else std::memset(last_occupied, 0, nv * 8);
  }
  if (sem_label) {
    if (c->cfg.with_semantics) HIP_TRY(D(sem_label, m.sem_label + slot * nv, nv * 4));
    else std::memset(sem_label, 0, nv * 4);
  }
  std::vector<float> lik_vm;
  if (likelihoods && c->cfg.with_semantics) {
    lik_vm.resize(nv * c->p.KS);
// ... 1646 lines not shown
```

Baseline: 4209.

## Certify free-space fuse items via per-tile min range and process them without projection

Computes a per-tile minimum range alongside the tile max during frame ingest. The cull kernel uses it to certify block items that lie entirely in front of all observed depths in their tiles, and sends them to a separate free-space list. The fuse kernel then handles that list with a simplified path that skips per-voxel image projection and sampling and just applies the truncated free-space update. This is meant to remove depth lookups and projection math for the many far-from-surface voxels at high resolution. It adds a tile-min reduction, a third item buffer and a second work loop, and it relies on the certification being conservative to preserve correctness.

Result: no change. 4172 (-0.9%).

```diff
diff --git a/include/khronos_amd.h b/include/khronos_amd.h
--- a/include/khronos_amd.h
+++ b/include/khronos_amd.h
@@ -114,6 +114,7 @@
   uint64_t n_md_host_walks;
   uint64_t n_md_prelaunched;
   uint64_t n_md_prelaunch_repeats;
+  uint64_t n_free_items;
 } khr_stats;
 
 typedef struct khr_cluster {
diff --git a/khronos_amd/capi.py b/khronos_amd/capi.py
--- a/khronos_amd/capi.py
+++ b/khronos_amd/capi.py
@@ -127,7 +127,7 @@
         "n_tracking_processed_blocks", "n_fuse_items", "n_seed_waits", "n_seed_waits_late", "seed_wait_max_us")] + [
         ("seed_wait_hist", C.c_uint64 * 8)] + [(n, C.c_uint64) for n in (
         "seed_wait_late_us", "seed_wait_late_frame", "seed_wait_late_state", "n_md_device_merges", "n_md_host_walks",
-        "n_md_prelaunched", "n_md_prelaunch_repeats")]
+        "n_md_prelaunched", "n_md_prelaunch_repeats", "n_free_items")]
 
 
 EXPORTS = [
diff --git a/khronos_amd/csrc/khr_device.h b/khronos_amd/csrc/khr_device.h
--- a/khronos_amd/csrc/khr_device.h
+++ b/khronos_amd/csrc/khr_device.h
@@ -43,6 +43,7 @@
   C_N_ITEMS1,
   C_N_ITEMS2,
   C_N_ITEMS3,
+  C_N_ITEMS_FREE,
   C_COUNT = 32
 };
 enum Stat64 : int { S_UPD = 0 , S_BAND , S_MESH_VERTS, S_PRUNED, S_CUM_UPD, S_CUM_BAND, S_CUM_VISITED, S_CUM_CALLS, S_COUNT = 8 };
@@ -84,6 +85,7 @@
   uint4* b;
   uint32_t cap;
   uint32_t* counts;
+  uint4* f;
 };
 __device__ inline uint32_t fuseClass(uint32_t band) { return band > 128u ? 0u : (band > 64u ? 1u : (band > 0u ? 2u : 3u)); }
 __device__ inline uint4* fuseDescPtr(const FuseList& l, uint32_t cls, uint32_t pos) {
@@ -338,6 +340,7 @@
     m.counters[C_N_ITEMS1] = 0u;
     m.counters[C_N_ITEMS2] = 0u;
     m.counters[C_N_ITEMS3] = 0u;
+    m.counters[C_N_ITEMS_FREE] = 0u;
   }
 }
 
diff --git a/khronos_amd/csrc/khr_kernels_fuse.h b/khronos_amd/csrc/khr_kernels_fuse.h
--- a/khronos_amd/csrc/khr_kernels_fuse.h
+++ b/khronos_amd/csrc/khr_kernels_fuse.h
@@ -61,6 +61,12 @@
   if (lane == 0) j = atomicAdd(s_q, 1u);
   j = static_cast<uint32_t>(__builtin_amdgcn_readfirstlane(static_cast<int>(j)));
   return first + gridDim.x * j;
+}
+typedef const FuseList __attribute__((address_space(4))) * FuseListK;
+__device__ __forceinline__ FuseListK kernargFuseList() {
+  const char __attribute__((address_space(4)))* kb = (const char __attribute__((address_space(4)))*)__builtin_amdgcn_kernarg_segment_ptr();
+  asm volatile("" : "+s"(kb));
+  return (FuseListK)(kb + ((sizeof(FuseArgs) + 7u) & ~static_cast<size_t>(7)));
 }
 __device__ __forceinline__ uint4 descOf(const FuseList& list, uint32_t nc0, uint32_t nc1, uint32_t nc2, uint32_t i) {
   const DescK la = (DescK)list.a, lb = (DescK)list.b;
@@ -356,6 +362,7 @@
   __shared__ uint32_t s_rec[WPW][5][kRecCap];
   __shared__ uint32_t s_stat[WPW][2];
   __shared__ uint32_t s_q;
+  __shared__ uint32_t s_qf;
   const int wave = __builtin_amdgcn_readfirstlane(static_cast<int>(threadIdx.x >> 6));
   const int lane = static_cast<int>(threadIdx.x & 63);
   const int range_mode = DEFCFG ? 0 : a.range_mode;
@@ -371,17 +378,14 @@
   const uint32_t n_items = list.counts[0] + list.counts[1] + list.counts[2] + list.counts[3];
   uint32_t n_upd = 0, n_band = 0;
   if (a.gate != nullptr && *a.gate != 0u) return;
-  if (threadIdx.x == 0) s_q = 0u;
+  if (threadIdx.x == 0) s_q = 0u, s_qf = 0u;
   __syncthreads();
   char* const sink_b = reinterpret_cast<char*>(a.sink) + (static_cast<size_t>(blockIdx.x) * WPW + static_cast<size_t>(wave)) * 256u;
   const bool trk = a.with_tracking != 0;
   const uint32_t first = firstListPos();
   auto pull = [&]() -> uint32_t { return pullListPos(&s_q, lane, first); };
   auto descOf = [&](uint32_t i) -> uint4 {
-    typedef const FuseList __attribute__((address_space(4))) * FuseListK;
-    const char __attribute__((address_space(4)))* kb = (const char __attribute__((address_space(4)))*)__builtin_amdgcn_kernarg_segment_ptr();
-    asm volatile("" : "+s"(kb));
-    const FuseListK kl = (FuseListK)(kb + ((sizeof(FuseArgs) + 7u) & ~static_cast<size_t>(7)));
+    const FuseListK kl = kernargFuseList();
     const uint32_t __attribute__((address_space(4)))* const kc = (const uint32_t __attribute__((address_space(4)))*)kl->counts;
     const uint32_t c0 = kc[0], c1 = c0 + kc[1], c2 = c1 + kc[2];
     const DescK la = (DescK)kl->a, lb = (DescK)kl->b;
@@ -433,6 +437,36 @@
     }
   };
 
+  auto stepStores = [&](char* const dist_b, char* const wgt_b, char* const lobs_b, ulonglong2* const obs_w, const uint32_t lin, const u4v ow_k,
+                        const bool ok, const float d_out, const float w_out, bool& touched) __attribute__((always_inline)) {
+      const unsigned long long m_ok = __builtin_amdgcn_ballot_w64(ok);
+      n_upd += static_cast<uint32_t>(__popcll(m_ok));
+      touched = touched || (m_ok != 0ull);
+      {
+        char* const d_b = m_ok != 0ull ? dist_b : sink_b;
+        char* const w_b = m_ok != 0ull ? wgt_b : sink_b;
+        const uint32_t vo = (m_ok != 0ull ? lin : static_cast<uint32_t>(lane)) * 4u;
+        *reinterpret_cast<float*>(d_b + vo) = d_out;
+        *reinterpret_cast<float*>(w_b + vo) = w_out;
+      }
+      {
+        const uint64_t bits0 = static_cast<uint64_t>(ow_k.x) | (static_cast<uint64_t>(ow_k.y) << 32);
+        const uint64_t stamp0 = static_cast<uint64_t>(ow_k.z) | (static_cast<uint64_t>(ow_k.w) << 32);
+        const bool same = stamp0 == a.stamp;
+        const uint64_t mat = (m_ok != 0ull && !same) ? (bits0 & ~m_ok) : 0ull;
+        const uint64_t nb = m_ok == 0ull ? bits0 : (same ? (bits0 | m_ok) : m_ok);
+        const uint64_t ns = m_ok == 0ull ? stamp0 : a.stamp;
+        const bool real = trk && mat != 0ull;
+        char* const st_b = real ? lobs_b : sink_b;
+        const uint32_t first_lin = lin - static_cast<uint32_t>(lane) + static_cast<uint32_t>(__builtin_ctzll(mat | (1ull << 63)));
+        const bool mine = ((mat >> static_cast<uint32_t>(lane)) & 1ull) != 0ull;
+        const uint32_t so = real ? (mine ? lin : first_lin) * 8u : 0u;
+        *reinterpret_cast<uint64_t*>(st_b + so) = stamp0;
+        ulonglong2* const wp = trk ? obs_w : reinterpret_cast<ulonglong2*>(sink_b + 16);
+        *wp = make_ulonglong2(nb, ns);
+      }
+  };
+
   auto phase2 = [&](FuseItem<VPS, ZR>& cur) {
     const size_t slot = cur.slot;
     char* const dist_b = reinterpret_cast<char*>(a.dist + slot * NV);
@@ -502,32 +536,7 @@
         ok = false;
       }
       }
-      const unsigned long long m_ok = __builtin_amdgcn_ballot_w64(ok);
-      n_upd += static_cast<uint32_t>(__popcll(m_ok));
-      touched = touched || (m_ok != 0ull);
-      {
-        char* const d_b = m_ok != 0ull ? dist_b : sink_b;
-        char* const w_b = m_ok != 0ull ? wgt_b : sink_b;
-        const uint32_t vo = (m_ok != 0ull ? lin : static_cast<uint32_t>(lane)) * 4u;
-        *reinterpret_cast<float*>(d_b + vo) = d_out;
-        *reinterpret_cast<float*>(w_b + vo) = w_out;
-      }
-      {
-        const uint64_t bits0 = static_cast<uint64_t>(ow_k.x) | (static_cast<uint64_t>(ow_k.y) << 32);
-        const uint64_t stamp0 = static_cast<uint64_t>(ow_k.z) | (static_cast<uint64_t>(ow_k.w) << 32);
-        const bool same = stamp0 == a.stamp;
-        const uint64_t mat = (m_ok != 0ull && !same) ? (bits0 & ~m_ok) : 0ull;
-        const uint64_t nb = m_ok == 0ull ? bits0 : (same ? (bits0 | m_ok) : m_ok);
-        const uint64_t ns = m_ok == 0ull ? stamp0 : a.stamp;
-        const bool real = trk && mat != 0ull;
-        char* const st_b = real ? lobs_b : sink_b;
-        const uint32_t first_lin = lin - static_cast<uint32_t>(lane) + static_cast<uint32_t>(__builtin_ctzll(mat | (1ull << 63)));
-        const bool mine = ((mat >> static_cast<uint32_t>(lane)) & 1ull) != 0ull;
-        const uint32_t so = real ? (mine ? lin : first_lin) * 8u : 0u;
-        *reinterpret_cast<uint64_t*>(st_b + so) = stamp0;
-        ulonglong2* const wp = trk ? (a.obs + w0 + k * PATCHES) : reinterpret_cast<ulonglong2*>(sink_b + 16);
-        *wp = make_ulonglong2(nb, ns);
-      }
+      stepStores(dist_b, wgt_b, lobs_b, a.obs + w0 + k * PATCHES, lin, ow_k, ok, d_out, w_out, touched);
     }
     const uint32_t item_band = cnt;
     if (__builtin_expect(cnt > 0u, 0)) {
@@ -580,6 +589,96 @@
         if (item_next >= n_items) break;
         item_next = item_nn;
         d_next = d_nn;
+      }
+    }
+  }
+  {
+    const FuseListK kl = kernargFuseList();
+    const DescK lf = (DescK)kl->f;
+    const uint32_t n_free = lf != nullptr ? ((const uint32_t __attribute__((address_space(4)))*)kl->counts)[4] : 0u;
+    struct FreeItem {
+      size_t slot;
+      int z0, sbi, lin_xy;
+      float oz, pxy2;
+      float d[ZR], w[ZR];
+    };
+    auto freeDesc = [&](uint32_t i) -> uint4 {
+      const u4v d = lf[i];
+      return make_uint4(d.x, d.y, d.z, d.w);
+    };
+    auto freeLoad = [&](FreeItem& it, const uint4 desc) {
+      const uint32_t dx = static_cast<uint32_t>(__builtin_amdgcn_readfirstlane(static_cast<int>(desc.x)));
+      it.slot = dx & 0xffffffu;
+      it.sbi = static_cast<int>(dx >> 24);
+      const int bx = __builtin_amdgcn_readfirstlane(static_cast<int>(desc.y));
+      const int by = __builtin_amdgcn_readfirstlane(static_cast<int>(desc.z));
+      const int bz = __builtin_amdgcn_readfirstlane(static_cast<int>(desc.w));
+      it.z0 = (it.sbi / PATCHES) * ZR;
+      const float ox = static_cast<float>(bx) * a.bs, oy = static_cast<float>(by) * a.bs;
+      it.oz = static_cast<float>(bz) * a.bs;
+      it.lin_xy = (it.sbi % PATCHES) * 64 + lane;
+      const int ix = it.lin_xy % VPS, iy = it.lin_xy / VPS;
+      const float px = ox + (static_cast<float>(ix) + 0.5f) * a.vs;
+      const float py = oy + (static_cast<float>(iy) + 0.5f) * a.vs;
+      it.pxy2 = a.R[6] * px + a.R[7] * py;
+      const char* const dist_b = reinterpret_cast<const char*>(a.dist + it.slot * NV);
+      const char* const wgt_b = reinterpret_cast<const char*>(a.weight + it.slot * NV);
+#pragma unroll
+      for (int k = 0; k < ZR; ++k) {
+        const uint32_t lin = static_cast<uint32_t>(it.lin_xy + (it.z0 + k) * SL);
+        it.d[k] = *reinterpret_cast<const float*>(dist_b + lin * 4u);
+        it.w[k] = *reinterpret_cast<const float*>(wgt_b + lin * 4u);
+      }
+    };
+    auto freeWork = [&](FreeItem& cur) {
+      const size_t slot = cur.slot;
+      char* const dist_b = reinterpret_cast<char*>(a.dist + slot * NV);
+      char* const wgt_b = reinterpret_cast<char*>(a.weight + slot * NV);
+      char* const lobs_b = reinterpret_cast<char*>(a.last_obs + slot * NV);
+      bool touched = false, wrote_neg = false;
+      const size_t w0 = slot * static_cast<size_t>(NV / 64) + static_cast<size_t>(cur.z0 * PATCHES + cur.sbi % PATCHES);
+#pragma unroll
+      for (int k = 0; k < ZR; ++k) {
+        const u4v ow_k = trk ? ((DescK)(a.obs + w0))[k * PATCHES] : u4v{0u, 0u, 0u, 0u};
+        const int iz = cur.z0 + k;
+        const uint32_t lin = static_cast<uint32_t>(cur.lin_xy + iz * SL);
+        const float pz = cur.oz + (static_cast<float>(iz) + 0.5f) * a.vs;
+        const float depth = (cur.pxy2 + a.R[8] * pz) + a.t[2];
+        bool ok = depth > 0.f;
+        ok = ok && !(depth < a.min_range || depth > a.max_range);
+        const float w = measurementWeight<EXACT>(a.vs, fxfy, depth, rcpRefined(depth), a.trunc, a.trunc, a.dropoff_eps, den, yden, use_dropoff, const_weight);
+        ok = ok && (w > 0.f);
+        const float d_old = cur.d[k], w_old = cur.w[k];
+        const VoxelAverage avg = runningAverage<EXACT>(d_old, w_old, a.trunc, w, a.trunc, a.max_weight);
+        wrote_neg = wrote_neg || (__builtin_amdgcn_ballot_w64(ok && avg.d_new < 0.f) != 0ull);
+        stepStores(dist_b, wgt_b, lobs_b, a.obs + w0 + k * PATCHES, lin, ow_k, ok, ok ? avg.d_new : d_old, ok ? avg.w_new : w_old, touched);
+      }
+      a.blk_band[slot * kBandSlots + (cur.sbi & (kBandSlots - 1))] = static_cast<uint16_t>((touched ? kItemTouched : 0u) | (wrote_neg ? kItemNeg : 0u));
+    };
+    auto pullFree = [&]() -> uint32_t { return pullListPos(&s_qf, lane, first); };
+    uint32_t fi = n_free != 0u ? pullFree() : 0xffffffffu;
+    if (fi < n_free) {
+      FreeItem fa, fb;
+      uint4 d_cur = freeDesc(fi);
+      freeLoad(fa, d_cur);
+      uint32_t fn = pullFree();
+      while (true) {
+        {
+          const uint4 d_next = fn < n_free ? freeDesc(fn) : d_cur;
+          freeLoad(fb, d_next);
+          freeWork(fa);
+          if (fn >= n_free) break;
+          d_cur = d_next;
+          fn = pullFree();
+        }
+        {
+          const uint4 d_next = fn < n_free ? freeDesc(fn) : d_cur;
+          freeLoad(fa, d_next);
+          freeWork(fb);
+          if (fn >= n_free) break;
+          d_cur = d_next;
+          fn = pullFree();
+        }
       }
     }
   }
diff --git a/khronos_amd/csrc/khr_kernels_fusion.h b/khronos_amd/csrc/khr_kernels_fusion.h
--- a/khronos_amd/csrc/khr_kernels_fusion.h
+++ b/khronos_amd/csrc/khr_kernels_fusion.h
@@ -11,7 +11,7 @@
                                   const int32_t* __restrict__ label_in, float* __restrict__ depth, float* __restrict__ range,
                                   uint32_t* __restrict__ rgba, int32_t* __restrict__ label, int32_t* __restrict__ dyn,
                                   float* __restrict__ tile_max, int tile, int tw, int W, int H, float fx, float fy, float cx,
-                                  float cy, int range_mode, float* d_out, float* r_out) {
+                                  float cy, int range_mode, float* d_out, float* r_out, float* __restrict__ tile_min = nullptr) {
   const int tx = tile % tw, ty = tile / tw;
   const int u = tx * kTile + (threadIdx.x & 15), v = ty * kTile + (threadIdx.x >> 4);
   float r = 0.f, d = 0.f;
@@ -36,13 +36,22 @@
   }
   *d_out = d;
   *r_out = r;
-  float rm = r;
-#pragma unroll
-  for (int o = 32; o > 0; o >>= 1) rm = fmaxf(rm, __shfl_down(rm, o));
-  __shared__ float s[4];
-  if ((threadIdx.x & 63) == 0) s[threadIdx.x >> 6] = rm;
+  float rm = r, rn = r;
+#pragma unroll
+  for (int o = 32; o > 0; o >>= 1) {
+    rm = fmaxf(rm, __shfl_down(rm, o));
+    rn = fminf(rn, __shfl_down(rn, o));
+  }
+  __shared__ float s[4], sn[4];
+  if ((threadIdx.x & 63) == 0) {
+    s[threadIdx.x >> 6] = rm;
+    sn[threadIdx.x >> 6] = rn;
+  }
   __syncthreads();
-  if (threadIdx.x == 0) tile_max[tile] = fmaxf(fmaxf(s[0], s[1]), fmaxf(s[2], s[3]));
+  if (threadIdx.x == 0) {
+    tile_max[tile] = fmaxf(fmaxf(s[0], s[1]), fmaxf(s[2], s[3]));
+    if (tile_min) tile_min[tile] = fminf(fminf(sn[0], sn[1]), fminf(sn[2], sn[3]));
+  }
 }
 
 __global__ __launch_bounds__(256) void k_frame_ingest(const float* __restrict__ depth_in,
@@ -50,14 +59,14 @@
                                                      const int32_t* __restrict__ label_in, float* __restrict__ depth,
                                                      float* __restrict__ range, uint32_t* __restrict__ rgba,
                                                      int32_t* __restrict__ label, int32_t* __restrict__ dyn,
-                                                     float* __restrict__ tile_max, int tw, int W, int H, float fx,
-                                                     float fy, float cx, float cy, int range_mode, DevMap m, int nvox,
+                                                     float* __restrict__ tile_max, float* __restrict__ tile_min, int tw, int W, int H,
+                                                     float fx, float fy, float cx, float cy, int range_mode, DevMap m, int nvox,
                                                      uint32_t* __restrict__ wg_stats, int do_begin) {
   if (blockIdx.x == 0 && threadIdx.x == 0) m.counters[C_N_SEEDS] = 0u;
   if (do_begin && blockIdx.x == 0) beginIntegrate(m, nvox, wg_stats);
   float d, r;
   ingestTile(depth_in, rgb_in, label_in, depth, range, rgba, label, dyn, tile_max, blockIdx.x, tw, W, H, fx, fy, cx, cy,
-             range_mode, &d, &r);
+             range_mode, &d, &r, tile_min);
 }
 
 struct TickIngest {
@@ -314,19 +323,23 @@
   if (threadIdx.x == 0) m.stats[S_CUM_CALLS] += extra_calls;
 }
 
+template <bool CERT = false>
 __device__ inline void cullBlocks(const DevMap& m, const DevParams& p, const DevFrame& f, const uint32_t* __restrict__ work,
                                   const uint32_t* __restrict__ n_work, FuseList out, uint32_t wpb,
                                   uint32_t* __restrict__ n_tsdf, const float* __restrict__ tile_max, int tw, int th,
-                                  uint32_t bid, uint32_t nblk, uint32_t* __restrict__ item_mask = nullptr, uint32_t cam = 0u) {
+                                  uint32_t bid, uint32_t nblk, uint32_t* __restrict__ item_mask = nullptr, uint32_t cam = 0u,
+                                  const float* __restrict__ tile_min = nullptr) {
   constexpr int kPerWg = 8;
   __shared__ uint4 s_blk[kPerWg];
-  __shared__ uint16_t s_item[4][kPerWg * kBandSlots];
-  __shared__ uint32_t s_nkeep, s_ccnt[4], s_off[4];
+  constexpr uint32_t NC = CERT ? 5u : 4u;
+  __shared__ uint16_t s_item[NC][kPerWg * kBandSlots];
+  __shared__ uint32_t s_nkeep, s_ccnt[NC], s_off[NC];
+  const bool certify = CERT && tile_min != nullptr && out.f != nullptr && item_mask == nullptr && p.range_mode == 0;
   const uint32_t n = *n_work;
   const uint32_t lane = threadIdx.x & 63;
   for (uint32_t base = bid * kPerWg; base < n; base += nblk * kPerWg) {
   if (threadIdx.x == 0) s_nkeep = 0;
-  if (threadIdx.x < 4) s_ccnt[threadIdx.x] = 0;
+  if (threadIdx.x < NC) s_ccnt[threadIdx.x] = 0;
   __syncthreads();
   for (uint32_t wi = base + (threadIdx.x >> 6); wi < min(n, base + kPerWg); wi += 4) {
     const uint32_t slot = work[wi];
@@ -382,6 +395,7 @@
       kslot = __shfl(kslot, 0);
       const uint32_t lpi = 64u / wpb, item = lane / lpi, sub = lane % lpi;
       bool ikeep = true;
+      [[maybe_unused]] bool ifree = false;
       if (tile_max && (p.dbg & 256) == 0) {
         const float margin = 1e-3f;
         const int patches = (p.vps * p.vps) >> 6, rows = 64 / p.vps, zr = p.vps / (static_cast<int>(wpb) / patches);
@@ -418,18 +432,38 @@
             const int nx = tx1 - tx0 + 1, nt = nx * (ty1 - ty0 + 1);
             if (tx1 >= tx0 && ty1 >= ty0 && nt <= 16 * static_cast<int>(lpi)) {
               float m0 = 0.f, m1 = 0.f;
+              [[maybe_unused]] float n0 = 1e30f, n1 = 1e30f;
               int t = static_cast<int>(sub);
               for (; t + static_cast<int>(lpi) < nt; t += 2 * static_cast<int>(lpi)) {
                 const int t2 = t + static_cast<int>(lpi);
-                const float a = tile_max[(ty0 + t / nx) * tw + tx0 + t % nx];
-                const float b = tile_max[(ty0 + t2 / nx) * tw + tx0 + t2 % nx];
+                const int ia = (ty0 + t / nx) * tw + tx0 + t % nx, ib = (ty0 + t2 / nx) * tw + tx0 + t2 % nx;
+                const float a = tile_max[ia];
+                const float b = tile_max[ib];
+                if constexpr (CERT) {
+                  const float na = certify ? tile_min[ia] : 0.f;
+                  const float nb = certify ? tile_min[ib] : 0.f;
+                  n0 = fminf(n0, na);
+                  n1 = fminf(n1, nb);
+                }
                 m0 = fmaxf(m0, a);
                 m1 = fmaxf(m1, b);
               }
-              if (t < nt) m0 = fmaxf(m0, tile_max[(ty0 + t / nx) * tw + tx0 + t % nx]);
+              if (t < nt) {
+                const int ia = (ty0 + t / nx) * tw + tx0 + t % nx;
+                const float a = tile_max[ia];
+                if constexpr (CERT) n0 = fminf(n0, certify ? tile_min[ia] : 0.f);
+                m0 = fmaxf(m0, a);
+              }
               float mr = fmaxf(m0, m1);
               for (uint32_t o = 1; o < lpi; o <<= 1) mr = fmaxf(mr, __shfl_xor(mr, static_cast<int>(o)));
               if (mr < zmin - p.trunc - margin) ikeep = false;
+              if constexpr (CERT) {
+                const bool inside = certify && static_cast<int>(floorf(umin)) - 2 >= 0 && static_cast<int>(floorf(vmin)) - 2 >= 0 &&
+                                    static_cast<int>(ceilf(umax)) + 3 <= f.W - 1 && static_cast<int>(ceilf(vmax)) + 3 <= f.H - 1;
+                float mn = fminf(n0, n1);
+                for (uint32_t o = 1; o < lpi; o <<= 1) mn = fminf(mn, __shfl_xor(mn, static_cast<int>(o)));
+                ifree = ikeep && inside && mn > zmax + p.trunc * 1.0625f + margin && mn >= f.min_range + margin && mr <= f.max_range - margin;
+              }
             }
           }
         }
@@ -441,13 +475,13 @@
         if ((old >> sh) & 0xffu) ikeep = false;
       }
       if (ikeep && sub == 0) {
-        const uint32_t cls = fuseClass(m.blk_band[static_cast<size_t>(slot) * kBandSlots + item] & kItemBandMask);
+        const uint32_t cls = (CERT && ifree) ? 4u : fuseClass(m.blk_band[static_cast<size_t>(slot) * kBandSlots + item] & kItemBandMask);
         s_item[cls][atomicAdd(&s_ccnt[cls], 1u)] = static_cast<uint16_t>((kslot << 8) | item);
       }
     }
   }
   __syncthreads();
-  if (threadIdx.x < 4) s_off[threadIdx.x] = s_ccnt[threadIdx.x] ? atomicAdd(&out.counts[threadIdx.x], s_ccnt[threadIdx.x]) : 0u;
+  if (threadIdx.x < NC) s_off[threadIdx.x] = s_ccnt[threadIdx.x] ? atomicAdd(&out.counts[threadIdx.x], s_ccnt[threadIdx.x]) : 0u;
   if (threadIdx.x == 0 && s_nkeep) atomicAdd(n_tsdf, s_nkeep);
   __syncthreads();
 #pragma unroll
@@ -457,6 +491,14 @@
       uint4 d = s_blk[it >> 8];
       d.x |= (it & 0xffu) << 24;
       *fuseDescPtr(out, cls, s_off[cls] + i) = d;
+    }
+  }
+  if constexpr (CERT) {
+    for (uint32_t i = threadIdx.x; i < s_ccnt[NC - 1]; i += blockDim.x) {
+      const uint32_t it = s_item[NC - 1][i];
+      uint4 d = s_blk[it >> 8];
+      d.x |= (it & 0xffu) << 24;
+      out.f[s_off[NC - 1] + i] = d;
     }
   }
   __syncthreads();
@@ -585,11 +627,14 @@
   initBlocks(m, p, new_list, blockIdx.x, gridDim.x);
 }
 
+template <bool CERT>
 __global__ __launch_bounds__(256) void k_init_cull(DevMap m, DevParams p, DevFrame f, const uint32_t* __restrict__ new_list,
                                                   const uint32_t* __restrict__ work, FuseList out, uint32_t wpb,
-                                                  const float* __restrict__ tile_max, int tw, int th, uint32_t n_cull) {
+                                                  const float* __restrict__ tile_max, const float* __restrict__ tile_min, int tw, int th,
+                                                  uint32_t n_cull) {
   if (blockIdx.x < n_cull)
-    cullBlocks(m, p, f, work, &m.counters[C_N_VISIBLE], out, wpb, &m.counters[C_N_TSDF], tile_max, tw, th, blockIdx.x, n_cull);
+    cullBlocks<CERT>(m, p, f, work, &m.counters[C_N_VISIBLE], out, wpb, &m.counters[C_N_TSDF], tile_max, tw, th, blockIdx.x, n_cull, nullptr, 0u,
+                     tile_min);
   else
     initBlocks(m, p, new_list, blockIdx.x - n_cull, gridDim.x - n_cull);
 }
diff --git a/khronos_amd/csrc/khronos_amd.hip b/khronos_amd/csrc/khronos_amd.hip
--- a/khronos_amd/csrc/khronos_amd.hip
+++ b/khronos_amd/csrc/khronos_amd.hip
@@ -78,6 +78,7 @@
   int32_t* obj = nullptr;
   uint8_t* rgb_staging = nullptr;
   float* tile_max = nullptr;
+  float* tile_min = nullptr;
   const float* x_depth = nullptr;
   const float* x_range = nullptr;
   const uint32_t* x_rgba = nullptr;
@@ -88,10 +89,12 @@
   const uint32_t* vRgba() const { return x_rgba ? x_rgba : rgba; }
   const int32_t* vLabel() const { return x_label ? x_label : label; }
   const float* vTileMax() const { return x_tile_max ? x_tile_max : tile_max; }
+  const float* vTileMin() const { return (x_tile_max || !has_tile_min) ? nullptr : tile_min; }
   int tw = 0, th = 0;
   khr_sensor sensor{};
   khr_frame meta{};
   bool valid = false, has_color = false, has_label = false, has_obj = false, objects_done = false;
+  bool has_tile_min = false;
   bool dyn_clean = false;
   bool dynw_valid = false;
   uint64_t aux_seq = 0;
@@ -749,6 +752,11 @@
   return KHR_OK;
 }
 
+static bool freeSpaceItems(const khr_config& cfg) {
+  return !cfg.disable_culling && cfg.range_mode == 0 && cfg.max_frame_pixels > 640u * 480u;
+}
+static bool freeSpaceItems(const khr_ctx* c) { return freeSpaceItems(c->cfg); }
+
 int khr_create(const khr_config* cfg, khr_ctx** out) {
   if (!cfg || !out) return fail(KHR_EINVAL, "null argument");
   *out = nullptr;
@@ -863,7 +871,7 @@
     c->wpb = static_cast<uint32_t>((cfg->voxels_per_side * cfg->voxels_per_side / 64) * zs);
     c->item_cap = static_cast<uint32_t>(cap) * c->wpb;
   }
-  KHR_CHAIN(devAlloc(c, &c->d_work4, 2 * static_cast<size_t>(c->item_cap), false));
+  KHR_CHAIN(devAlloc(c, &c->d_work4, (freeSpaceItems(*cfg) ? 3 : 2) * static_cast<size_t>(c->item_cap), false));
   if (cfg->voxels_per_side == 8 && rc == KHR_OK) {
     const size_t bits_words = static_cast<size_t>(c->item_cap) * 4;
     if (c->h_frames.alloc(kMaxMultiFrames) || c->d_frames.alloc(kMaxMultiFrames) || c->ev_frames.ensure() ||
@@ -953,6 +961,7 @@
     KHR_CHAIN(devAlloc(c, &s.obj, npx));
     KHR_CHAIN(devAlloc(c, &s.rgb_staging, npx * 3, false));
     KHR_CHAIN(devAlloc(c, &s.tile_max, npx / 16 + 64, false));
+    if (freeSpaceItems(*cfg)) KHR_CHAIN(devAlloc(c, &s.tile_min, npx / 16 + 64, false));
   }
   if (rc != KHR_OK) return rc;
   hipError_t e = hipMemsetAsync(m.ht_keys, 0xff, sizeof(uint64_t) * ht, c->stream);
@@ -1085,6 +1094,7 @@
   s.tw = (sensor.width + kTile - 1) / kTile;
   s.th = (sensor.height + kTile - 1) / kTile;
   s.dyn_clean = true, s.dynw_valid = false;
+  s.has_tile_min = false;
   return s;
 }
 
@@ -1141,11 +1151,12 @@
     }
   }
   hipLaunchKernelGGL(k_frame_ingest, dim3(s.tw * s.th), dim3(256), 0, ist, depth_src, rgb_src, label_src, s.depth,
-                     s.range, s.rgba, s.label, s.dyn, s.tile_max, s.tw, sensor->width, sensor->height, sensor->fx, sensor->fy,
+                     s.range, s.rgba, s.label, s.dyn, s.tile_max, freeSpaceItems(c) ? s.tile_min : nullptr, s.tw, sensor->width, sensor->height, sensor->fx, sensor->fy,
                      sensor->cx, sensor->cy, c->p.range_mode, c->m, c->p.nvox, c->d_wg_stats, opts.begin ? 1 : 0);
   HIP_TRY(hipGetLastError());
   c->begun = opts.begin;
   if (!on_device && !pinned) HIP_TRY(hipStreamSynchronize(c->stream));
+  s.has_tile_min = freeSpaceItems(c);
   s.valid = true;
   return slot;
 }
@@ -1312,6 +1323,11 @@
   return KHR_OK;
 }
 
+static FuseList windowList(khr_ctx* c) {
+  return FuseList{c->d_work4, c->d_work4 + c->item_cap, c->item_cap, &c->m.counters[C_N_ITEMS0],
+                  freeSpaceItems(c) ? c->d_work4 + 2 * static_cast<size_t>(c->item_cap) : nullptr};
+}
+
 static int integrateAlloc(khr_ctx* c, FrameSlot& s, const DevFrame& f, int allocate_blocks) {
   DevMap& m = c->m;
   if (!c->begun) hipLaunchKernelGGL(k_begin_integrate, dim3(1), dim3(256), 0, c->stream, m, c->p.nvox, c->d_wg_stats);
@@ -1324,14 +1340,17 @@
     hipLaunchKernelGGL(k_alloc_visible, dim3(gridFor(total)), dim3(256), 0, c->stream, m, c->p, f, fr, c->d_work, c->d_new,
                        c->h_pinned.dev() + 2, c->seed_publish_pending ? c->seed_ticket : 0u, &m.counters[C_N_VISIBLE], 0);
     c->seed_publish_pending = false;
-    hipLaunchKernelGGL(k_init_cull, dim3(1024 + 1024), dim3(256), 0, c->stream, m, c->p, f, c->d_new, c->d_work,
-                       FuseList{c->d_work4, c->d_work4 + c->item_cap, c->item_cap, &m.counters[C_N_ITEMS0]}, c->wpb,
-                       c->cfg.disable_culling ? nullptr : s.vTileMax(), s.tw, s.th, 1024u);
+    const float* const tile_min = freeSpaceItems(c) ? s.vTileMin() : nullptr;
+    if (tile_min != nullptr)
+      hipLaunchKernelGGL(k_init_cull<true>, dim3(1024 + 1024), dim3(256), 0, c->stream, m, c->p, f, c->d_new, c->d_work, windowList(c), c->wpb,
+                         s.vTileMax(), tile_min, s.tw, s.th, 1024u);
+    else
+      hipLaunchKernelGGL(k_init_cull<false>, dim3(1024 + 1024), dim3(256), 0, c->stream, m, c->p, f, c->d_new, c->d_work, windowList(c), c->wpb,
+                         c->cfg.disable_culling ? nullptr : s.vTileMax(), nullptr, s.tw, s.th, 1024u);
     c->host_index_valid = false, ++c->map_gen;
   } else {
     hipLaunchKernelGGL(k_list_live, dim3(gridFor(m.capacity)), dim3(256), 0, c->stream, m, c->d_work,
-                       &m.counters[C_N_VISIBLE], 0u, FuseList{c->d_work4, c->d_work4 + c->item_cap, c->item_cap, &m.counters[C_N_ITEMS0]},
-                       c->wpb);
+                       &m.counters[C_N_VISIBLE], 0u, windowList(c), c->wpb);
   }
   HIP_TRY(hipGetLastError());
   return KHR_OK;
@@ -1492,7 +1511,7 @@
 static int integrateUpdate(khr_ctx* c, FrameSlot& s, const DevFrame& f, int allocate_blocks, int use_mask,
                            int object_id, bool defer_fold, const UpdateLists* lists = nullptr, const uint32_t* gate = nullptr) {
   DevMap& m = c->m;
-  FuseList list{c->d_work4, c->d_work4 + c->item_cap, c->item_cap, &m.counters[C_N_ITEMS0]};
+  FuseList list = windowList(c);
   if (lists) list = lists->list;
   FuseArgs a{};
   fillFuseMap(c, &a);
@@ -3772,7 +3791,8 @@
   s.pool_exhausted = c->h_counters[C_POOL_EXHAUSTED];
   s.n_tsdf_blocks = c->h_counters[C_N_TSDF];
   s.n_fuse_items = static_cast<uint64_t>(c->h_counters[C_N_ITEMS0]) + c->h_counters[C_N_ITEMS1] + c->h_counters[C_N_ITEMS2] +
-                   c->h_counters[C_N_ITEMS3];
+                   c->h_counters[C_N_ITEMS3] + c->h_counters[C_N_ITEMS_FREE];
+  s.n_free_items = c->h_counters[C_N_ITEMS_FREE];
   s.n_seed_waits = c->n_seed_waits;
   s.n_seed_waits_late = c->n_seed_waits_late;
   s.seed_wait_max_us = c->seed_wait_max_us;
```
